# svohr/mixemt

Measured on AMD Instinct MI355X. Metric: read x hap cells/sec through the EM iteration (EM iters/sec reported beside it as em_iters_per_s), 1000000 reads x 5408 haps in total, whole job, higher is better.
Workload: dtype f64

## Files before the change

include/mixemt_hip.h:

```cpp
#ifndef MIXEMT_HIP_H
#define MIXEMT_HIP_H

#include <stddef.h>
#include <stdint.h>

#ifdef __cplusplus
extern "C" {
#endif

#define MXM_VERSION 603

typedef struct mxm_em_state {
    int32_t done;
    int32_t iters;
    double  l1;
    uint32_t ticket;
    uint32_t error;
} mxm_em_state;

int         mxm_version(void);
const char *mxm_last_error(void);
int         mxm_preload(void);

int         mxm_linear_supported(int32_t H);

int         mxm_restart_tile(int32_t H);

size_t      mxm_workspace_bytes(int64_t R, int32_t H, int32_t B);

int mxm_build_em_matrix(const uint8_t *E, int64_t lde,
                        const double *lhit, const double *lmiss,
                        const int64_t *row_ptr, const uint16_t *site,
                        const uint8_t *obs,
                        int64_t R, int32_t H, int32_t S,
                        double *M, int64_t ldm, void *stream);

int mxm_expand_tables(const uint8_t *maj, const int32_t *mk_ptr, const uint16_t *mk_hap, const uint8_t *mk_base,
                      const uint8_t *map256, int32_t S, int32_t H, int64_t lde, uint8_t *out, void *stream);

int mxm_build_em_matrix_lut(const uint8_t *Ecode, int64_t lde, const double *lhit, const double *lmiss,
                            const uint8_t *obsmap, const int64_t *row_ptr, const uint16_t *site,
                            const uint8_t *obs, const int64_t *order, int64_t R, int32_t H, int32_t S,
                            double *M, int64_t ldm, void *stream);

int mxm_build_em_matrix_lut_rows(const uint8_t *Ecode, int64_t lde, const double *lhit, const double *lmiss,
                                 const uint8_t *obsmap, const int64_t *row_ptr, const uint16_t *site,
                                 const uint8_t *obs, const int64_t *rows, int64_t n_rows, int32_t H, int32_t S,
                                 double *M_out, int64_t ldm, void *stream);

int mxm_build_em_matrix_sparse(const uint8_t *maj, const double *lhit, const double *lmiss,
                               const int32_t *mk_ptr, const uint16_t *mk_hap, const uint8_t *mk_base,
                               const int64_t *row_ptr, const uint16_t *site, const uint8_t *obs,
                               const int64_t *order, int64_t R, int32_t H, int32_t S,
                               double *M, int64_t ldm, int64_t *fallback, int64_t *n_fallback, void *stream);

size_t mxm_record_bytes(int64_t R, int32_t H);
int mxm_build_em_records(const uint8_t *maj, const double *lhit, const double *lmiss,
                         const int32_t *mk_ptr, const uint16_t *mk_hap, const uint8_t *mk_base,
                         const int64_t *row_ptr, const uint16_t *site, const uint8_t *obs,
                         const int64_t *order, int64_t R, int32_t H, int32_t S, double *M, int64_t ldm,
                         uint8_t *rec, size_t rec_bytes, int64_t *rec_off, int32_t *ndist, double *rowmax,
                         int64_t *stats, int64_t *fallback, int64_t *n_fallback, void *stream);

int mxm_linearize(const double *M, int64_t ldm, int64_t R, int32_t H,
                  double *P, int64_t ldp, double *rowmax, void *stream);

int mxm_em_iter(const double *M, int64_t ldm, const double *P, int64_t ldp,
                const double *w, const double *props, const double *ln_props,
                int64_t R, int32_t H, int32_t B,
                const mxm_em_state *state, double *colsum,
                void *ws, size_t ws_bytes, void *stream);

int mxm_m_finalize(const double *colsum, double *ln_cur, double *ln_new,
                   double *props_cur, int32_t H, int32_t B, double tol,
                   int32_t max_iter, mxm_em_state *state, void *stream);

int mxm_linearize_f32(const double *M, int64_t ldm, int64_t R, int32_t H,
                      float *P, int64_t ldp, double *rowmax, void *stream);
int mxm_em_iter_f32(const float *P, int64_t ldp, const double *w, const double *props,
                    int64_t R, int32_t H, int32_t B, const mxm_em_state *state,
                    double *colsum, void *ws, size_t ws_bytes, void *stream);
int mxm_em_loop_f32(const float *P, int64_t ldp, const double *w, int64_t R, int32_t H,
                    int32_t B, double *props_cur, double *ln_cur, double *ln_new,
                    double *colsum, mxm_em_state *state, double tol, int32_t max_iter,
                    int32_t check_every, void *ws, size_t ws_bytes, void *stream,
                    mxm_em_state *state_host);

typedef struct mxm_coded {
    const uint8_t *rec;
    const int64_t *rec_off;
    const int32_t *ndist;
    int64_t        R;
    const double  *P_rest;
    int64_t        ldp_rest;
    const double  *w_rest;
    int64_t        R_rest;
    const int64_t *wide_rows;
    int64_t        n_wide;
    const uint8_t *qrec;
    const int64_t *qoff;
    const int32_t *nquad;
    const int64_t *quad_rows;
    int64_t        n_quad_rows;
    const int64_t *byte_rows;
    int64_t        n_byte_rows;
} mxm_coded;
size_t mxm_coded_bytes(int64_t R, int32_t H);
size_t mxm_quad_bytes(int64_t R, int32_t H);
size_t mxm_quad_lists_scratch_bytes(int64_t R);
int mxm_quad_lists(const int32_t *ndist, const int32_t *nquad, int64_t R, int64_t *quad_rows, int64_t *byte_rows,
                   int64_t *counts, void *scratch, size_t scratch_bytes, void *stream);
int mxm_build_quads(const mxm_coded *c, int32_t H, uint8_t *qrec, size_t qrec_bytes, int64_t *qoff, int32_t *nquad,
                    uint64_t *stats, void *stream);
int mxm_encode_rows(const double *M, int64_t ldm, int64_t R, int32_t H, uint8_t *rec, size_t rec_bytes,
                    int64_t *rec_off, int32_t *ndist, double *rowmax, int64_t *stats, void *stream);
int mxm_decode_rows(const mxm_coded *c, int32_t H, double *P, int64_t ldp, void *stream);
int mxm_scatter_records(const int64_t *rows, int64_t n, const int64_t *sub_off, const int32_t *sub_nd, const double *sub_rm,
                        int64_t base, int64_t *rec_off, int32_t *ndist, double *rowmax, void *stream);
int mxm_row_argmax_votes_coded(const mxm_coded *c, int32_t H, int32_t n_runs, const double *ln_props,
                               const double *props, const double *rowmax, const double *M_rest, int64_t ldm_rest,
                               const int64_t *rest_rows, int64_t n_rest, const double *w, int32_t *best,
                               double *votes, void *ws, size_t ws_bytes, void *stream);
int mxm_em_step_coded(const mxm_coded *c, int32_t H, const double *ln_props, const double *props,
                      const double *rowmax, const double *M_rest, int64_t ldm_rest, const int64_t *rest_rows,
                      int64_t n_rest, double *out, int64_t ldo, int32_t mode, void *stream);
int mxm_gather_columns_coded(const mxm_coded *c, int32_t H, const int32_t *cols, int32_t nC,
                             const double *M_rest, int64_t ldm_rest, const int64_t *rest_rows, int64_t n_rest,
                             double *out, int64_t ldo, void *stream);
int mxm_em_iter_coded(const mxm_coded *c, const double *w, const double *props, int32_t H, int32_t B,
                      mxm_em_state *state , double *colsum, void *ws,
                      size_t ws_bytes, void *stream);
int64_t mxm_quad_loop_min_rows(int32_t B );
int mxm_restart_tile_coded(const mxm_coded *c, int32_t H);
int mxm_em_loop_coded(const mxm_coded *c, const double *w, int32_t H, int32_t B,
                      double *props_cur, double *ln_cur, double *ln_new, double *colsum,
                      mxm_em_state *state, double tol, int32_t max_iter, int32_t check_every,
                      void *ws, size_t ws_bytes, void *stream, mxm_em_state *state_host);

typedef struct mxm_sample_tile {
    int32_t sample;
    int32_t count;
    int64_t first;
} mxm_sample_tile;
int64_t mxm_samples_plan(const int64_t *row0_host, int32_t S, mxm_sample_tile *tiles_host, int64_t cap, int32_t *tile0_host);
size_t  mxm_samples_workspace_bytes(int64_t n_tiles, int32_t S, int32_t H);
int mxm_em_iter_samples(const mxm_coded *c, const int64_t *row0_host, int32_t S, const double *w, const double *props,
                        int32_t H, mxm_em_state *state, double *colsum, void *ws, size_t ws_bytes, void *stream);
int mxm_em_loop_samples(const mxm_coded *c, const int64_t *row0_host, int32_t S, const double *w, int32_t H,
                        double *props_cur, double *ln_cur, double *ln_new, double *colsum, mxm_em_state *state, double tol,
                        int32_t max_iter, int32_t check_every, void *ws, size_t ws_bytes, void *stream,
                        mxm_em_state *state_host);


int mxm_em_loop(const double *M, int64_t ldm, const double *P, int64_t ldp,
                const double *w, int64_t R, int32_t H, int32_t B,
                double *props_cur, double *ln_cur, double *ln_new, double *colsum,
                mxm_em_state *state, double tol, int32_t max_iter,
                int32_t check_every, void *ws, size_t ws_bytes, void *stream,
                mxm_em_state *state_host);

int mxm_em_step(const double *M, int64_t ldm, const double *w,
                const double *ln_props, int64_t R, int32_t H,
                double *out, int64_t ldo, int32_t mode, double *colsum,
                void *ws, size_t ws_bytes, void *stream);

int mxm_log_normalize(const double *colsum, int32_t H, double *ln_new,
                      void *stream);

int mxm_l1_exp_diff(const double *a, const double *b, int32_t H,
                    double *l1_out, void *stream);

int mxm_add_scalar(double *x, int64_t ld, int64_t R, int32_t H, double delta,
                   void *stream);

int mxm_row_argmax_votes(const double *X, int64_t ldx, const double *w,
                         int64_t R, int32_t H, int32_t *best, double *votes,
                         void *ws, size_t ws_bytes, void *stream);

int mxm_first_seen(const int32_t *best, int64_t R, int32_t H, int64_t *first, void *stream);

int mxm_assign_reads(const double *X, int64_t ldx, const double *log_props,
                     const int32_t *cols, int32_t nC, int64_t R, int32_t H,
                     double log_min_fold, int32_t *assigned, void *stream);

int mxm_gather_columns(const double *M, int64_t ldm, int64_t R, int32_t H,
                       const int32_t *cols, int32_t nC, double *out, int64_t ldo,
                       void *stream);

int mxm_fold_logaddexp(double *acc, int64_t lda, const double *const *in_host,
                       const int64_t *ld_in_host, int32_t n_in, int64_t R, int32_t H,
                       double delta, void *stream);

int64_t mxm_encode_signatures(const char *text, const int64_t *off, int64_t R,
                              const int32_t *site_of_pos, int64_t ref_len, int64_t *row_ptr,
                              uint16_t *site, uint8_t *obs, int64_t cap);

typedef struct mxm_aln_columns {
    int64_t         n_aln, n_frag;
    const int64_t  *ref_start;
    const int32_t  *mapq;
    const int64_t  *frag;
    const int64_t  *cig_ptr;
    const uint32_t *cigar;
    const int64_t  *seq_ptr;
    const uint8_t  *seq;
    const uint8_t  *qual;
    const uint8_t  *has_qual;
} mxm_aln_columns;
typedef struct mxm_aln_sizes {
    int64_t n_rows, nnz, n_grouped, n_dropped, text_bytes, n_frag_seen, frag_nnz;
} mxm_aln_sizes;
typedef struct mxm_aln_enc mxm_aln_enc;
int  mxm_aln_encode(const mxm_aln_columns *cols, const int32_t *site_of_pos, int64_t ref_len, const int64_t *site_pos,
                    int32_t n_sites, int32_t min_mq, int32_t min_bq, int32_t n_threads, mxm_aln_enc **out);
int  mxm_aln_sizes_of(const mxm_aln_enc *enc, mxm_aln_sizes *sizes);
int  mxm_aln_fetch(const mxm_aln_enc *enc, int64_t *row_ptr, uint16_t *site, uint8_t *obs, int64_t *weights,
                   int64_t *group_ptr, int64_t *group_frag, int64_t *dropped, char *text, int64_t *text_off);
int  mxm_aln_fetch_fragments(const mxm_aln_enc *enc, int64_t *frag_id, int64_t *frag_ptr, uint16_t *site, uint8_t *obs);
void mxm_aln_free(mxm_aln_enc *enc);

typedef struct mxm_bam_sizes {
    int64_t n_aln, n_frag, n_cigar, n_bases, names_bytes, n_ref, n_records_total, n_skipped_unplaced;
} mxm_bam_sizes;
typedef struct mxm_bam mxm_bam;
int  mxm_bam_read(const char *path, int32_t n_threads, mxm_bam **out);
int  mxm_bam_sizes_of(const mxm_bam *bam, mxm_bam_sizes *sizes);
int  mxm_bam_columns(const mxm_bam *bam, mxm_aln_columns *cols);
int  mxm_bam_fetch_names(const mxm_bam *bam, char *names, int64_t *name_off, int32_t *ref_id, uint16_t *flag);
void mxm_bam_free(mxm_bam *bam);

int  mxm_observe_bases(const mxm_aln_columns *cols, const uint8_t *is_reverse, int32_t min_mq, int32_t min_bq, int64_t L,
                       uint32_t *counts, void *stream);

int  mxm_observe_bases_labelled(const mxm_aln_columns *cols, const uint8_t *is_reverse, const int32_t *label,
                                int32_t n_labels, int32_t min_mq, int32_t min_bq, int64_t L, uint32_t *counts,
                                void *stream);

int  mxm_consensus(const uint32_t *counts, int32_t n_labels, int64_t L, int64_t ref_len, int64_t min_cov, int32_t strict,
                   uint8_t *cons, uint8_t *tied, uint32_t *n_tied, void *stream);

int  mxm_new_variants(const uint8_t *cons, int64_t ld, int32_t n_rows, const int32_t *rows, int32_t n_use, int64_t ref_len,
                      uint32_t *newvar, uint32_t *n_new, void *stream);

int  mxm_first_observed(const mxm_aln_columns *cols, const int32_t *label, const int32_t *joined, int32_t n_labels,
                        int32_t min_mq, int32_t min_bq, int64_t ref_len, const uint8_t *tied, uint8_t *cons, void *stream);

int  mxm_extend_assign(const mxm_aln_columns *cols, int32_t *label, int32_t *joined, int32_t unassigned, int32_t n_rows,
                       const int32_t *rows, int32_t n_use, int32_t round, int32_t min_mq, int32_t min_bq,
                       const uint32_t *newvar, int64_t ref_len, int32_t *frag_state, int32_t *moved_owner,
                       uint32_t *n_moved, void *stream);

typedef struct mxm_exchange mxm_exchange;
size_t mxm_exchange_handle_bytes(void);
int  mxm_exchange_create(int32_t world, int32_t rank, int64_t n_doubles, mxm_exchange **out, void *handle_out);
int  mxm_exchange_connect(mxm_exchange *x, const void *handles);
int  mxm_exchange_push(mxm_exchange *x, const double *colsum, int64_t n, void *stream);
int  mxm_exchange_pull(mxm_exchange *x, double *colsum, int64_t n, mxm_em_state *state, int32_t nb, void *stream);
int  mxm_exchange_reduce(mxm_exchange *x, double *colsum, int64_t n, mxm_em_state *state, int32_t nb, void *stream);
int  mxm_exchange_info(const mxm_exchange *x, int32_t *fine_grained, int64_t *bytes);
void mxm_exchange_destroy(mxm_exchange *x);

#ifdef __cplusplus
}
#endif
#include "mixemt_hip_samples_finish.h"
#include "mixemt_hip_var_check.h"
#endif
```

mixemt_amd/_lib.py:

```python

import ctypes
import os

_PKG = os.path.dirname(os.path.abspath(__file__))
LIB_PATH = os.environ.get("MXM_LIB") or os.path.join(_PKG, "lib", "libmixemt_hip.so")

c_i32, c_i64, c_f64 = ctypes.c_int32, ctypes.c_int64, ctypes.c_double
c_ptr, c_size = ctypes.c_void_p, ctypes.c_size_t


class EmState(ctypes.Structure):
    _fields_ = [("done", c_i32), ("iters", c_i32), ("l1", c_f64), ("ticket", ctypes.c_uint32), ("error", ctypes.c_uint32)]


class Coded(ctypes.Structure):
    _fields_ = [("rec", c_ptr), ("rec_off", c_ptr), ("ndist", c_ptr), ("R", c_i64),
                ("P_rest", c_ptr), ("ldp_rest", c_i64), ("w_rest", c_ptr), ("R_rest", c_i64),
                ("wide_rows", c_ptr), ("n_wide", c_i64),
                ("qrec", c_ptr), ("qoff", c_ptr), ("nquad", c_ptr), ("quad_rows", c_ptr), ("n_quad_rows", c_i64),
                ("byte_rows", c_ptr), ("n_byte_rows", c_i64)]


class SampleTile(ctypes.Structure):
    _fields_ = [("sample", c_i32), ("count", c_i32), ("first", c_i64)]


class AlnColumns(ctypes.Structure):
    _fields_ = [("n_aln", c_i64), ("n_frag", c_i64), ("ref_start", c_ptr), ("mapq", c_ptr), ("frag", c_ptr),
                ("cig_ptr", c_ptr), ("cigar", c_ptr), ("seq_ptr", c_ptr), ("seq", c_ptr), ("qual", c_ptr),
                ("has_qual", c_ptr)]


class AlnSizes(ctypes.Structure):
    _fields_ = [("n_rows", c_i64), ("nnz", c_i64), ("n_grouped", c_i64), ("n_dropped", c_i64), ("text_bytes", c_i64),
                ("n_frag_seen", c_i64), ("frag_nnz", c_i64)]


class BamSizes(ctypes.Structure):
    _fields_ = [("n_aln", c_i64), ("n_frag", c_i64), ("n_cigar", c_i64), ("n_bases", c_i64), ("names_bytes", c_i64),
                ("n_ref", c_i64), ("n_records_total", c_i64), ("n_skipped_unplaced", c_i64)]


SIGNATURES = {
    "mxm_version": (ctypes.c_int, []),
    "mxm_last_error": (ctypes.c_char_p, []),
    "mxm_linear_supported": (ctypes.c_int, [c_i32]),
    "mxm_workspace_bytes": (c_size, [c_i64, c_i32, c_i32]),
    "mxm_restart_tile": (ctypes.c_int, [c_i32]),
    "mxm_restart_tile_coded": (ctypes.c_int, [ctypes.POINTER(Coded), c_i32]),
    "mxm_quad_loop_min_rows": (c_i64, [c_i32]),
    "mxm_build_em_matrix": (ctypes.c_int, [c_ptr, c_i64, c_ptr, c_ptr, c_ptr, c_ptr, c_ptr,
                                           c_i64, c_i32, c_i32, c_ptr, c_i64, c_ptr]),
    "mxm_build_em_matrix_lut": (ctypes.c_int, [c_ptr, c_i64, c_ptr, c_ptr, c_ptr, c_ptr, c_ptr, c_ptr, c_ptr,
                                               c_i64, c_i32, c_i32, c_ptr, c_i64, c_ptr]),
    "mxm_build_em_matrix_sparse": (ctypes.c_int, [c_ptr, c_ptr, c_ptr, c_ptr, c_ptr, c_ptr, c_ptr, c_ptr, c_ptr, c_ptr,
                                                  c_i64, c_i32, c_i32, c_ptr, c_i64, c_ptr, c_ptr, c_ptr]),
    "mxm_build_em_matrix_lut_rows": (ctypes.c_int, [c_ptr, c_i64, c_ptr, c_ptr, c_ptr, c_ptr, c_ptr, c_ptr, c_ptr,
                                                    c_i64, c_i32, c_i32, c_ptr, c_i64, c_ptr]),
    "mxm_scatter_records": (ctypes.c_int, [c_ptr, c_i64, c_ptr, c_ptr, c_ptr, c_i64, c_ptr, c_ptr, c_ptr, c_ptr]),
    "mxm_preload": (ctypes.c_int, []),
    "mxm_record_bytes": (c_size, [c_i64, c_i32]),
    "mxm_build_em_records": (ctypes.c_int, [c_ptr, c_ptr, c_ptr, c_ptr, c_ptr, c_ptr, c_ptr, c_ptr, c_ptr, c_ptr,
                                            c_i64, c_i32, c_i32, c_ptr, c_i64, c_ptr, c_size, c_ptr, c_ptr, c_ptr,
                                            c_ptr, c_ptr, c_ptr, c_ptr]),
    "mxm_linearize": (ctypes.c_int, [c_ptr, c_i64, c_i64, c_i32, c_ptr, c_i64, c_ptr, c_ptr]),
    "mxm_em_iter": (ctypes.c_int, [c_ptr, c_i64, c_ptr, c_i64, c_ptr, c_ptr, c_ptr, c_i64, c_i32, c_i32,
                                   c_ptr, c_ptr, c_ptr, c_size, c_ptr]),
    "mxm_m_finalize": (ctypes.c_int, [c_ptr, c_ptr, c_ptr, c_ptr, c_i32, c_i32, c_f64, c_i32, c_ptr,
                                      c_ptr]),
    "mxm_em_loop": (ctypes.c_int, [c_ptr, c_i64, c_ptr, c_i64, c_ptr, c_i64, c_i32, c_i32,
                                   c_ptr, c_ptr, c_ptr, c_ptr, c_ptr, c_f64, c_i32, c_i32, c_ptr, c_size,
                                   c_ptr, ctypes.POINTER(EmState)]),
    "mxm_linearize_f32": (ctypes.c_int, [c_ptr, c_i64, c_i64, c_i32, c_ptr, c_i64, c_ptr, c_ptr]),
    "mxm_em_iter_f32": (ctypes.c_int, [c_ptr, c_i64, c_ptr, c_ptr, c_i64, c_i32, c_i32, c_ptr, c_ptr, c_ptr,
                                       c_size, c_ptr]),
    "mxm_em_loop_f32": (ctypes.c_int, [c_ptr, c_i64, c_ptr, c_i64, c_i32, c_i32, c_ptr, c_ptr, c_ptr, c_ptr,
                                       c_ptr, c_f64, c_i32, c_i32, c_ptr, c_size, c_ptr,
                                       ctypes.POINTER(EmState)]),
    "mxm_coded_bytes": (c_size, [c_i64, c_i32]),
    "mxm_exchange_handle_bytes": (c_size, []),
    "mxm_exchange_create": (ctypes.c_int, [c_i32, c_i32, c_i64, ctypes.POINTER(c_ptr), c_ptr]),
    "mxm_exchange_connect": (ctypes.c_int, [c_ptr, c_ptr]),
    "mxm_exchange_push": (ctypes.c_int, [c_ptr, c_ptr, c_i64, c_ptr]),
    "mxm_exchange_pull": (ctypes.c_int, [c_ptr, c_ptr, c_i64, c_ptr, c_i32, c_ptr]),
    "mxm_exchange_reduce": (ctypes.c_int, [c_ptr, c_ptr, c_i64, c_ptr, c_i32, c_ptr]),
    "mxm_exchange_info": (ctypes.c_int, [c_ptr, ctypes.POINTER(c_i32), ctypes.POINTER(c_i64)]),
    "mxm_exchange_destroy": (None, [c_ptr]),
    "mxm_expand_tables": (ctypes.c_int, [c_ptr, c_ptr, c_ptr, c_ptr, c_ptr, c_i32, c_i32, c_i64, c_ptr, c_ptr]),
    "mxm_quad_bytes": (c_size, [c_i64, c_i32]),
    "mxm_quad_lists_scratch_bytes": (c_size, [c_i64]),
    "mxm_quad_lists": (ctypes.c_int, [c_ptr, c_ptr, c_i64, c_ptr, c_ptr, c_ptr, c_ptr, c_size, c_ptr]),
    "mxm_build_quads": (ctypes.c_int, [ctypes.POINTER(Coded), c_i32, c_ptr, c_size, c_ptr, c_ptr, c_ptr, c_ptr]),
    "mxm_encode_rows": (ctypes.c_int, [c_ptr, c_i64, c_i64, c_i32, c_ptr, c_size, c_ptr, c_ptr, c_ptr, c_ptr, c_ptr]),
    "mxm_decode_rows": (ctypes.c_int, [ctypes.POINTER(Coded), c_i32, c_ptr, c_i64, c_ptr]),
    "mxm_row_argmax_votes_coded": (ctypes.c_int, [ctypes.POINTER(Coded), c_i32, c_i32, c_ptr, c_ptr, c_ptr, c_ptr, c_i64,
                                                  c_ptr, c_i64, c_ptr, c_ptr, c_ptr, c_ptr, c_size, c_ptr]),
    "mxm_em_step_coded": (ctypes.c_int, [ctypes.POINTER(Coded), c_i32, c_ptr, c_ptr, c_ptr, c_ptr, c_i64, c_ptr, c_i64,
                                         c_ptr, c_i64, c_i32, c_ptr]),
    "mxm_gather_columns_coded": (ctypes.c_int, [ctypes.POINTER(Coded), c_i32, c_ptr, c_i32, c_ptr, c_i64, c_ptr, c_i64,
                                                c_ptr, c_i64, c_ptr]),
    "mxm_em_iter_coded": (ctypes.c_int, [ctypes.POINTER(Coded), c_ptr, c_ptr, c_i32, c_i32, c_ptr, c_ptr, c_ptr,
                                         c_size, c_ptr]),
    "mxm_em_loop_coded": (ctypes.c_int, [ctypes.POINTER(Coded), c_ptr, c_i32, c_i32, c_ptr, c_ptr, c_ptr, c_ptr,
                                         c_ptr, c_f64, c_i32, c_i32, c_ptr, c_size, c_ptr,
                                         ctypes.POINTER(EmState)]),
    "mxm_samples_tile_rows": (ctypes.c_int, []),
    "mxm_samples_plan": (c_i64, [c_ptr, c_i32, c_ptr, c_i64, c_ptr]),
    "mxm_samples_workspace_bytes": (c_size, [c_i64, c_i32, c_i32]),
    "mxm_em_iter_samples": (ctypes.c_int, [ctypes.POINTER(Coded), c_ptr, c_i32, c_ptr, c_ptr, c_i32, c_ptr, c_ptr, c_ptr,
                                           c_size, c_ptr]),
    "mxm_em_loop_samples": (ctypes.c_int, [ctypes.POINTER(Coded), c_ptr, c_i32, c_ptr, c_i32, c_ptr, c_ptr, c_ptr, c_ptr,
                                           c_ptr, c_f64, c_i32, c_i32, c_ptr, c_size, c_ptr, ctypes.POINTER(EmState)]),
    "mxm_em_step": (ctypes.c_int, [c_ptr, c_i64, c_ptr, c_ptr, c_i64, c_i32, c_ptr, c_i64, c_i32,
                                   c_ptr, c_ptr, c_size, c_ptr]),
    "mxm_log_normalize": (ctypes.c_int, [c_ptr, c_i32, c_ptr, c_ptr]),
    "mxm_l1_exp_diff": (ctypes.c_int, [c_ptr, c_ptr, c_i32, c_ptr, c_ptr]),
    "mxm_add_scalar": (ctypes.c_int, [c_ptr, c_i64, c_i64, c_i32, c_f64, c_ptr]),
    "mxm_assign_reads": (ctypes.c_int, [c_ptr, c_i64, c_ptr, c_ptr, c_i32, c_i64, c_i32, c_f64, c_ptr, c_ptr]),
    "mxm_diag_stream_read": (ctypes.c_int, [c_ptr, c_size, c_i32, c_i32, c_ptr, c_ptr]),
    "mxm_diag_stream_coded": (ctypes.c_int, [ctypes.POINTER(Coded), c_i32, c_i32, c_ptr, c_ptr]),
    "mxm_diag_stream_quads": (ctypes.c_int, [ctypes.POINTER(Coded), c_i32, c_i32, c_ptr, c_ptr]),
    "mxm_diag_fused_force_abort": (ctypes.c_int, [c_i32]),
    "mxm_set_fused_coded_grid": (ctypes.c_int, [c_i32]),
    "mxm_set_quad_left_grid": (ctypes.c_int, [c_i32]),
    "mxm_set_coded_batch_tile": (ctypes.c_int, [c_i32]),
    "mxm_set_sparse_long_rows": (ctypes.c_int, [c_i32]),
    "mxm_set_quad_encoder": (ctypes.c_int, [c_i32]),
    "mxm_set_sparse_long_entries": (ctypes.c_int, [c_i32]),
    "mxm_diag_fused_stamps": (ctypes.c_int, [c_ptr, ctypes.POINTER(ctypes.c_ulonglong)]),
    "mxm_set_timing_events": (ctypes.c_int, [c_ptr, c_ptr]),
    "mxm_set_batch_tile": (ctypes.c_int, [c_i32]),
    "mxm_encode_signatures": (ctypes.c_int64, [ctypes.c_char_p, c_ptr, c_i64, c_ptr, c_i64, c_ptr, c_ptr, c_ptr,
                                               c_i64]),
    "mxm_aln_encode": (ctypes.c_int, [ctypes.POINTER(AlnColumns), c_ptr, c_i64, c_ptr, c_i32, c_i32, c_i32, c_i32,
                                      ctypes.POINTER(c_ptr)]),
    "mxm_aln_sizes_of": (ctypes.c_int, [c_ptr, ctypes.POINTER(AlnSizes)]),
    "mxm_aln_fetch": (ctypes.c_int, [c_ptr, c_ptr, c_ptr, c_ptr, c_ptr, c_ptr, c_ptr, c_ptr, c_ptr, c_ptr]),
    "mxm_aln_fetch_fragments": (ctypes.c_int, [c_ptr, c_ptr, c_ptr, c_ptr, c_ptr]),
    "mxm_aln_free": (None, [c_ptr]),
    "mxm_bam_read": (ctypes.c_int, [ctypes.c_char_p, c_i32, ctypes.POINTER(c_ptr)]),
    "mxm_bam_sizes_of": (ctypes.c_int, [c_ptr, ctypes.POINTER(BamSizes)]),
    "mxm_bam_columns": (ctypes.c_int, [c_ptr, ctypes.POINTER(AlnColumns)]),
    "mxm_bam_fetch_names": (ctypes.c_int, [c_ptr, c_ptr, c_ptr, c_ptr, c_ptr]),
    "mxm_bam_free": (None, [c_ptr]),
    "mxm_observe_bases": (ctypes.c_int, [ctypes.POINTER(AlnColumns), c_ptr, c_i32, c_i32, c_i64, c_ptr, c_ptr]),
    "mxm_observe_bases_labelled": (ctypes.c_int, [ctypes.POINTER(AlnColumns), c_ptr, c_ptr, c_i32, c_i32, c_i32, c_i64,
                                                  c_ptr, c_ptr]),
    "mxm_consensus": (ctypes.c_int, [c_ptr, c_i32, c_i64, c_i64, c_i64, c_i32, c_ptr, c_ptr, c_ptr, c_ptr]),
    "mxm_new_variants": (ctypes.c_int, [c_ptr, c_i64, c_i32, ctypes.POINTER(c_i32), c_i32, c_i64, c_ptr, c_ptr, c_ptr]),
    "mxm_first_observed": (ctypes.c_int, [ctypes.POINTER(AlnColumns), c_ptr, c_ptr, c_i32, c_i32, c_i32, c_i64, c_ptr,
                                          c_ptr, c_ptr]),
    "mxm_extend_assign": (ctypes.c_int, [ctypes.POINTER(AlnColumns), c_ptr, c_ptr, c_i32, c_i32, ctypes.POINTER(c_i32),
                                         c_i32, c_i32, c_i32, c_i32, c_ptr, c_i64, c_ptr, c_ptr, c_ptr, c_ptr]),
    "mxm_set_compact_restarts": (ctypes.c_int, [c_i32]),
    "mxm_set_loop_graph": (ctypes.c_int, [c_i32]),
    "mxm_set_loop_fused": (ctypes.c_int, [c_i32, c_i32]),
    "mxm_set_progress_callback": (ctypes.c_int, [c_ptr, c_ptr, c_i32]),
    "mxm_set_min_rows_per_wg": (ctypes.c_int, [c_i32]),
    "mxm_reset_tuning": (ctypes.c_int, []),
    "mxm_describe_stream_kernel": (ctypes.c_int, [c_i32, c_i32, ctypes.c_char_p, c_size]),
    "mxm_set_sparse_max_distinct": (ctypes.c_int, [c_i32]),
    "mxm_row_argmax_votes": (ctypes.c_int, [c_ptr, c_i64, c_ptr, c_i64, c_i32, c_ptr, c_ptr,
                                            c_ptr, c_size, c_ptr]),
    "mxm_first_seen": (ctypes.c_int, [c_ptr, c_i64, c_i32, c_ptr, c_ptr]),
    "mxm_gather_columns": (ctypes.c_int, [c_ptr, c_i64, c_i64, c_i32, c_ptr, c_i32, c_ptr, c_i64, c_ptr]),
    "mxm_fold_logaddexp": (ctypes.c_int, [c_ptr, c_i64, ctypes.POINTER(c_ptr), ctypes.POINTER(c_i64), c_i32,
                                          c_i64, c_i32, c_f64, c_ptr]),
}

FINISH_SIGNATURES = {
    "mxm_samples_finish_workspace_bytes": (c_size, [c_i64, c_i32, c_i32]),
    "mxm_votes_samples": (ctypes.c_int, [ctypes.POINTER(Coded), c_ptr, c_i32, c_i32, c_ptr, c_ptr, c_ptr, c_ptr, c_ptr, c_ptr,
                                         c_ptr, c_ptr, c_ptr, c_ptr, c_ptr, c_size, c_ptr]),
    "mxm_gather_columns_samples": (ctypes.c_int, [ctypes.POINTER(Coded), c_ptr, c_i32, c_i32, c_ptr, c_ptr, c_i32, c_ptr,
                                                  c_ptr, c_size, c_ptr]),
    "mxm_em_loop_samples_narrow": (ctypes.c_int, [ctypes.POINTER(Coded), c_ptr, c_i32, c_i32, c_ptr, c_i32, c_ptr, c_ptr,
                                                  c_ptr, c_ptr, c_ptr, c_ptr, c_f64, c_i32, c_i32, c_ptr, c_ptr, c_size,
                                                  c_ptr, ctypes.POINTER(EmState)]),
    "mxm_assign_reads_samples": (ctypes.c_int, [ctypes.POINTER(Coded), c_ptr, c_i32, c_i32, c_ptr, c_i32, c_ptr, c_ptr,
                                                c_ptr, c_ptr, c_ptr, c_ptr, c_f64, c_ptr, c_ptr, c_ptr, c_size, c_ptr]),
}

VARCHECK_SIGNATURES = {
    "mxm_check_variants_samples": (ctypes.c_int, [c_ptr, c_i32, c_i64, c_ptr, c_ptr, c_i32, c_ptr, c_ptr, c_i32, c_i64, c_ptr,
                                                  c_ptr, c_i32, c_f64, c_f64, c_f64, c_i32, c_i32, c_ptr, c_ptr, c_ptr, c_ptr]),
}

ABI_VERSION = 603

PROGRESS_FN = ctypes.CFUNCTYPE(None, ctypes.POINTER(EmState), c_i32, c_ptr)

_lib = None


class MixemtHipError(RuntimeError):
    pass


def load():
    global _lib
    if _lib is not None:
        return _lib
    if not os.path.exists(LIB_PATH):
        raise MixemtHipError(
            "libmixemt_hip.so is not built (%s); run `python -m mixemt_amd.build` -- "
            "there is no CPU fallback for the EM hot path" % LIB_PATH)
    from . import _dev
    lib = ctypes.CDLL(LIB_PATH)
    try:
        lib.mxm_version.restype = ctypes.c_int
        lib.mxm_version.argtypes = []
        have = lib.mxm_version()
    except AttributeError:
        have = None
    if have != ABI_VERSION:
        raise MixemtHipError("%s reports ABI version %s, this binding was written for %d: rebuild with "
                             "`python -m mixemt_amd.build --force`" % (LIB_PATH, have, ABI_VERSION))
    for name, (restype, argtypes) in (list(SIGNATURES.items()) + list(FINISH_SIGNATURES.items())
                                      + list(VARCHECK_SIGNATURES.items())):
        try:
            fn = getattr(lib, name)
        except AttributeError:
            raise MixemtHipError("%s has ABI version %d but lacks %s: rebuild with "
                                 "`python -m mixemt_amd.build --force`" % (LIB_PATH, have, name))
        fn.restype = restype
        fn.argtypes = argtypes
    _lib = lib
    try:
        if _dev.torch is not None and _dev.torch.cuda.is_available():
            lib.mxm_preload()
    except Exception:
        pass
    return lib


def check(rc, what):
    if rc != 0:
        msg = load().mxm_last_error().decode("utf-8", "replace")
        raise ValueError("%s failed (%d): %s" % (what, rc, msg))
```

mixemt_amd/build.py:

```python

import hashlib
import os
import shutil
import subprocess
import sys

_PKG = os.path.dirname(os.path.abspath(__file__))
_ROOT = os.path.dirname(_PKG)
SRC = os.path.join(_PKG, "csrc", "mixemt_hip.hip")
HDRS = [os.path.join(_ROOT, "include", name) for name in ("mixemt_hip.h", "mixemt_hip_tuning.h", "mixemt_hip_samples_finish.h",
                                                           "mixemt_hip_var_check.h")]
LIB_DIR = os.path.join(_PKG, "lib")
LIB = os.path.join(LIB_DIR, "libmixemt_hip.so")
ARCH = "gfx950"


def _hipcc():
    for cand in (os.environ.get("HIPCC"), shutil.which("hipcc"), "/opt/rocm/bin/hipcc"):
        if cand and os.path.exists(cand):
            return cand
    raise RuntimeError("hipcc not found (set HIPCC or add /opt/rocm/bin to PATH)")


def _sources():
    csrc = os.path.dirname(SRC)
    return sorted(os.path.join(csrc, f) for f in os.listdir(csrc) if f.endswith((".hip", ".hpp"))) + HDRS


def _digest(flags):
    h = hashlib.sha256()
    for path in _sources():
        with open(path, "rb") as fin:
            h.update(fin.read())
    h.update(" ".join(flags).encode())
    return h.hexdigest()


def build(force=False, defines=(), verbose=False, out=None):
    global LIB
    if out is not None:
        LIB = os.path.abspath(out)
    flags = ["--offload-arch=%s" % ARCH, "-O3", "-std=c++17", "-shared", "-fPIC", "-Werror=format",
             "-I" + os.path.join(_ROOT, "include"), "-I" + os.path.dirname(SRC)]
    flags += ["-D%s" % d for d in defines]
    stamp = LIB + ".stamp"
    want = _digest(flags)
    if not force and os.path.exists(LIB) and os.path.exists(stamp):
        with open(stamp) as fin:
            if fin.read().strip() == want:
                return LIB
    os.makedirs(os.path.dirname(LIB), exist_ok=True)
    cmd = [_hipcc()] + flags + [SRC, "-o", LIB, "-lz"]
    if verbose:
        sys.stderr.write(" ".join(cmd) + "\n")
    proc = subprocess.run(cmd, stdout=subprocess.PIPE, stderr=subprocess.STDOUT, text=True)
    if proc.returncode != 0:
        raise RuntimeError("hipcc failed:\n" + proc.stdout)
    with open(stamp, "w") as fout:
        fout.write(want + "\n")
    return LIB


if __name__ == "__main__":
    defs = []
    argv = sys.argv[1:]
    i = 0
    while i < len(argv):
        if argv[i] == "-D":
            defs.append(argv[i + 1])
            i += 2
        elif argv[i].startswith("-D"):
            defs.append(argv[i][2:])
            i += 1
        else:
            i += 1
    out_path = argv[argv.index("--out") + 1] if "--out" in argv else None
    print(build(force="--force" in argv, defines=defs, verbose=True, out=out_path))
```

mixemt_amd/csrc/mixemt_hip.hip:

```cpp
#include <hip/hip_runtime.h>
#include <stdint.h>
#include <stdio.h>
#include <stdlib.h>
#include <string.h>
#include <math.h>
#include <algorithm>
#include <atomic>
#include <mutex>
#include <type_traits>
#include <utility>
#include <vector>

#include "mixemt_hip.h"
#include "mixemt_hip_tuning.h"

#include "common.hpp"
#include "aln_encode.hpp"
#include "bam_reader.hpp"
#include "coded_kernels.hpp"
#include "quad_kernels.hpp"
#include "quad_batched_kernels.hpp"
#include "build_kernels.hpp"
#include "build_lut_kernels.hpp"
#include "build_sparse_kernels.hpp"
#include "em_kernels.hpp"
#include "estep_kernels.hpp"
#include "aux_kernels.hpp"
#include "records_kernels.hpp"
#include "fused_kernels.hpp"
#include "fused_cols_kernels.hpp"
#include "fused_coded_kernels.hpp"
#include "fused_narrow_kernels.hpp"
#include "samples_kernels.hpp"
#include "samples_finish_kernels.hpp"
#include "exchange.hpp"
#include "aln_walk.hpp"
#include "observe_kernels.hpp"
#include "var_check_kernels.hpp"
#include "assemble_kernels.hpp"


struct mxm_em_state;
typedef void (*mxm_progress_fn)(const mxm_em_state *state_host, int32_t B, void *user);
struct mxm_tuning {
    int sparse_maxd = -1;
    int min_rows_per_wg = 8;
    int compact_restarts = 2;
    int max_bt = 4;
    int loop_graph = -1;
    int loop_fused = -1;
    int fused_chunk = 0;
    int fused_cols = 1;
    int fused_coded_wg = 0;
    int quad_left_wg = 0;
    int sparse_long_entries = 5120;
    int quad_encoder = 1;
    int sparse_long = 1;
    int coded_bt = 3;
    int fused_force_abort = 0;
    double fused_cells = 1.0e8;
    hipEvent_t ev_start = nullptr, ev_stop = nullptr;
    mxm_progress_fn progress = nullptr;
    void *progress_user = nullptr;
    int progress_every = 10;
};
static std::mutex g_tune_mu;
static mxm_tuning g_tune;
static thread_local mxm_tuning T;
#define MXM_ENTER() do { std::lock_guard<std::mutex> lk_(g_tune_mu); T = g_tune; } while (0)
template <typename F>
static int tune_set(F f) {
    std::lock_guard<std::mutex> lk(g_tune_mu);
    f(g_tune);
    return 0;
}
extern "C" int mxm_reset_tuning(void) {
    return tune_set([](mxm_tuning &t) { t = mxm_tuning(); });
}

static inline int clamp_grid(int64_t want, int cap) {
    if (want < 1) want = 1;
    return (int)(want < cap ? want : cap);
}

static inline int64_t part_ld(int H) { return ((int64_t)H + 1) & ~(int64_t)1; }

static hipError_t raise_dynamic_lds(const void *kernel, size_t bytes, const char *name) {
    const hipError_t e = hipFuncSetAttribute(kernel, hipFuncAttributeMaxDynamicSharedMemorySize, (int)bytes);
    if (e != hipSuccess)
        snprintf(g_err, sizeof(g_err), "%s: cannot opt into %zu bytes of dynamic LDS: %s", name, bytes,
                 hipGetErrorString(e));
    return e;
}
static int dynamic_lds_ok(const void *kernel, size_t bytes, const char *name, const char *who = nullptr, int H = 0,
                          const char *too_wide = nullptr) {
    if (too_wide != nullptr && bytes > 150 * 1024) return fail(-1, "%s: H=%d %s", who, H, too_wide);
    if (bytes > 60 * 1024 && raise_dynamic_lds(kernel, bytes, name) != hipSuccess) return -2;
    return 0;
}

#define RC_TRY(expr)                                                                         \
    do {                                                                                     \
        const int rc_ = (expr);                                                              \
        if (rc_ != 0) return rc_;                                                            \
    } while (0)

template <int MAX, typename F>
static bool dispatch_width(int n, F &&f) {
    if constexpr (MAX < 1) {
        return false;
    } else {
        if (n != MAX) return dispatch_width<MAX - 1>(n, f);
        f(std::integral_constant<int, MAX>{});
        return true;
    }
}

extern "C" int mxm_version(void) { return MXM_VERSION; }
extern "C" const char *mxm_last_error(void) { return g_err; }

extern "C" int mxm_linear_supported(int32_t H) {
    return (H >= MXM_LINEAR_MIN_H && H <= 8192) ? 1 : 0;
}

static size_t fused_sync_bytes() { return (sizeof(fused_sync) + 255) & ~(size_t)255; }
static size_t fused_snapshot_bytes(int H, int B) {
    return ((size_t)3 * B * H * sizeof(double) + (size_t)B * sizeof(mxm_em_state) + 255) & ~(size_t)255;
}
static size_t fused_rows_bytes(int H, int nwg) { return (size_t)(nwg + 2) * part_ld(H) * sizeof(double); }
static size_t fused_cols_bytes(int64_t R, int nwg) {
    const size_t ldz = (size_t)((R + 1) & ~(int64_t)1);
    return ((size_t)(nwg + 1) * ldz + 2 * (size_t)nwg) * sizeof(double);
}

extern "C" size_t mxm_workspace_bytes(int64_t R, int32_t H, int32_t B) {
    const size_t tiles = (size_t)MXM_MAX_WG * MXM_MAX_BT * (size_t)part_ld(H) * sizeof(double);
    size_t fused = fused_rows_bytes(H, MXM_MAX_WG);
    if (R > 0 && R <= (int64_t)FCOLS_MAX_RPT * FCOLS_THREADS) fused = std::max(fused, fused_cols_bytes(R, MXM_MAX_WG));
    fused += fused_sync_bytes() + fused_snapshot_bytes(H, B > 0 ? B : 1) + 512;
    return std::max(tiles, fused);
}

extern "C" int64_t mxm_encode_signatures(const char *text, const int64_t *off, int64_t R,
                                         const int32_t *site_of_pos, int64_t ref_len, int64_t *row_ptr,
                                         uint16_t *site, uint8_t *obs, int64_t cap) {
    int64_t n = 0;
    row_ptr[0] = 0;
    for (int64_t r = 0; r < R; ++r) {
        const char *p = text + off[r];
        const char *end = text + off[r + 1] - 1;
        if (p >= end) return -(r + 1);
        while (p < end) {
            int64_t pos = 0;
            int digits = 0;
            while (p < end && *p >= '0' && *p <= '9' && digits < 10) {
                pos = pos * 10 + (*p - '0');
                ++p;
                ++digits;
            }
            if (digits == 0 || digits >= 10 || p >= end || *p != ':') return -(r + 1);
            ++p;
            const char *b = p;
            while (p < end && *p != ',') {
                if (*p == ':') return -(r + 1);
                ++p;
            }
            if (pos >= ref_len || site_of_pos[pos] < 0 || n >= cap) return -(r + 1);
            site[n] = (uint16_t)site_of_pos[pos];
            obs[n] = (p - b == 1) ? (uint8_t)*b : (uint8_t)0;
            ++n;
            if (p < end) {
                ++p;
                if (p >= end) return -(r + 1);
            }
        }
        row_ptr[r + 1] = n;
    }
    return n;
}

extern "C" int mxm_build_em_matrix(const uint8_t *E, int64_t lde, const double *lhit,
                                   const double *lmiss, const int64_t *row_ptr, const uint16_t *site,
                                   const uint8_t *obs, int64_t R, int32_t H, int32_t S, double *M,
                                   int64_t ldm, void *stream) {
    if (R < 0 || H <= 0 || S <= 0) return fail(-1, "mxm_build_em_matrix: bad shape R=%lld H=%d", (long long)R, H);
    if (lde < (((int64_t)H + 7) & ~(int64_t)7) || (lde & 7) != 0 || (reinterpret_cast<uintptr_t>(E) & 7) != 0)
        return fail(-1, "mxm_build_em_matrix: E must be 8-byte aligned with lde a multiple of 8 and >= H rounded up to 8 (lde=%lld)", (long long)lde);
    if (ldm < H) return fail(-1, "mxm_build_em_matrix: ldm < H");
    if (S > 65536) return fail(-1, "mxm_build_em_matrix: more than 65536 variant sites");
    if (R == 0) return 0;
    const int grid = clamp_grid(R, num_cu() * 8);
    const int vec_ok = ((ldm & 1) == 0) && ((reinterpret_cast<uintptr_t>(M) & 15) == 0);
    hipLaunchKernelGGL(build_em_matrix_kernel, dim3(grid), dim3(BUILD_THREADS), 0, (hipStream_t)stream, E,
                       lde, lhit, lmiss, row_ptr, site, obs, R, (int)H, M, ldm, vec_ok);
    HIP_TRY(hipGetLastError());
    return 0;
}

static int build_lut_impl(const char *who, const uint8_t *Ecode, int64_t lde, const double *lhit,
                          const double *lmiss, const uint8_t *obsmap, const int64_t *row_ptr, const uint16_t *site,
                          const uint8_t *obs, const int64_t *order, int64_t R, int32_t H, int32_t S, double *M, int64_t ldm,
                          int compact, hipStream_t s) {
    if (H > 8192) return fail(-1, "%s: more than 8192 haplogroups (H=%d)%s", who, H, compact ? "" : ": use mxm_build_em_matrix");
    if (lde < (((int64_t)H + 7) & ~(int64_t)7) || (lde & 7) != 0 || (reinterpret_cast<uintptr_t>(Ecode) & 7) != 0)
        return fail(-1, "%s: Ecode must be 8-byte aligned with lde a multiple of 8 and >= H rounded up to 8 (lde=%lld)", who, (long long)lde);
    if (ldm < H) return fail(-1, "%s: ldm < H", who);
    if (S > 65536 || (int64_t)S * lde >= ((int64_t)1 << 31))
        return fail(-1, "%s: table of %d x %lld bytes exceeds one buffer descriptor", who, S, (long long)lde);
    if (R == 0) return 0;
    const int grid = clamp_grid(R, num_cu() * 8);
    const int nt = (H + LUT_THREADS * LUT_CPL - 1) / (LUT_THREADS * LUT_CPL);
    const int vec_ok = ((ldm & 1) == 0) && ((reinterpret_cast<uintptr_t>(M) & 15) == 0);
    const bool ok = dispatch_width<8>(nt, [&](auto n) {
        constexpr int NT = decltype(n)::value;
        hipLaunchKernelGGL((build_lut_kernel<NT, LUT_CPL>), dim3(grid), dim3(LUT_THREADS), 0, s, Ecode, lde, (int64_t)S * lde, lhit,
                           lmiss, obsmap, row_ptr, site, obs, order, R, (int)H, M, ldm, vec_ok, compact);
    });
    if (!ok) return fail(-1, "%s: H=%d outside the kernel's range", who, H);
    HIP_TRY(hipGetLastError());
    return 0;
}

extern "C" int mxm_build_em_matrix_lut(const uint8_t *Ecode, int64_t lde, const double *lhit, const double *lmiss,
                                       const uint8_t *obsmap, const int64_t *row_ptr, const uint16_t *site,
                                       const uint8_t *obs, const int64_t *order, int64_t R, int32_t H, int32_t S,
                                       double *M, int64_t ldm, void *stream) {
    if (R < 0 || H <= 0 || S <= 0) return fail(-1, "mxm_build_em_matrix_lut: bad shape R=%lld H=%d", (long long)R, H);
    return build_lut_impl("mxm_build_em_matrix_lut", Ecode, lde, lhit, lmiss, obsmap, row_ptr, site, obs,
                          order, R, H, S, M, ldm, 0, (hipStream_t)stream);
}

extern "C" int mxm_build_em_matrix_lut_rows(const uint8_t *Ecode, int64_t lde, const double *lhit, const double *lmiss,
                                            const uint8_t *obsmap, const int64_t *row_ptr, const uint16_t *site,
                                            const uint8_t *obs, const int64_t *rows, int64_t n_rows, int32_t H, int32_t S,
                                            double *M_out, int64_t ldm, void *stream) {
    if (n_rows < 0 || H <= 0 || S <= 0 || rows == nullptr) return fail(-1, "mxm_build_em_matrix_lut_rows: bad arguments");
    return build_lut_impl("mxm_build_em_matrix_lut_rows", Ecode, lde, lhit, lmiss, obsmap, row_ptr, site, obs, rows, n_rows, H, S,
                          M_out, ldm, 1, (hipStream_t)stream);
}

__global__ __launch_bounds__(256) void scatter_records_kernel(const int64_t *__restrict__ rows, int64_t n, const int64_t *__restrict__ sub_off,
                                                             const int32_t *__restrict__ sub_nd, const double *__restrict__ sub_rm,
                                                             int64_t base, int64_t *__restrict__ rec_off, int32_t *__restrict__ ndist,
                                                             double *__restrict__ rowmax) {
    const int64_t i = (int64_t)blockIdx.x * 256 + threadIdx.x;
    if (i >= n || sub_nd[i] <= 0) return;
    const int64_t r = rows[i];
    rec_off[r] = sub_off[i] + base;
    ndist[r] = sub_nd[i];
    rowmax[r] = sub_rm[i];
}
extern "C" int mxm_scatter_records(const int64_t *rows, int64_t n, const int64_t *sub_off, const int32_t *sub_nd, const double *sub_rm,
                                   int64_t base, int64_t *rec_off, int32_t *ndist, double *rowmax, void *stream) {
    if (n < 0 || (n > 0 && (rows == nullptr || sub_off == nullptr || sub_nd == nullptr || sub_rm == nullptr || rec_off == nullptr ||
                            ndist == nullptr || rowmax == nullptr)))
        return fail(-1, "mxm_scatter_records: bad arguments");
    if (n == 0) return 0;
    hipLaunchKernelGGL(scatter_records_kernel, dim3((unsigned)((n + 255) / 256)), dim3(256), 0, (hipStream_t)stream, rows, n, sub_off,
                       sub_nd, sub_rm, base, rec_off, ndist, rowmax);
    HIP_TRY(hipGetLastError());
    return 0;
}

__global__ void preload_kernel() {}
extern "C" int mxm_preload(void) {
    hipLaunchKernelGGL(preload_kernel, dim3(1), dim3(64), 0, (hipStream_t)nullptr);
    HIP_TRY(hipGetLastError());
    HIP_TRY(hipDeviceSynchronize());
    return 0;
}

extern "C" int mxm_set_sparse_max_distinct(int32_t n) {
    return tune_set([n](mxm_tuning &t) { t.sparse_maxd = n < 0 ? -1 : n; });
}

static inline int coded_ld(int H) { return (H + 7) & ~7; }

static int build_sparse_impl(const char *who, const uint8_t *maj, const double *lhit, const double *lmiss,
                             const int32_t *mk_ptr, const uint16_t *mk_hap, const uint8_t *mk_base,
                             const int64_t *row_ptr, const uint16_t *site, const uint8_t *obs, const int64_t *order,
                             int64_t R, int32_t H, int32_t S, double *M, int64_t ldm, const spb_records *out,
                             int64_t *fallback, int64_t *n_fallback, hipStream_t s) {
    if (R < 0 || H <= 0 || S <= 0) return fail(-1, "%s: bad shape R=%lld H=%d", who, (long long)R, H);
    if (H > 8192) return fail(-1, "%s: more than 8192 haplogroups (H=%d): use mxm_build_em_matrix", who, H);
    if (M != nullptr && ldm < H) return fail(-1, "%s: ldm < H", who);
    if (maj == nullptr || mk_ptr == nullptr || fallback == nullptr || n_fallback == nullptr)
        return fail(-1, "%s: marker tables and the fallback list are required", who);
    HIP_TRY(hipMemsetAsync(n_fallback, 0, sizeof(int64_t), s));
    if (out != nullptr) HIP_TRY(hipMemsetAsync(out->stats, 0, 2 * sizeof(int64_t), s));
    if (R == 0) return 0;
    const int hpad = (H + 1) & ~1;
    const int nch = (hpad / 2 + SPB_THREADS - 1) / SPB_THREADS;
    const int vec_ok = (M != nullptr) && ((ldm & 1) == 0) && ((reinterpret_cast<uintptr_t>(M) & 15) == 0);
#ifndef SPB_PASSES
#define SPB_PASSES 3
#endif
    const int passes = SPB_PASSES;
    const int maxd = (T.sparse_maxd < 0 || T.sparse_maxd > SPB_MAXD) ? SPB_MAXD : T.sparse_maxd;
    const int maxd_long = (T.sparse_maxd < 0 || T.sparse_maxd > SPB_MAXD_LONG) ? SPB_MAXD_LONG : T.sparse_maxd;
    const int kpp = (nch + passes - 1) / passes;
    const size_t lds = (size_t)kpp * 2 * SPB_THREADS * 8 + SPB_SLOTS * 8 + 6 * 1024;
    int per_cu = (int)((160 * 1024) / lds);
    if (per_cu > 8) per_cu = 8;
    if (per_cu < 1) per_cu = 1;
    const int grid = clamp_grid(R, num_cu() * per_cu * 2);
    const int long_too = T.sparse_long;
    const int grid_long = clamp_grid((R + SPB_LONG_CHUNK - 1) / SPB_LONG_CHUNK, num_cu() * 4 * 2);
    spb_records none = {};
    const spb_records rec = out != nullptr ? *out : none;
    auto launch = [&](auto kernel, int nwg, int max_distinct, int long_rows_too, int long_entries) {
        hipLaunchKernelGGL(kernel, dim3(nwg), dim3(SPB_THREADS), 0, s, maj, lhit, lmiss, mk_ptr, mk_hap, mk_base, row_ptr, site, obs,
                           order, R, (int)H, M, ldm, vec_ok, fallback, reinterpret_cast<unsigned long long *>(n_fallback), max_distinct,
                           rec, long_rows_too, long_entries);
    };
    constexpr int P = SPB_PASSES < 4 ? SPB_PASSES : 4;
    bool one_pass_too_wide = false;
    const bool ok = dispatch_width<16>(nch, [&](auto n) {
        constexpr int N = decltype(n)::value;
        if constexpr (P == 1 && N > 7) one_pass_too_wide = true;
        else if (out != nullptr) launch(build_sparse_kernel<N, P, true, 1>, grid, maxd, long_too, 0);
        else launch(build_sparse_kernel<N, P, false, 1>, grid, maxd, long_too, 0);
    });
    if (one_pass_too_wide) return fail(-1, "%s: one pass covers H <= 3584", who);
    if (!ok) return fail(-1, "%s: H=%d outside the kernel's range", who, H);
    HIP_TRY(hipGetLastError());
    if (long_too != 0) {
#ifndef SPB_LONG_KPP
#define SPB_LONG_KPP 2
#endif
        (void)dispatch_width<16>(nch, [&](auto n) {
            constexpr int N = decltype(n)::value, PL = (N + SPB_LONG_KPP - 1) / SPB_LONG_KPP;
            if (out != nullptr) launch(build_sparse_kernel<N, PL, true, 2>, grid_long, maxd_long, 0, T.sparse_long_entries);
            else launch(build_sparse_kernel<N, PL, false, 2>, grid_long, maxd_long, 0, T.sparse_long_entries);
        });
    }
    HIP_TRY(hipGetLastError());
    return 0;
}

extern "C" int mxm_build_em_matrix_sparse(const uint8_t *maj, const double *lhit, const double *lmiss,
                                          const int32_t *mk_ptr, const uint16_t *mk_hap, const uint8_t *mk_base,
                                          const int64_t *row_ptr, const uint16_t *site, const uint8_t *obs,
                                          const int64_t *order, int64_t R, int32_t H, int32_t S, double *M, int64_t ldm,
                                          int64_t *fallback, int64_t *n_fallback, void *stream) {
    MXM_ENTER();
    if (M == nullptr) return fail(-1, "mxm_build_em_matrix_sparse: M required");
    return build_sparse_impl("mxm_build_em_matrix_sparse", maj, lhit, lmiss, mk_ptr, mk_hap, mk_base, row_ptr, site, obs,
                             order, R, H, S, M, ldm, nullptr, fallback, n_fallback, (hipStream_t)stream);
}

extern "C" size_t mxm_record_bytes(int64_t R, int32_t H) {
    if (R < 0 || H <= 0) return 0;
    return (size_t)(R > 0 ? R : 1) * (2 * (size_t)coded_ld(H) + 16 * ENC_MAX_WIDE);
}

extern "C" int mxm_build_em_records(const uint8_t *maj, const double *lhit, const double *lmiss,
                                    const int32_t *mk_ptr, const uint16_t *mk_hap, const uint8_t *mk_base,
                                    const int64_t *row_ptr, const uint16_t *site, const uint8_t *obs,
                                    const int64_t *order, int64_t R, int32_t H, int32_t S, double *M, int64_t ldm,
                                    uint8_t *rec, size_t rec_bytes, int64_t *rec_off, int32_t *ndist, double *rowmax,
                                    int64_t *stats, int64_t *fallback, int64_t *n_fallback, void *stream) {
    MXM_ENTER();
    if (!mxm_linear_supported(H))
        return fail(-1, "mxm_build_em_records: records need H in [65, 8192] (H=%d)", H);
    if (rec == nullptr || (reinterpret_cast<uintptr_t>(rec) & 15) || rec_bytes < (size_t)coded_ld(H) + 16 * ENC_MAX_CODES ||
        rec_off == nullptr || ndist == nullptr || rowmax == nullptr || stats == nullptr)
        return fail(-1, "mxm_build_em_records: record buffer (16-byte aligned, >= one record) and output arrays required");
    spb_records out;
    out.rec = rec;
    out.rec_cap = (long long)rec_bytes;
    out.rec_off = rec_off;
    out.ndist = ndist;
    out.rowmax = rowmax;
    out.stats = reinterpret_cast<unsigned long long *>(stats);
    out.ldc = coded_ld(H);
    return build_sparse_impl("mxm_build_em_records", maj, lhit, lmiss, mk_ptr, mk_hap, mk_base, row_ptr, site, obs, order,
                             R, H, S, M, ldm, &out, fallback, n_fallback, (hipStream_t)stream);
}

template <typename ST>
static int linearize_wide(const double *M, int64_t ldm, int64_t R, int H, ST *P, int64_t ldp, double *rowmax,
                          hipStream_t s) {
    const int nch = (H / 2 + 255) / 256;
    int cap = num_cu() * 2 < MXM_MAX_WG ? num_cu() * 2 : MXM_MAX_WG;
    const int nwg = clamp_grid((R + 1) / 2, cap);
    const bool ok = dispatch_width<16>(nch, [&](auto n) {
        hipLaunchKernelGGL((linearize_wide_kernel<decltype(n)::value, ST>), dim3(nwg), dim3(256), 0, s, M, ldm, R, H, P, ldp, rowmax);
    });
    return ok ? 0 : 1;
}

static inline bool wide_rows_ok(const void *M, int64_t ldm, int H) {
    return ((H & 1) == 0) && ((ldm & 1) == 0) && ((reinterpret_cast<uintptr_t>(M) & 15) == 0) && H >= 64 && H <= 8192;
}

extern "C" int mxm_linearize(const double *M, int64_t ldm, int64_t R, int32_t H, double *P, int64_t ldp,
                             double *rowmax, void *stream) {
    if (R < 0 || H <= 0) return fail(-1, "mxm_linearize: bad shape");
    if (ldm < H || ldp < H || (ldp & 1)) return fail(-1, "mxm_linearize: ldp must be even and >= H (ldp=%lld)", (long long)ldp);
    if (R == 0) return 0;
    if (wide_rows_ok(M, ldm, H) && (reinterpret_cast<uintptr_t>(P) & 15) == 0 &&
        linearize_wide<double>(M, ldm, R, (int)H, P, ldp, rowmax, (hipStream_t)stream) == 0) {
        HIP_TRY(hipGetLastError());
        return 0;
    }
    const int grid = clamp_grid(R, num_cu() * 8);
    hipLaunchKernelGGL(linearize_kernel, dim3(grid), dim3(ROW_THREADS), 0, (hipStream_t)stream, M, ldm, R,
                       (int)H, P, ldp, rowmax);
    HIP_TRY(hipGetLastError());
    return 0;
}

extern "C" int mxm_set_timing_events(void *ev_start, void *ev_stop) {
    return tune_set([=](mxm_tuning &t) { t.ev_start = (hipEvent_t)ev_start; t.ev_stop = (hipEvent_t)ev_stop; });
}

extern "C" int mxm_set_min_rows_per_wg(int32_t n) {
    if (n < 1) return fail(-1, "mxm_set_min_rows_per_wg: n < 1");
    return tune_set([n](mxm_tuning &t) { t.min_rows_per_wg = n; });
}

extern "C" int mxm_set_compact_restarts(int32_t mode) {
    return tune_set([mode](mxm_tuning &t) { t.compact_restarts = mode < 0 ? 0 : (mode > 2 ? 2 : mode); });
}

extern "C" int mxm_set_batch_tile(int32_t bt) {
    if (bt < 1 || bt > 4) return fail(-1, "mxm_set_batch_tile: tile must be 1..4");
    return tune_set([bt](mxm_tuning &t) { t.max_bt = bt; });
}

extern "C" int mxm_set_fused_coded_grid(int32_t nwg) {
    return tune_set([nwg](mxm_tuning &t) { t.fused_coded_wg = nwg > 0 ? nwg : 0; });
}

extern "C" int mxm_set_sparse_long_rows(int32_t on) {
    return tune_set([on](mxm_tuning &t) { t.sparse_long = on ? 1 : 0; });
}
extern "C" int mxm_set_sparse_long_entries(int32_t n) {
    return tune_set([n](mxm_tuning &t) { t.sparse_long_entries = n > 0 ? n : 0; });
}
extern "C" int mxm_set_coded_batch_tile(int32_t bt) {
    if (bt != 1 && bt != 3) return fail(-1, "mxm_set_coded_batch_tile: 1 or 3, got %d", bt);
    return tune_set([bt](mxm_tuning &t) { t.coded_bt = bt; });
}
extern "C" int mxm_set_quad_encoder(int32_t kind) {
    if (kind != 0 && kind != 1) return fail(-1, "mxm_set_quad_encoder: 0 or 1, got %d", kind);
    return tune_set([kind](mxm_tuning &t) { t.quad_encoder = kind; });
}
extern "C" int mxm_set_quad_left_grid(int32_t nwg) {
    return tune_set([nwg](mxm_tuning &t) { t.quad_left_wg = nwg > 0 ? nwg : 0; });
}

extern "C" int mxm_diag_fused_force_abort(int32_t on) {
    return tune_set([on](mxm_tuning &t) { t.fused_force_abort = on ? 1 : 0; });
}

#ifndef MXM_V1_THREADS
#define MXM_V1_THREADS 256
#endif
#ifndef MXM_V1_NBUF
#define MXM_V1_NBUF 2
#endif
#ifndef MXM_V1_WG_PER_CU
#define MXM_V1_WG_PER_CU 2
#endif
#ifndef MXM_V2_THREADS
#define MXM_V2_THREADS 512
#endif
#ifndef MXM_V2_NBUF
#define MXM_V2_NBUF 2
#endif
#ifndef MXM_V3_THREADS
#define MXM_V3_THREADS 512
#endif
#ifndef MXM_V3_NBUF
#define MXM_V3_NBUF 2
#endif
#ifndef MXM_V4_THREADS
#define MXM_V4_THREADS 512
#endif
#ifndef MXM_V4_NBUF
#define MXM_V4_NBUF 2
#endif
#ifndef MXM_V2_PREG
#define MXM_V2_PREG 1
#endif
#ifndef MXM_V3_PREG
#define MXM_V3_PREG 2
#endif
#ifndef MXM_V4_PREG
#define MXM_V4_PREG 2
#endif
#ifndef MXM_V1B_THREADS
#define MXM_V1B_THREADS 512
#endif
#ifndef MXM_V1B_NBUF
#define MXM_V1B_NBUF 3
#endif
#define MXM_MAX_COL2 4096
#define MXM_LDS_BUDGET (156 * 1024)

static inline int variant_threads(int nb) {
    return nb == 1 ? MXM_V1_THREADS : (nb == 2 ? MXM_V2_THREADS : (nb == 3 ? MXM_V3_THREADS : MXM_V4_THREADS));
}
static inline int variant_preg(int nb) {
    return nb == 1 ? 1 : (nb == 2 ? MXM_V2_PREG : (nb == 3 ? MXM_V3_PREG : MXM_V4_PREG));
}

static size_t batch_lds_bytes(int H, int nb) {
    const int threads = variant_threads(nb);
    const int nch = ((H + 1) / 2 + threads - 1) / threads;
    return (size_t)(nb - variant_preg(nb)) * nch * threads * 16;
}

static bool batch_fits(int H, int nb) {
    if (nb <= 1) return true;
    static const int max_nch[MXM_MAX_BT + 1] = {0, 16, 8, 7, 6};
    const int threads = variant_threads(nb);
    const int nch = ((H + 1) / 2 + threads - 1) / threads;
    return nch <= max_nch[nb] && batch_lds_bytes(H, nb) <= MXM_LDS_BUDGET;
}

template <int THREADS, int NCH, int BT, int NBUF, int PREG>
static int launch_wide(const double *P, int64_t ldp, const double *w, const double *props, int64_t R,
                       int H, int grid, double *partial, int64_t ldpart,
                       const mxm_em_state *state, mxm_slots slots, hipStream_t stream) {
    if constexpr (NCH * THREADS > MXM_MAX_COL2) {
        return fail(-1, "mxm_em_iter: H=%d outside the linear kernel's range", H);
    } else {
        const size_t lds = (size_t)(BT - PREG) * NCH * THREADS * sizeof(d2);
        RC_TRY(dynamic_lds_ok(reinterpret_cast<const void *>(&em_iter_wide_kernel<THREADS, NCH, BT, NBUF, PREG>), lds, "em_iter_wide_kernel"));
        hipLaunchKernelGGL((em_iter_wide_kernel<THREADS, NCH, BT, NBUF, PREG>), dim3(grid), dim3(THREADS), lds,
                           stream, P, ldp, w, props, R, H, partial, ldpart, state, slots);
        return 0;
    }
}

template <int THREADS, int BT, int NBUF, int PREG>
static int dispatch_wide(int nch, const double *P, int64_t ldp, const double *w, const double *props,
                         int64_t R, int H, int grid, double *partial,
                         int64_t ldpart, const mxm_em_state *state, mxm_slots slots, hipStream_t stream) {
    int rc = 0;
    const bool ok = dispatch_width<16>(nch, [&](auto n) {
        rc = launch_wide<THREADS, decltype(n)::value, BT, NBUF, PREG>(P, ldp, w, props, R, H, grid, partial, ldpart, state, slots, stream);
    });
    return ok ? rc : fail(-1, "mxm_em_iter: H=%d outside the linear kernel's range", H);
}

static inline mxm_slots slots_from(int first) {
    mxm_slots sl;
    for (int i = 0; i < MXM_MAX_BT; ++i) sl.s[i] = first + i;
    return sl;
}

static int stream_linear_tile(const double *P, int64_t ldp, const double *w, const double *props, int64_t R,
                              int H, int nb, mxm_slots &slots, const mxm_em_state *state,
                              double *partial, hipStream_t stream, bool timed, int *nwg_out, int max_wg = MXM_MAX_WG,
                              int v1_shape = -1) {
    const int64_t ldpart = part_ld(H);
    const int ncol2 = (H + 1) / 2;
    if (v1_shape < 0) v1_shape = 1;
    const bool alt = (nb == 1) && (v1_shape == 1);
    const int threads = alt ? MXM_V1B_THREADS : variant_threads(nb);
    const int wg_per_cu = alt ? 1 : ((nb == 1) ? MXM_V1_WG_PER_CU : 1);
    const int nch = (ncol2 + threads - 1) / threads;
    int cap = num_cu() * wg_per_cu;
    if (cap > max_wg) cap = max_wg;
    const int nwg = clamp_grid((R + T.min_rows_per_wg - 1) / T.min_rows_per_wg, cap);
    for (int i = nb; i < MXM_MAX_BT; ++i) slots.s[i] = slots.s[0];
    if (timed && T.ev_start != nullptr) HIP_TRY(hipEventRecord(T.ev_start, stream));
    int rc;
    if (alt)
        rc = dispatch_wide<MXM_V1B_THREADS, 1, MXM_V1B_NBUF, 1>(nch, P, ldp, w, props, R, H, nwg, partial, ldpart, state, slots, stream);
    else if (nb == 1)
        rc = dispatch_wide<MXM_V1_THREADS, 1, MXM_V1_NBUF, 1>(nch, P, ldp, w, props, R, H, nwg, partial, ldpart, state, slots, stream);
    else if (nb == 2)
        rc = dispatch_wide<MXM_V2_THREADS, 2, MXM_V2_NBUF, MXM_V2_PREG>(nch, P, ldp, w, props, R, H, nwg, partial, ldpart, state, slots, stream);
    else if (nb == 3)
        rc = dispatch_wide<MXM_V3_THREADS, 3, MXM_V3_NBUF, MXM_V3_PREG>(nch, P, ldp, w, props, R, H, nwg, partial, ldpart, state, slots, stream);
    else
        rc = dispatch_wide<MXM_V4_THREADS, 4, MXM_V4_NBUF, MXM_V4_PREG>(nch, P, ldp, w, props, R, H, nwg, partial, ldpart, state, slots, stream);
    if (rc != 0) return rc;
    HIP_TRY(hipGetLastError());
    if (timed && T.ev_stop != nullptr) HIP_TRY(hipEventRecord(T.ev_stop, stream));
    *nwg_out = nwg;
    return 0;
}

extern "C" int mxm_describe_stream_kernel(int32_t H, int32_t nb, char *buf, size_t len) {
    if (buf == nullptr || len == 0 || H <= 0 || nb < 1 || nb > MXM_MAX_BT) return fail(-1, "mxm_describe_stream_kernel: bad arguments");
    const int ncol2 = (H + 1) / 2;
    const bool alt = nb == 1;
    const int threads = alt ? MXM_V1B_THREADS : variant_threads(nb);
    const int nbuf = alt ? MXM_V1B_NBUF : (nb == 2 ? MXM_V2_NBUF : (nb == 3 ? MXM_V3_NBUF : MXM_V4_NBUF));
    snprintf(buf, len, "em_iter_wide_kernel<%d, %d, %d, %d, %d>", threads, (ncol2 + threads - 1) / threads, nb, nbuf,
             variant_preg(nb));
    return 0;
}

struct fin_args {
    double *ln_cur, *ln_new, *props_cur;
    mxm_em_state *state;
    double tol;
    int max_iter;
};

static int reduce_tile(const double *partial, int nwg, int nb, int H, double *colsum, const mxm_em_state *state,
                       const mxm_slots &slots, const fin_args *fin, hipStream_t stream,
                       wide_check wc = wide_check{nullptr, 0, 0}) {
    if (fin != nullptr && H <= 64 * FIN_MAX_BLOCKS)
        hipLaunchKernelGGL(colreduce_finalize_kernel, dim3((H + 63) / 64, nb), dim3(COLRED_THREADS), 0, stream, partial,
                           part_ld(H), nwg, nb, H, colsum, fin->ln_cur, fin->ln_new, fin->props_cur, fin->tol, fin->max_iter,
                           fin->state, slots, wc);
    else
        hipLaunchKernelGGL(colreduce_kernel, dim3((H + 63) / 64, nb), dim3(COLRED_THREADS), 0, stream, partial, part_ld(H), nwg,
                           nb, H, (const double *)nullptr, colsum, const_cast<mxm_em_state *>(state), slots, wc);
    HIP_TRY(hipGetLastError());
    return 0;
}

static int reduce_one(const double *partial, int nwg, int H, double *colsum, const mxm_em_state *state, hipStream_t stream) {
    hipLaunchKernelGGL(colreduce_kernel, dim3((H + 63) / 64, 1), dim3(COLRED_THREADS), 0, stream, partial, part_ld(H), nwg, 1, H,
                       (const double *)nullptr, colsum, const_cast<mxm_em_state *>(state), slots_from(0), wide_check{nullptr, 0, 0});
    HIP_TRY(hipGetLastError());
    return 0;
}

static int em_iter_linear_tile(const double *P, int64_t ldp, const double *w, const double *props, int64_t R,
                               int H, int nb, mxm_slots slots, const mxm_em_state *state, double *colsum,
                               double *partial, hipStream_t stream, bool timed, const fin_args *fin = nullptr) {
    int nwg = 0;
    RC_TRY(stream_linear_tile(P, ldp, w, props, R, H, nb, slots, state, partial, stream, timed, &nwg));
    return reduce_tile(partial, nwg, nb, H, colsum, state, slots, fin, stream);
}

#ifndef MXM_F32_THREADS
#define MXM_F32_THREADS 256
#endif
#ifndef MXM_F32_NBUF
#define MXM_F32_NBUF 2
#endif
#ifndef MXM_F32_WG_PER_CU
#define MXM_F32_WG_PER_CU 2
#endif

template <int NCH>
static int launch_wide_f32(const float *P, int64_t ldp, const double *w, const double *props, int64_t R, int H,
                           int grid, double *partial, int64_t ldpart,
                           const mxm_em_state *state, hipStream_t stream) {
    if constexpr (NCH * MXM_F32_THREADS > 2048) {
        return fail(-1, "mxm_em_iter_f32: H=%d outside the kernel's range", H);
    } else {
        hipLaunchKernelGGL((em_iter_wide_f32_kernel<MXM_F32_THREADS, NCH, MXM_F32_NBUF>), dim3(grid),
                           dim3(MXM_F32_THREADS), 0, stream, P, ldp, w, props, R, H, partial, ldpart,
                           state);
        return 0;
    }
}

static int em_iter_f32_one(const float *P, int64_t ldp, const double *w, const double *props, int64_t R, int H,
                           const mxm_em_state *state, double *colsum, double *partial, hipStream_t stream,
                           bool timed) {
    const int64_t ldpart = part_ld(H);
    const int nch = ((H + 3) / 4 + MXM_F32_THREADS - 1) / MXM_F32_THREADS;
    const int nbuf = MXM_F32_NBUF;
    int cap = num_cu() * MXM_F32_WG_PER_CU;
    if (cap > MXM_MAX_WG) cap = MXM_MAX_WG;
    const int nwg = clamp_grid((R + nbuf - 1) / nbuf, cap);
    if (timed && T.ev_start != nullptr) HIP_TRY(hipEventRecord(T.ev_start, stream));
    int lrc = 0;
    const bool ok = dispatch_width<8>(nch, [&](auto n) {
        lrc = launch_wide_f32<decltype(n)::value>(P, ldp, w, props, R, H, nwg, partial, ldpart, state, stream);
    });
    if (!ok) return fail(-1, "mxm_em_iter_f32: H=%d outside the kernel's range", H);
    if (lrc != 0) return lrc;
    HIP_TRY(hipGetLastError());
    if (timed && T.ev_stop != nullptr) HIP_TRY(hipEventRecord(T.ev_stop, stream));
    return reduce_one(partial, nwg, H, colsum, state, stream);
}

#define MXM_NARROW_MAX_H 64
template <bool ITER>
static int launch_narrow(const double *M, int64_t ldm, const double *w, const double *ln_props, int64_t R, int H,
                         double *out, int64_t ldo, int mode, double *partial, int64_t ldpart,
                         const mxm_em_state *state, hipStream_t stream, int *nwg_out) {
    const int cap = num_cu() * 4 < MXM_MAX_WG ? num_cu() * 4 : MXM_MAX_WG;
    const int rows_per_wg = (H <= 32) ? 256 : 128;
    const int nwg = clamp_grid((R + rows_per_wg - 1) / rows_per_wg, cap);
    *nwg_out = nwg;
#define NARROW_LAUNCH(hmax, lpr)                                                                             \
    hipLaunchKernelGGL((estep_narrow_kernel<hmax, ITER, lpr>), dim3(nwg), dim3(256), 0, stream, M, ldm, w, ln_props, R, H, \
                       out, ldo, mode, partial, ldpart, state)
    if (H <= 4) NARROW_LAUNCH(4, 1);
    else if (H <= 8) NARROW_LAUNCH(8, 1);
    else if (H <= 16) NARROW_LAUNCH(16, 1);
    else if (H <= 32) NARROW_LAUNCH(32, 1);
    else NARROW_LAUNCH(32, 2);
#undef NARROW_LAUNCH
    HIP_TRY(hipGetLastError());
    return 0;
}

static int em_iter_log_one(const double *M, int64_t ldm, const double *w, const double *ln_props, int64_t R, int H,
                           const mxm_em_state *state, double *colsum, double *partial, hipStream_t stream) {
    if (M == nullptr) return fail(-1, "mxm_em_iter: M is NULL and the linear path does not apply");
    if (ln_props == nullptr) return fail(-1, "mxm_em_iter: ln_props is NULL and the log-space path needs it");
    const size_t lds = 2 * (size_t)H * sizeof(double);
    const int64_t ldpart = part_ld(H);
    int nwg;
    if (lds > 150 * 1024) {
        nwg = clamp_grid(R, num_cu() * 2 < MXM_MAX_WG ? num_cu() * 2 : MXM_MAX_WG);
        hipLaunchKernelGGL((estep_global_kernel<true>), dim3(nwg), dim3(ROW_THREADS), 0, stream, M, ldm, w, ln_props, R, H,
                           (double *)nullptr, (int64_t)0, 0, partial, ldpart, state, (const int64_t *)nullptr);
        HIP_TRY(hipGetLastError());
    } else if (H <= MXM_NARROW_MAX_H) {
        const int rc = launch_narrow<true>(M, ldm, w, ln_props, R, H, (double *)nullptr, (int64_t)0, 0, partial, ldpart,
                                           state, stream, &nwg);
        if (rc != 0) return rc;
    } else {
        nwg = clamp_grid(R, num_cu() * 2 < MXM_MAX_WG ? num_cu() * 2 : MXM_MAX_WG);
        RC_TRY(dynamic_lds_ok(reinterpret_cast<const void *>(&estep_log_kernel<true>), lds, "estep_log_kernel"));
        hipLaunchKernelGGL((estep_log_kernel<true>), dim3(nwg), dim3(ROW_THREADS), lds, stream, M, ldm, w, ln_props,
                           R, H, (double *)nullptr, (int64_t)0, 0, partial, ldpart, state);
        HIP_TRY(hipGetLastError());
    }
    return reduce_one(partial, nwg, H, colsum, state, stream);
}

extern "C" int mxm_em_iter(const double *M, int64_t ldm, const double *P, int64_t ldp, const double *w,
                           const double *props, const double *ln_props, int64_t R, int32_t H, int32_t B,
                           const mxm_em_state *state, double *colsum, void *ws, size_t ws_bytes, void *stream) {
    MXM_ENTER();
    if (R <= 0 || H <= 0 || B <= 0) return fail(-1, "mxm_em_iter: bad shape R=%lld H=%d", (long long)R, H);
    if (ws == nullptr || ws_bytes < mxm_workspace_bytes(R, H, B)) return fail(-1, "mxm_em_iter: workspace too small");
    if (P != nullptr && ((ldp & 1) || ldp < H)) return fail(-1, "mxm_em_iter: ldp must be even and >= H");
    if (M != nullptr && ldm < H) return fail(-1, "mxm_em_iter: ldm < H");
    const bool linear = (P != nullptr) && mxm_linear_supported(H);
    int max_bt = linear ? T.max_bt : 1;
    while (max_bt > 1 && !batch_fits((int)H, max_bt)) --max_bt;
    for (int b = 0; b < B;) {
        const int left = B - b;
        const int passes = (left + max_bt - 1) / max_bt;
        const int nb = (left + passes - 1) / passes;
        const mxm_em_state *st = state ? state + b : nullptr;
        int rc;
        if (linear)
            rc = em_iter_linear_tile(P, ldp, w, props, R, (int)H, nb, slots_from(b), state, colsum, (double *)ws,
                                     (hipStream_t)stream, b == 0);
        else
            rc = em_iter_log_one(M, ldm, w, ln_props ? ln_props + (int64_t)b * H : nullptr, R, (int)H, st,
                                 colsum + (int64_t)b * H, (double *)ws, (hipStream_t)stream);
        if (rc != 0) return rc;
        b += nb;
    }
    return 0;
}

extern "C" int mxm_linearize_f32(const double *M, int64_t ldm, int64_t R, int32_t H, float *P, int64_t ldp,
                                 double *rowmax, void *stream) {
    if (R < 0 || H <= 0) return fail(-1, "mxm_linearize_f32: bad shape");
    if (ldm < H || ldp < H || (ldp & 3)) return fail(-1, "mxm_linearize_f32: ldp must be a multiple of 4 and >= H (ldp=%lld)", (long long)ldp);
    if (R == 0) return 0;
    if (wide_rows_ok(M, ldm, H) && (reinterpret_cast<uintptr_t>(P) & 7) == 0 && (ldp & 1) == 0 &&
        linearize_wide<float>(M, ldm, R, (int)H, P, ldp, rowmax, (hipStream_t)stream) == 0) {
        HIP_TRY(hipGetLastError());
        return 0;
    }
    const int grid = clamp_grid(R, num_cu() * 8);
    hipLaunchKernelGGL(linearize_f32_kernel, dim3(grid), dim3(ROW_THREADS), 0, (hipStream_t)stream, M, ldm, R, (int)H,
                       P, ldp, rowmax);
    HIP_TRY(hipGetLastError());
    return 0;
}

extern "C" int mxm_em_iter_f32(const float *P, int64_t ldp, const double *w, const double *props, int64_t R,
                               int32_t H, int32_t B, const mxm_em_state *state, double *colsum, void *ws,
                               size_t ws_bytes, void *stream) {
    MXM_ENTER();
    if (R <= 0 || H <= 0 || B <= 0) return fail(-1, "mxm_em_iter_f32: bad shape R=%lld H=%d", (long long)R, H);
    if (!mxm_linear_supported(H)) return fail(-1, "mxm_em_iter_f32: H=%d outside the linear kernel's range", H);
    if (P == nullptr || (ldp & 3) || ldp < H) return fail(-1, "mxm_em_iter_f32: ldp must be a multiple of 4 and >= H");
    if (ws == nullptr || ws_bytes < mxm_workspace_bytes(R, H, B)) return fail(-1, "mxm_em_iter_f32: workspace too small");
    for (int b = 0; b < B; ++b) {
        const int rc = em_iter_f32_one(P, ldp, w, props + (int64_t)b * H, R, (int)H, state ? state + b : nullptr,
                                       colsum + (int64_t)b * H, (double *)ws, (hipStream_t)stream, b == 0);
        if (rc != 0) return rc;
    }
    return 0;
}

extern "C" size_t mxm_coded_bytes(int64_t R, int32_t H) { return mxm_record_bytes(R, H); }

extern "C" int mxm_encode_rows(const double *M, int64_t ldm, int64_t R, int32_t H, uint8_t *rec, size_t rec_bytes,
                               int64_t *rec_off, int32_t *ndist, double *rowmax, int64_t *stats, void *stream) {
    if (R <= 0 || H <= 0 || ldm < H) return fail(-1, "mxm_encode_rows: bad shape R=%lld H=%d", (long long)R, H);
    if (!mxm_linear_supported(H) || (reinterpret_cast<uintptr_t>(M) & 7) != 0)
        return fail(-1, "mxm_encode_rows: needs H in [65, 8192] (H=%d ldm=%lld)", H, (long long)ldm);
    if (rec == nullptr || (reinterpret_cast<uintptr_t>(rec) & 15) || rec_bytes < (size_t)coded_ld(H) + 16 * ENC_MAX_CODES)
        return fail(-1, "mxm_encode_rows: record buffer missing, unaligned or smaller than one record");
    if (rec_off == nullptr || ndist == nullptr || rowmax == nullptr || stats == nullptr)
        return fail(-1, "mxm_encode_rows: output arrays required");
    hipStream_t s = (hipStream_t)stream;
    HIP_TRY(hipMemsetAsync(stats, 0, 2 * sizeof(int64_t), s));
    const int ldc = coded_ld(H);
    const int nch = (ldc / 4 + ENC_THREADS - 1) / ENC_THREADS;
    const int grid = clamp_grid(R, num_cu() * 4);
    const int grid_w = clamp_grid((R + 31) / 32, num_cu() * 3);
    const bool ok = dispatch_width<8>(nch, [&](auto n) {
        constexpr int NCH = decltype(n)::value;
        unsigned long long *st = reinterpret_cast<unsigned long long *>(stats);
        hipLaunchKernelGGL((encode_rows_kernel<NCH>), dim3(grid), dim3(ENC_THREADS), 0, s, M, ldm, R, (int)H, ldc, rec,
                           (int64_t)rec_bytes, rec_off, ndist, rowmax, st);
        hipLaunchKernelGGL((encode_wide_rows_kernel<NCH>), dim3(grid_w), dim3(ENC_THREADS), 0, s, M, ldm, R, (int)H, ldc, rec,
                           (int64_t)rec_bytes, rec_off, ndist, rowmax, st);
    });
    if (!ok) return fail(-1, "mxm_encode_rows: H=%d outside the kernel's range", H);
    HIP_TRY(hipGetLastError());
    return 0;
}

static int coded_check(const mxm_coded *c, int32_t H, const char *who) {
    if (c == nullptr || c->R <= 0 || H <= 0 || !mxm_linear_supported(H))
        return fail(-1, "%s: bad coded matrix (rows %lld, H %d)", who, (long long)(c ? c->R : 0), H);
    if (c->rec == nullptr || c->rec_off == nullptr || c->ndist == nullptr) return fail(-1, "%s: coded matrix arrays missing", who);
    if (c->R_rest < 0 || (c->R_rest > 0 && (c->P_rest == nullptr || c->ldp_rest < H || (c->ldp_rest & 1) ||
                                            (reinterpret_cast<uintptr_t>(c->P_rest) & 15))))
        return fail(-1, "%s: the dense rest needs 16-byte aligned rows with an even ld >= H", who);
    if (c->n_wide < 0 || (c->n_wide > 0 && c->wide_rows == nullptr)) return fail(-1, "%s: n_wide > 0 needs wide_rows", who);
    if (c->qrec != nullptr) {
        if (c->qoff == nullptr || c->nquad == nullptr || c->n_quad_rows < 0 || c->n_byte_rows < 0 ||
            (c->n_quad_rows > 0 && c->quad_rows == nullptr) || (c->n_byte_rows > 0 && c->byte_rows == nullptr) ||
            (reinterpret_cast<uintptr_t>(c->qrec) & 31))
            return fail(-1, "%s: quad dictionary arrays missing (or qrec not 32-byte aligned)", who);
        if (c->n_quad_rows + c->n_byte_rows + c->n_wide + c->R_rest != c->R)
            return fail(-1, "%s: quad_rows + byte_rows + wide_rows + the dense rest must be all %lld rows", who, (long long)c->R);
    }
    return 0;
}

static int rest_check(const char *who, int32_t H, const double *M_rest, int64_t ldm_rest, const int64_t *rest_rows, int64_t n_rest) {
    if (n_rest < 0 || (n_rest > 0 && (M_rest == nullptr || rest_rows == nullptr || ldm_rest < H)))
        return fail(-1, "%s: the rows without a record need M_rest, rest_rows and ldm_rest >= H", who);
    return 0;
}

extern "C" size_t mxm_quad_bytes(int64_t R, int32_t H) {
    (void)H;
    constexpr size_t largest = QUAD_CODE_BYTES + QUAD_MAX * 32, per_piece = (size_t)QUAD_CHUNK / largest;
    return R > 0 ? (((size_t)R + per_piece - 1) / per_piece + 5120) * (size_t)QUAD_CHUNK : 0;
}

extern "C" int mxm_expand_tables(const uint8_t *maj, const int32_t *mk_ptr, const uint16_t *mk_hap, const uint8_t *mk_base,
                                 const uint8_t *map256, int32_t S, int32_t H, int64_t lde, uint8_t *out, void *stream) {
    if (maj == nullptr || mk_ptr == nullptr || mk_hap == nullptr || mk_base == nullptr || out == nullptr || S <= 0 || H <= 0 || lde < H)
        return fail(-1, "mxm_expand_tables: bad arguments");
    hipLaunchKernelGGL(expand_tables_kernel, dim3(clamp_grid(S, num_cu() * 8)), dim3(256), 0, (hipStream_t)stream, maj, mk_ptr, mk_hap,
                       mk_base, map256, (int)S, (int)H, lde, out);
    HIP_TRY(hipGetLastError());
    return 0;
}

extern "C" size_t mxm_quad_lists_scratch_bytes(int64_t R) {
    return R > 0 ? (size_t)((R + QLIST_CHUNK - 1) / QLIST_CHUNK) * 2 * sizeof(long long) : 0;
}

extern "C" int mxm_quad_lists(const int32_t *ndist, const int32_t *nquad, int64_t R, int64_t *quad_rows, int64_t *byte_rows,
                              int64_t *counts, void *scratch, size_t scratch_bytes, void *stream) {
    MXM_ENTER();
    if (ndist == nullptr || nquad == nullptr || R <= 0 || quad_rows == nullptr || byte_rows == nullptr || counts == nullptr)
        return fail(-1, "mxm_quad_lists: bad arguments");
    if (scratch == nullptr || scratch_bytes < mxm_quad_lists_scratch_bytes(R)) return fail(-1, "mxm_quad_lists: scratch too small");
    const int64_t nchunk = (R + QLIST_CHUNK - 1) / QLIST_CHUNK;
    if (nchunk > 0x7fffffff) return fail(-1, "mxm_quad_lists: too many rows");
    hipStream_t s = (hipStream_t)stream;
    long long *cc = static_cast<long long *>(scratch);
    hipLaunchKernelGGL(quad_list_count_kernel, dim3((unsigned)nchunk), dim3(QLIST_THREADS), 0, s, ndist, nquad, R, cc);
    hipLaunchKernelGGL(quad_list_scan_kernel, dim3(1), dim3(QLIST_THREADS), 0, s, cc, nchunk, reinterpret_cast<long long *>(counts));
    hipLaunchKernelGGL(quad_list_fill_kernel, dim3((unsigned)nchunk), dim3(QLIST_THREADS), 0, s, ndist, nquad, R, cc, quad_rows, byte_rows);
    HIP_TRY(hipGetLastError());
    return 0;
}

extern "C" int mxm_build_quads(const mxm_coded *c, int32_t H, uint8_t *qrec, size_t qrec_bytes, int64_t *qoff, int32_t *nquad,
                               uint64_t *stats, void *stream) {
    MXM_ENTER();
    if (c == nullptr || c->R <= 0 || c->rec == nullptr || c->rec_off == nullptr || c->ndist == nullptr || !mxm_linear_supported(H))
        return fail(-1, "mxm_build_quads: bad coded matrix (rows %lld, H %d)", (long long)(c ? c->R : 0), H);
    if (qoff == nullptr || nquad == nullptr || stats == nullptr || (qrec == nullptr && qrec_bytes > 0) ||
        (reinterpret_cast<uintptr_t>(qrec) & 31))
        return fail(-1, "mxm_build_quads: qoff, nquad, stats and a 32-byte aligned qrec required");
    const int ldc = coded_ld(H);
    if (ldc / 4 > 8 * QUAD_THREADS) return fail(-1, "mxm_build_quads: H=%d beyond eight quads per thread", H);
    HIP_TRY(hipMemsetAsync(stats, 0, 2 * sizeof(uint64_t), (hipStream_t)stream));
    if (T.quad_encoder == 1 && ldc / 4 <= 64 * QW_K)
        hipLaunchKernelGGL(quad_encode_wave_kernel, dim3(clamp_grid((c->R + QW_WAVES - 1) / QW_WAVES, std::min(num_cu() * QW_MIN_WAVES, 5120 / QW_WAVES))), dim3(QUAD_THREADS),
                           0, (hipStream_t)stream, c->rec, c->rec_off, c->ndist, ldc, (int)H, c->R, qrec,
                           (unsigned long long)qrec_bytes, qoff, nquad, reinterpret_cast<unsigned long long *>(stats));
    else
        hipLaunchKernelGGL(quad_encode_kernel, dim3(clamp_grid(c->R, num_cu() * 8)), dim3(QUAD_THREADS), 0, (hipStream_t)stream,
                           c->rec, c->rec_off, c->ndist, ldc, (int)H, c->R, qrec, (unsigned long long)qrec_bytes, qoff, nquad,
                           reinterpret_cast<unsigned long long *>(stats));
    HIP_TRY(hipGetLastError());
    return 0;
}

extern "C" int mxm_decode_rows(const mxm_coded *c, int32_t H, double *P, int64_t ldp, void *stream) {
    RC_TRY(coded_check(c, H, "mxm_decode_rows"));
    if (P == nullptr || ldp < H) return fail(-1, "mxm_decode_rows: ldp < H");
    hipLaunchKernelGGL(decode_rows_kernel, dim3(clamp_grid(c->R, num_cu() * 8)), dim3(256), 0, (hipStream_t)stream, c->rec,
                       c->rec_off, c->ndist, coded_ld(H), c->R, (int)H, P, ldp);
    HIP_TRY(hipGetLastError());
    return 0;
}

extern "C" int mxm_row_argmax_votes_coded(const mxm_coded *c, int32_t H, int32_t n_runs, const double *ln_props,
                                          const double *props, const double *rowmax, const double *M_rest, int64_t ldm_rest,
                                          const int64_t *rest_rows, int64_t n_rest, const double *w, int32_t *best,
                                          double *votes, void *ws, size_t ws_bytes, void *stream) {
    RC_TRY(coded_check(c, H, "mxm_row_argmax_votes_coded"));
    if (ln_props == nullptr || best == nullptr || n_runs < 1 || n_runs > RECK_MAX_RUNS)
        return fail(-1, "mxm_row_argmax_votes_coded: ln_props, best and 1..%d runs required", RECK_MAX_RUNS);
    if (n_runs > 1 && (props == nullptr || rowmax == nullptr))
        return fail(-1, "mxm_row_argmax_votes_coded: several runs need props and rowmax (each run's row normaliser)");
    RC_TRY(rest_check("mxm_row_argmax_votes_coded", H, M_rest, ldm_rest, rest_rows, n_rest));
    if (votes != nullptr && (ws == nullptr || ws_bytes < mxm_workspace_bytes(c->R, H, 1)))
        return fail(-1, "mxm_row_argmax_votes_coded: workspace too small");
    hipStream_t s = (hipStream_t)stream;
    const size_t lse_lds = (size_t)n_runs * sizeof(double);
    const int ldc_a = coded_ld(H);
    const int nch_a = (ldc_a / 4 + 255) / 256;
    const bool fast = n_runs == 1 && dispatch_width<8>(nch_a, [&](auto n) {
        constexpr int NCH = decltype(n)::value;
        int per_cu = 2;
        if (hipOccupancyMaxActiveBlocksPerMultiprocessor(&per_cu, records_argmax_narrow_kernel<NCH>, 256, 0) != hipSuccess || per_cu < 1) {
            (void)hipGetLastError();
            per_cu = 2;
        }
        hipLaunchKernelGGL((records_argmax_narrow_kernel<NCH>), dim3(clamp_grid(c->R, num_cu() * per_cu)), dim3(256), 0, s, c->rec,
                           c->rec_off, c->ndist, ldc_a, c->R, (int)H, ln_props, best);
        hipLaunchKernelGGL((records_argmax_kernel<NCH, true>), dim3(clamp_grid((c->R + 255) / 256, num_cu() * 2)), dim3(256), 0, s,
                           c->rec, c->rec_off, c->ndist, ldc_a, c->R, (int)H, ln_props, best, (const int64_t *)nullptr);
    });
    if (!fast)
        hipLaunchKernelGGL(posterior_argmax_kernel<true>, dim3(clamp_grid(c->R, num_cu() * 8)), dim3(256), lse_lds, s, c->rec, c->rec_off,
                           c->ndist, coded_ld(H), (const double *)nullptr, (int64_t)0, (const int64_t *)nullptr, c->R, (int)H,
                           (int)n_runs, ln_props, props, rowmax, best);
    HIP_TRY(hipGetLastError());
    if (n_rest > 0) {
        hipLaunchKernelGGL(posterior_argmax_kernel<false>, dim3(clamp_grid(n_rest, num_cu() * 8)), dim3(256), lse_lds, s,
                           (const uint8_t *)nullptr, (const int64_t *)nullptr, (const int32_t *)nullptr, 0, M_rest, ldm_rest,
                           rest_rows, n_rest, (int)H, (int)n_runs, ln_props, props, rowmax, best);
        HIP_TRY(hipGetLastError());
    }
    if (votes != nullptr) {
        const int64_t ldpart = part_ld(H);
        const int nwg = clamp_grid((c->R + 255) / 256, num_cu() * 2 < MXM_MAX_WG ? num_cu() * 2 : MXM_MAX_WG);
        const size_t vlds = (size_t)H * sizeof(double);
        RC_TRY(dynamic_lds_ok(reinterpret_cast<const void *>(&votes_from_best_kernel), vlds, "votes_from_best_kernel",
                              "mxm_row_argmax_votes_coded", H, "too wide for the vote kernel"));
        hipLaunchKernelGGL(votes_from_best_kernel, dim3(nwg), dim3(256), vlds, s, best, w, c->R, (int)H, (double *)ws, ldpart);
        HIP_TRY(hipGetLastError());
        return reduce_one((const double *)ws, nwg, (int)H, votes, nullptr, s);
    }
    return 0;
}

extern "C" int mxm_em_step_coded(const mxm_coded *c, int32_t H, const double *ln_props, const double *props,
                                 const double *rowmax, const double *M_rest, int64_t ldm_rest, const int64_t *rest_rows,
                                 int64_t n_rest, double *out, int64_t ldo, int32_t mode, void *stream) {
    RC_TRY(coded_check(c, H, "mxm_em_step_coded"));
    if (ln_props == nullptr || props == nullptr || rowmax == nullptr || out == nullptr || ldo < H)
        return fail(-1, "mxm_em_step_coded: bad arguments");
    RC_TRY(rest_check("mxm_em_step_coded", H, M_rest, ldm_rest, rest_rows, n_rest));
    hipLaunchKernelGGL(coded_posterior_kernel, dim3(clamp_grid(c->R, num_cu() * 8)), dim3(256), 0, (hipStream_t)stream, c->rec,
                       c->rec_off, c->ndist, coded_ld(H), c->R, (int)H, ln_props, props, rowmax, out, ldo, (int)mode);
    HIP_TRY(hipGetLastError());
    if (n_rest > 0) {
        const size_t lds = 2 * (size_t)H * sizeof(double);
        RC_TRY(dynamic_lds_ok(reinterpret_cast<const void *>(&estep_log_kernel<false>), lds, "estep_log_kernel", "mxm_em_step_coded", H,
                              "too large"));
        hipLaunchKernelGGL((estep_log_kernel<false>), dim3(clamp_grid(n_rest, num_cu() * 2)), dim3(ROW_THREADS), lds,
                           (hipStream_t)stream, M_rest, ldm_rest, (const double *)nullptr, ln_props, n_rest, (int)H, out, ldo,
                           (int)mode, (double *)nullptr, (int64_t)0, (const mxm_em_state *)nullptr, rest_rows);
        HIP_TRY(hipGetLastError());
    }
    return 0;
}

extern "C" int mxm_gather_columns_coded(const mxm_coded *c, int32_t H, const int32_t *cols, int32_t nC, const double *M_rest,
                                        int64_t ldm_rest, const int64_t *rest_rows, int64_t n_rest, double *out,
                                        int64_t ldo, void *stream) {
    RC_TRY(coded_check(c, H, "mxm_gather_columns_coded"));
    if (cols == nullptr || out == nullptr || nC <= 0 || ldo < nC) return fail(-1, "mxm_gather_columns_coded: bad arguments");
    RC_TRY(rest_check("mxm_gather_columns_coded", H, M_rest, ldm_rest, rest_rows, n_rest));
    const int64_t blocks = (c->R * nC + 255) / 256;
    hipLaunchKernelGGL(coded_gather_columns_kernel, dim3(clamp_grid(blocks, num_cu() * 16)), dim3(256), 0, (hipStream_t)stream,
                       c->rec, c->rec_off, c->ndist, coded_ld(H), c->R, cols, (int)nC, out, ldo);
    HIP_TRY(hipGetLastError());
    if (n_rest > 0) {
        hipLaunchKernelGGL(gather_columns_kernel, dim3(clamp_grid((n_rest * nC + 255) / 256, num_cu() * 16)), dim3(256), 0,
                           (hipStream_t)stream, M_rest, ldm_rest, n_rest, cols, (int)nC, out, ldo, rest_rows);
        HIP_TRY(hipGetLastError());
    }
    return 0;
}

struct coded_shape { int threads, nbuf, wg_per_cu; };
static const coded_shape g_coded_shapes[] = {{256, 4, 2}};
static const int g_coded_shape = 0;
template <int THREADS, int NBUF, int MINWG>
static int launch_coded(int nch, int nwg, hipStream_t stream, const mxm_coded *c, int ldc, const double *w, const double *props,
                        int H, double *partial, int64_t ldpart, const mxm_em_state *state, int run,
                        const int64_t *row_list = nullptr, int64_t n_list = 0, int part_row0 = 0) {
    bool launched = false;
    (void)dispatch_width<8>(nch, [&](auto n) {
        constexpr int NCH = decltype(n)::value;
        if constexpr (NCH * THREADS <= 2048) {
            hipLaunchKernelGGL((em_iter_coded_kernel<THREADS, NCH, NBUF, MINWG>), dim3(nwg), dim3(THREADS), 0, stream, c->rec, c->rec_off,
                               c->ndist, ldc, w, c->wide_rows, c->n_wide, props, c->R, H, partial, ldpart, state, run, row_list, n_list,
                               c->nquad, part_row0);
            launched = true;
        }
    });
    return launched ? 0 : fail(-1, "mxm_em_iter_coded: H=%d outside the kernel's range", H);
}
#define QUAD_MAX_NCH 6
static int quad_left_share(const mxm_coded *c, int slots) {
    if (c->n_byte_rows <= 0 && c->n_wide <= 0) return 0;
    const double left_cost = 1.0 * (double)c->n_byte_rows + 1.5 * (double)c->n_wide;
    const double quad_cost = 0.67 * (double)c->n_quad_rows;
    int n = (int)((double)slots * left_cost / (left_cost + quad_cost) + 0.5);
    if (T.quad_left_wg > 0) n = T.quad_left_wg;
    if (n < 4) n = 4;
    if (n > slots / 2) n = slots / 2;
    const int64_t left = c->n_byte_rows > c->n_wide ? c->n_byte_rows : c->n_wide;
    n = clamp_grid(left, n);
    return n < 1 ? 1 : n;
}
static int launch_quad(int nch, int nwg, hipStream_t stream, const mxm_coded *c, const double *w, const double *props, int H,
                       double *partial, int64_t ldpart, const mxm_em_state *state, int run) {
    const bool ok = dispatch_width<QUAD_MAX_NCH>(nch, [&](auto n) {
        hipLaunchKernelGGL((em_iter_quad_kernel<decltype(n)::value, 4>), dim3(nwg), dim3(QUAD_THREADS), 0, stream, c->qrec, c->qoff,
                           c->nquad, c->quad_rows, c->n_quad_rows, c->R, w, props, H, partial, ldpart, 0, state, run);
    });
    return ok ? 0 : fail(-1, "mxm_em_iter_coded: H=%d outside the quad kernel's range", H);
}
static int launch_quad_coded(int nch, int nwg, int nwg_left, hipStream_t stream, const mxm_coded *c, int ldc, const double *w,
                             const double *props, int H, double *partial, int64_t ldpart, const mxm_em_state *state, int run) {
    const int64_t *byte_rows = c->byte_rows != nullptr ? c->byte_rows : c->quad_rows;
    const bool ok = dispatch_width<QUAD_MAX_NCH>(nch, [&](auto n) {
        hipLaunchKernelGGL((em_iter_quad_coded_kernel<decltype(n)::value, 4>), dim3(nwg), dim3(QUAD_THREADS), 0, stream, c->rec,
                           c->rec_off, c->ndist, ldc, c->wide_rows, c->n_wide, byte_rows, c->n_byte_rows, c->qrec, c->qoff, c->nquad,
                           c->quad_rows, c->n_quad_rows, c->R, w, props, H, partial, ldpart, nwg_left, state, run);
    });
    return ok ? 0 : fail(-1, "mxm_em_iter_coded: H=%d outside the quad kernel's range", H);
}

static int em_iter_coded_one(const mxm_coded *c, const double *w, const double *props, int H, int run,
                             const mxm_em_state *state, double *colsum, double *partial, hipStream_t stream, bool timed,
                             const fin_args *fin = nullptr) {
    const int64_t ldpart = part_ld(H);
    const int ldc = coded_ld(H);
    const coded_shape sh = g_coded_shapes[g_coded_shape];
    const int nch = (ldc / 4 + sh.threads - 1) / sh.threads;
    int cap = num_cu() * sh.wg_per_cu;
    if (cap > MXM_MAX_WG - num_cu()) cap = MXM_MAX_WG - num_cu();
    if (cap < 1) cap = 1;
    const bool quads = c->qrec != nullptr && c->n_quad_rows > 0 && nch <= QUAD_MAX_NCH;
    int nwg_q = 0, nwg = 0;
    if (quads) {
        const int slots = cap < 2 * num_cu() ? cap : 2 * num_cu();
        const int nwg_b = quad_left_share(c, slots);
        nwg_q = clamp_grid((c->n_quad_rows + sh.nbuf - 1) / sh.nbuf, slots - nwg_b < 1 ? 1 : slots - nwg_b);
        nwg = nwg_q + nwg_b;
    } else {
        nwg = clamp_grid((c->R + sh.nbuf - 1) / sh.nbuf, cap);
    }
    if (timed && T.ev_start != nullptr) HIP_TRY(hipEventRecord(T.ev_start, stream));
    int *chk = reinterpret_cast<int *>(partial + (int64_t)MXM_MAX_WG * ldpart);
    int lrc;
    if (quads) {
        if (nwg > nwg_q) lrc = launch_quad_coded(nch, nwg, nwg - nwg_q, stream, c, ldc, w, props, H, partial, ldpart, state, run);
        else lrc = launch_quad(nch, nwg_q, stream, c, w, props, H, partial, ldpart, state, run);
        if (lrc != 0) return lrc;
    } else {
        lrc = launch_coded<256, 4, 2>(nch, nwg, stream, c, ldc, w, props, H, partial, ldpart, state, run);
        if (lrc != 0) return lrc;
    }
    HIP_TRY(hipGetLastError());
    if (timed && T.ev_stop != nullptr) HIP_TRY(hipEventRecord(T.ev_stop, stream));
    int nwg_rest = 0;
    mxm_slots sl;
    for (int i = 0; i < MXM_MAX_BT; ++i) sl.s[i] = run;
    if (c->R_rest > 0) {
        const int rc = stream_linear_tile(c->P_rest, c->ldp_rest, c->w_rest, props, c->R_rest, H, 1, sl, state,
                                          partial + (int64_t)nwg * ldpart, stream, false, &nwg_rest, MXM_MAX_WG - nwg,
                                          0 );
        if (rc != 0) return rc;
    }
    return reduce_tile(partial, nwg + nwg_rest, 1, H, colsum, state, sl, fin, stream, wide_check{chk, nwg, quads ? 0ll : (long long)c->n_wide});
}

#define QB_BT 3
static bool coded_batch_ok(const mxm_coded *c, int H) {
    if (T.coded_bt < QB_BT || c == nullptr || c->qrec == nullptr || c->n_quad_rows <= 0) return false;
    if (c->R_rest > 0 && !batch_fits(H, QB_BT)) return false;
    const int nch256 = (coded_ld(H) / 4 + QUAD_THREADS - 1) / QUAD_THREADS;
    return nch256 <= QUAD_MAX_NCH && mxm_linear_supported(H);
}
static int em_iter_coded_batched(const mxm_coded *c, const double *w, const double *props, int H, const mxm_slots &tile,
                                 const mxm_em_state *state, double *colsum, double *partial, hipStream_t stream, bool timed,
                                 const fin_args *fin = nullptr) {
    const int64_t ldpart = part_ld(H);
    const int ldc = coded_ld(H);
    const int nch = ((ldc / 4 + QUAD_THREADS - 1) / QUAD_THREADS + 1) / 2;
    int cap = num_cu();
    if (cap > MXM_MAX_WG / QB_BT - num_cu() / QB_BT) cap = MXM_MAX_WG / QB_BT - num_cu() / QB_BT;
    if (cap < 1) cap = 1;
    const int nwg = clamp_grid((c->n_quad_rows + 2) / 3, cap);
    mxm_slots sl = tile;
    for (int i = QB_BT; i < MXM_MAX_BT; ++i) sl.s[i] = sl.s[0];
    if (timed && T.ev_start != nullptr) HIP_TRY(hipEventRecord(T.ev_start, stream));
    const int64_t *byte_rows = c->byte_rows != nullptr ? c->byte_rows : c->quad_rows;
    const int64_t *wide_rows = c->wide_rows != nullptr ? c->wide_rows : c->quad_rows;
    const bool left = c->n_byte_rows > 0 || c->n_wide > 0;
    const bool ok = dispatch_width<3>(nch, [&](auto n) {
        constexpr int NCH = decltype(n)::value;
        auto pass = [&](auto kernel) {
            hipLaunchKernelGGL(kernel, dim3(nwg), dim3(QB_THREADS), 0, stream, c->rec, c->rec_off, c->ndist, ldc, wide_rows, c->n_wide,
                               byte_rows, c->n_byte_rows, c->qrec, c->qoff, c->nquad, c->quad_rows, c->n_quad_rows, c->R, w, props, H,
                               partial, ldpart, state, sl);
        };
        pass(em_iter_quad_batched_kernel<QB_BT, NCH, 1>);
        if (left) pass(em_iter_quad_batched_kernel<QB_BT, NCH, 6>);
    });
    if (!ok) return fail(-1, "mxm_em_iter_coded: H=%d outside the batched quad kernel's range", H);
    HIP_TRY(hipGetLastError());
    if (timed && T.ev_stop != nullptr) HIP_TRY(hipEventRecord(T.ev_stop, stream));
    int nwg_rest = 0;
    if (c->R_rest > 0) {
        const int rc = stream_linear_tile(c->P_rest, c->ldp_rest, c->w_rest, props, c->R_rest, H, QB_BT, sl, state,
                                          partial + (int64_t)nwg * QB_BT * ldpart, stream, false, &nwg_rest,
                                          (MXM_MAX_WG - nwg * QB_BT) / QB_BT);
        if (rc != 0) return rc;
    }
    int *chk = reinterpret_cast<int *>(partial + (int64_t)MXM_MAX_WG * ldpart);
    return reduce_tile(partial, nwg + nwg_rest, QB_BT, H, colsum, state, sl, fin, stream, wide_check{chk, nwg, 0ll});
}

extern "C" int mxm_em_iter_coded(const mxm_coded *c, const double *w, const double *props, int32_t H, int32_t B,
                                 mxm_em_state *state, double *colsum, void *ws, size_t ws_bytes, void *stream) {
    MXM_ENTER();
    RC_TRY(coded_check(c, H, "mxm_em_iter_coded"));
    if (B <= 0 || props == nullptr || colsum == nullptr) return fail(-1, "mxm_em_iter_coded: bad arguments");
    if (ws == nullptr || ws_bytes < mxm_workspace_bytes(c->R, H, B)) return fail(-1, "mxm_em_iter_coded: workspace too small");
    int b = 0;
    if (coded_batch_ok(c, (int)H)) {
        for (; b + QB_BT <= B; b += QB_BT) {
            RC_TRY(em_iter_coded_batched(c, w, props, (int)H, slots_from(b), state, colsum, (double *)ws, (hipStream_t)stream, b == 0));
        }
    }
    for (; b < B; ++b) {
        RC_TRY(em_iter_coded_one(c, w, props, (int)H, b, state, colsum, (double *)ws, (hipStream_t)stream, b == 0));
    }
    return 0;
}

extern "C" int mxm_restart_tile_coded(const mxm_coded *c, int32_t H) {
    MXM_ENTER();
    return coded_batch_ok(c, (int)H) ? QB_BT : 1;
}

extern "C" int mxm_restart_tile(int32_t H) {
    MXM_ENTER();
    if (!mxm_linear_supported(H)) return 1;
    int bt = T.max_bt;
    while (bt > 1 && !batch_fits((int)H, bt)) --bt;
    return bt;
}

extern "C" int mxm_m_finalize(const double *colsum, double *ln_cur, double *ln_new, double *props_cur, int32_t H,
                              int32_t B, double tol, int32_t max_iter, mxm_em_state *state, void *stream) {
    if (H <= 0 || B <= 0 || state == nullptr) return fail(-1, "mxm_m_finalize: bad arguments");
    if (H > 64 * FIN_MAX_BLOCKS) {
        hipLaunchKernelGGL(finalize_any_kernel, dim3(1, B), dim3(FIN_THREADS), 0, (hipStream_t)stream, colsum, ln_cur, ln_new,
                           props_cur, (int)H, tol, (int)max_iter, state, 0, 0, slots_from(0));
        HIP_TRY(hipGetLastError());
        return 0;
    }
    hipLaunchKernelGGL(finalize_kernel, dim3((H + FIN_THREADS - 1) / FIN_THREADS, B), dim3(FIN_THREADS), 0, (hipStream_t)stream,
                       colsum, ln_cur, ln_new, props_cur, (int)H, tol, (int)max_iter, state, 0, 0, slots_from(0));
    HIP_TRY(hipGetLastError());
    return 0;
}

extern "C" int mxm_set_loop_graph(int32_t mode) {
    return tune_set([mode](mxm_tuning &t) { t.loop_graph = mode < 0 ? -1 : (mode > 0 ? 1 : 0); });
}

extern "C" int mxm_set_progress_callback(mxm_progress_fn fn, void *user, int32_t every) {
    return tune_set([=](mxm_tuning &t) { t.progress = fn; t.progress_user = user; t.progress_every = every > 0 ? every : 10; });
}

extern "C" int mxm_set_loop_fused(int32_t mode, int32_t chunk) {
    return tune_set([=](mxm_tuning &t) {
        t.loop_fused = mode < 0 ? -1 : (mode > 0 ? 1 : 0);
        t.fused_cols = (mode == 2) ? 0 : 1;
        t.fused_chunk = chunk > 0 ? chunk : 0;
    });
}

static bool fused_cols_eligible(int64_t R, int H, int nwg) {
    if (!T.fused_cols || nwg != 256) return false;
    if (R > (int64_t)FCOLS_MAX_RPT * FCOLS_THREADS || (R + nwg - 1) / nwg > 2 * FCOLS_NQ) return false;
    const int cp = (H + nwg - 1) / nwg;
    if (cp > FCOLS_MAX_CP) return false;
    return cp <= 22 || R <= 2 * (int64_t)FCOLS_THREADS;
}
static bool fused_cols_fits(int64_t R, int H, int B, int nwg, size_t ws_bytes) {
    return ws_bytes >= fused_sync_bytes() + fused_cols_bytes(R, nwg) + fused_snapshot_bytes(H, B) + 256;
}

static bool fused_eligible(const double *P, int64_t ldp, int64_t R, int H, int B, size_t ws_bytes, bool p_is_f32, int running) {
    if (T.loop_fused == 0 || p_is_f32 || P == nullptr || !mxm_linear_supported(H)) return false;
    if ((ldp & 1) || (reinterpret_cast<uintptr_t>(P) & 15)) return false;
    int nwg = num_cu() < MXM_MAX_WG ? num_cu() : MXM_MAX_WG;
    const int ncol2 = (H + 1) / 2;
    if ((ncol2 + nwg - 1) / nwg > 16 * FUSED_MAX_M) return false;
    if ((ncol2 + FUSED_THREADS - 1) / FUSED_THREADS > FUSED_MAX_NCH) return false;
    if ((int64_t)nwg * part_ld(H) * 8 >= ((int64_t)1 << 31)) return false;
    if (ws_bytes < fused_sync_bytes() + fused_rows_bytes(H, nwg) + fused_snapshot_bytes(H, B) + 256) return false;
    if (T.loop_fused == 1) return true;
    if (running <= 3 && fused_cols_eligible(R, H, nwg) && fused_cols_fits(R, H, B, nwg, ws_bytes)) return true;
    return running <= 1 && (double)R * (double)H <= T.fused_cells;
}

static int fused_coded_grid(int64_t R) {
    int nwg = num_cu() * 2 < MXM_MAX_WG ? num_cu() * 2 : MXM_MAX_WG;
    if (T.fused_coded_wg > 0) {
        if (T.fused_coded_wg < nwg) nwg = T.fused_coded_wg;
    } else {
        const int best = ((int)(5.2 * sqrt((double)R)) + 7) & ~7;
        if (best < nwg) nwg = best;
    }
    if ((int64_t)nwg > R) nwg = (int)R;
    return nwg < 1 ? 1 : nwg;
}
#define QUAD_PER_ITER_MIN_ROWS 300000
#define QUAD_BATCH_MIN_ROWS 15000
extern "C" int64_t mxm_quad_loop_min_rows(int32_t B) { return B >= 3 ? QUAD_BATCH_MIN_ROWS : QUAD_PER_ITER_MIN_ROWS; }
static bool fused_coded_eligible(const mxm_coded *c, int H, int B, size_t ws_bytes, int running = 1) {
    if (T.loop_fused == 0 || c == nullptr || c->R_rest > 0 || !mxm_linear_supported(H) || (H & 1)) return false;
    if (c->qrec != nullptr && c->n_quad_rows >= QUAD_PER_ITER_MIN_ROWS && T.loop_fused != 1 &&
        (coded_ld(H) / 4 + QUAD_THREADS - 1) / QUAD_THREADS <= QUAD_MAX_NCH)
        return false;
    if (running >= 3 && T.loop_fused != 1 && c->n_quad_rows >= QUAD_BATCH_MIN_ROWS && coded_batch_ok(c, H)) return false;
    const int nwg = fused_coded_grid(c->R);
    const int ncol2 = H / 2;
    if ((ncol2 + nwg - 1) / nwg > 16 * FCODED_MAX_M) return false;
    if ((coded_ld(H) / 4 + FCODED_THREADS - 1) / FCODED_THREADS > 8) return false;
    if ((int64_t)nwg * part_ld(H) * 8 >= ((int64_t)1 << 31)) return false;
    return ws_bytes >= fused_sync_bytes() + fused_rows_bytes(H, nwg) + fused_snapshot_bytes(H, B) + 256;
}

extern "C" int mxm_diag_fused_stamps(const void *ws, unsigned long long *out_host) {
    if (ws == nullptr || out_host == nullptr) return fail(-1, "mxm_diag_fused_stamps: bad arguments");
    const fused_sync *sync = reinterpret_cast<const fused_sync *>(ws);
    HIP_TRY(hipMemcpy(out_host, sync->stamps, sizeof(sync->stamps), hipMemcpyDeviceToHost));
    return 0;
}

template <typename K>
static bool grid_fits(K kernel, int threads, int nwg) {
    int per_cu = 0;
    if (hipOccupancyMaxActiveBlocksPerMultiprocessor(&per_cu, kernel, threads, 0) != hipSuccess) {
        (void)hipGetLastError();
        return false;
    }
    return (long long)per_cu * num_cu() >= nwg;
}

template <int CP, int RPT>
static bool launch_fused_cols(int nwg, hipStream_t s, const double *P, int64_t ldp, const double *w, int64_t R, int H,
                              int B, double *ln_cur, double *ln_new, double *props_cur, mxm_em_state *state, double tol,
                              int max_iter, int chunk, double *zpart, int64_t ldz, double *cbuf, double *l1part,
                              fused_sync *sync) {
    if (!grid_fits(em_fused_cols_kernel<CP, RPT>, FCOLS_THREADS, nwg)) return false;
    hipLaunchKernelGGL((em_fused_cols_kernel<CP, RPT>), dim3(nwg), dim3(FCOLS_THREADS), 0, s, P, ldp, w, R, H, B, ln_cur,
                       ln_new, props_cur, state, tol, max_iter, chunk, zpart, ldz, cbuf, l1part, sync);
    return true;
}

template <int NCH>
static bool launch_fused(int nwg, hipStream_t s, const double *P, int64_t ldp, const double *w, int64_t R, int H, int B,
                         double *ln_cur, double *ln_new, double *props_cur, mxm_em_state *state, double tol,
                         int max_iter, int chunk, double *partial, int64_t ldpart, double *tbuf, fused_sync *sync) {
    if (!grid_fits(em_fused_loop_kernel<NCH, FUSED_NBUF>, FUSED_THREADS, nwg)) return false;
    hipLaunchKernelGGL((em_fused_loop_kernel<NCH, FUSED_NBUF>), dim3(nwg), dim3(FUSED_THREADS), 0, s, P, ldp, w, R, H, B, ln_cur,
                       ln_new, props_cur, state, tol, max_iter, chunk, partial, ldpart, tbuf, sync);
    return true;
}

template <int NCH>
static bool launch_fused_coded(int nwg, bool resident, hipStream_t s, const mxm_coded *c, int ldc, const double *w, int H, int B,
                               double *ln_cur, double *ln_new, double *props_cur, mxm_em_state *state, double tol,
                               int max_iter, int chunk, double *partial, int64_t ldpart, double *tbuf, fused_sync *sync) {
    if constexpr (NCH * FCODED_THREADS > 2048) {
        return false;
    } else {
        fcoded_args a;
        a.partial = partial; a.tbuf = tbuf; a.ln_cur = ln_cur; a.ln_new = ln_new; a.props_cur = props_cur;
        a.state = state; a.sync = sync; a.ldpart = ldpart; a.tol = tol; a.max_iter = max_iter; a.H = H;
        if (resident) {
            if (!grid_fits(em_fused_coded_kernel<NCH, 4, true>, FCODED_THREADS, nwg)) return false;
            hipLaunchKernelGGL((em_fused_coded_kernel<NCH, 4, true>), dim3(nwg), dim3(FCODED_THREADS), 0, s, c->rec, c->rec_off,
                               c->ndist, ldc, w, c->wide_rows, c->n_wide, c->R, B, chunk, a);
        } else {
            if (!grid_fits(em_fused_coded_kernel<NCH, 4, false>, FCODED_THREADS, nwg)) return false;
            hipLaunchKernelGGL((em_fused_coded_kernel<NCH, 4, false>), dim3(nwg), dim3(FCODED_THREADS), 0, s, c->rec, c->rec_off,
                               c->ndist, ldc, w, c->wide_rows, c->n_wide, c->R, B, chunk, a);
        }
        return true;
    }
}

static int fused_narrow_grid(int64_t R, int H, int *rpt_out) {
    if (H < 1 || H > 16 || R < 1) return 0;
    const int hmax = H <= 4 ? 4 : (H <= 8 ? 8 : 16);
    int cap = num_cu() < FNARROW_MAX_WG ? num_cu() : FNARROW_MAX_WG;
    const int nwg = clamp_grid((R + FNARROW_THREADS - 1) / FNARROW_THREADS, cap);
    const int64_t per = (R + (int64_t)nwg * FNARROW_THREADS - 1) / ((int64_t)nwg * FNARROW_THREADS);
    int rpt = 1;
    while (rpt < per) rpt *= 2;
    if (rpt * hmax > FNARROW_MAX_CELLS || (hmax == 16 && rpt > 1)) return 0;
    *rpt_out = rpt;
    return nwg;
}
static size_t fused_narrow_bytes(int H, int nwg) { return (size_t)2 * H * ((nwg + 7) & ~7) * sizeof(double); }

template <int HMAX, int RPT>
static bool launch_fused_narrow_one(int nwg, hipStream_t s, const double *M, int64_t ldm, const double *w, int64_t R, int H, int B,
                                    double *ln_cur, double *ln_new, double *props_cur, mxm_em_state *state, double tol,
                                    int max_iter, int chunk, double *partial, fused_sync *sync) {
    if constexpr (HMAX * RPT > FNARROW_MAX_CELLS || (HMAX == 16 && RPT > 1)) {
        return false;
    } else {
        if (!grid_fits(em_fused_narrow_kernel<HMAX, RPT>, FNARROW_THREADS, nwg)) return false;
        hipLaunchKernelGGL((em_fused_narrow_kernel<HMAX, RPT>), dim3(nwg), dim3(FNARROW_THREADS), 0, s, M, ldm, w, R, H, B, ln_cur,
                           ln_new, props_cur, state, tol, max_iter, chunk, partial, (nwg + 7) & ~7, sync);
        return true;
    }
}
static bool launch_fused_narrow(int nwg, int rpt, hipStream_t s, const double *M, int64_t ldm, const double *w, int64_t R, int H,
                                int B, double *ln_cur, double *ln_new, double *props_cur, mxm_em_state *state, double tol,
                                int max_iter, int chunk, double *partial, fused_sync *sync) {
    bool fits = false;
    auto columns = [&](auto hmax) {
        (void)dispatch_width<8>(rpt, [&](auto k) {
            constexpr int HMAX = decltype(hmax)::value, RPT = decltype(k)::value;
            if constexpr ((RPT & (RPT - 1)) == 0)
                fits = launch_fused_narrow_one<HMAX, RPT>(nwg, s, M, ldm, w, R, H, B, ln_cur, ln_new, props_cur, state, tol, max_iter,
                                                          chunk, partial, sync);
        });
    };
    if (H <= 4) columns(std::integral_constant<int, 4>{});
    else if (H <= 8) columns(std::integral_constant<int, 8>{});
    else columns(std::integral_constant<int, 16>{});
    return fits;
}

enum class fused_route { none, records, narrow, dense };
struct fused_matrix {
    fused_route route;
    const mxm_coded *coded;
    const double *M;
    int64_t ldm;
    const double *P;
    int64_t ldp;
};

static int read_state(mxm_em_state *state_host, const mxm_em_state *state, int n, hipStream_t s) {
    HIP_TRY(hipMemcpyAsync(state_host, state, sizeof(mxm_em_state) * n, hipMemcpyDeviceToHost, s));
    HIP_TRY(hipStreamSynchronize(s));
    return 0;
}

#define MXM_FUSED_GAVE_UP 1
static int em_loop_fused(const fused_matrix &m, const double *w, int64_t R, int32_t H, int32_t B, double *props_cur,
                         double *ln_cur, double *ln_new, mxm_em_state *state, double tol, int32_t max_iter, int32_t chunk,
                         void *ws, size_t ws_bytes, hipStream_t s, mxm_em_state *state_host) {
    const mxm_coded *coded = m.coded;
    const double *P = m.P;
    const int64_t ldp = m.ldp;
    static std::mutex one_loop_at_a_time;
    std::lock_guard<std::mutex> guard(one_loop_at_a_time);
    int narrow_rpt = 1;
    const int nwg = m.route == fused_route::narrow    ? fused_narrow_grid(R, (int)H, &narrow_rpt)
                    : m.route == fused_route::records ? fused_coded_grid(coded->R)
                                                      : (num_cu() < MXM_MAX_WG ? num_cu() : MXM_MAX_WG);
    const int64_t ldpart = part_ld(H);
    char *base = static_cast<char *>(ws);
    fused_sync *sync = reinterpret_cast<fused_sync *>(base);
    double *tbuf = reinterpret_cast<double *>(base + fused_sync_bytes());
    double *partial = tbuf + 2 * ldpart;
    const int nch = ((H + 1) / 2 + FUSED_THREADS - 1) / FUSED_THREADS;
    const size_t vec = (size_t)B * H * sizeof(double);
    char *snap = base + ((ws_bytes - fused_snapshot_bytes(H, B)) & ~(size_t)255);
    auto snapshot = [&](bool save) -> hipError_t {
        double *vecs[3] = {props_cur, ln_cur, ln_new};
        for (int i = 0; i < 3; ++i) {
            const hipError_t e = save ? hipMemcpyAsync(snap + i * vec, vecs[i], vec, hipMemcpyDeviceToDevice, s)
                                      : hipMemcpyAsync(vecs[i], snap + i * vec, vec, hipMemcpyDeviceToDevice, s);
            if (e != hipSuccess) return e;
        }
        return save ? hipMemcpyAsync(snap + 3 * vec, state, sizeof(mxm_em_state) * B, hipMemcpyDeviceToDevice, s)
                    : hipMemcpyAsync(state, snap + 3 * vec, sizeof(mxm_em_state) * B, hipMemcpyDeviceToDevice, s);
    };
    if (chunk < 1) chunk = 1;
    bool launched_once = false;
    for (;;) {
        RC_TRY(read_state(state_host, state, B, s));
        bool all_done = true, gave_up = false;
        for (int b = 0; b < B; ++b) {
            gave_up = gave_up || state_host[b].done < 0;
            all_done = all_done && state_host[b].done != 0;
        }
        if (gave_up) {
            HIP_TRY(snapshot(false));
            RC_TRY(read_state(state_host, state, B, s));
            fail(-3, "mxm_em_loop: the one-launch loop's grid barrier timed out: not all %d workgroups became resident "
                     "(is another process or stream using the GPU?)", nwg);
            return MXM_FUSED_GAVE_UP;
        }
        if (launched_once && T.progress != nullptr) T.progress(state_host, B, T.progress_user);
        if (all_done) return 0;
        HIP_TRY(snapshot(true));
        HIP_TRY(hipMemsetAsync(sync, 0, fused_sync_bytes(), s));
        if (T.fused_force_abort)
            HIP_TRY(hipMemsetAsync(&sync->abort_[0], 1, sizeof(unsigned), s));
        bool fits = true;
        if (m.route == fused_route::narrow) {
            fits = launch_fused_narrow(nwg, narrow_rpt, s, m.M, m.ldm, w, R, (int)H, (int)B, ln_cur, ln_new, props_cur,
                                       state, tol, (int)max_iter, (int)chunk, reinterpret_cast<double *>(base + fused_sync_bytes()), sync);
        } else if (m.route == fused_route::records) {
            const int ldc = coded_ld(H);
            const int cnch = (ldc / 4 + FCODED_THREADS - 1) / FCODED_THREADS;
            const bool resident = (coded->R + nwg - 1) / nwg <= FCODED_THREADS && (coded->n_wide + nwg - 1) / nwg <= FCODED_THREADS;
            const bool ok = dispatch_width<8>(cnch, [&](auto n) {
                fits = launch_fused_coded<decltype(n)::value>(nwg, resident, s, coded, ldc, w, (int)H, (int)B, ln_cur, ln_new, props_cur,
                                                              state, tol, (int)max_iter, (int)chunk, partial, ldpart, tbuf, sync);
            });
            if (!ok) return fail(-1, "mxm_em_loop_coded: H=%d outside the one-launch loop's range", H);
        } else if (fused_cols_eligible(R, (int)H, nwg) && fused_cols_fits(R, (int)H, (int)B, nwg, ws_bytes)) {
            const int64_t ldz = (R + 1) & ~(int64_t)1;
            double *zpart = reinterpret_cast<double *>(base + fused_sync_bytes());
            double *cbuf = zpart + (int64_t)nwg * ldz;
            double *l1part = cbuf + ldz;
            const int cp = ((int)H + nwg - 1) / nwg;
            const int rpt = (int)((R + FCOLS_THREADS - 1) / FCOLS_THREADS);
            auto columns = [&](auto cpmax) {
                constexpr int CP = decltype(cpmax)::value, MAX_RPT = CP == 24 ? 2 : 3;
                (void)dispatch_width<MAX_RPT>(rpt < 1 ? 1 : (rpt > MAX_RPT ? MAX_RPT : rpt), [&](auto k) {
                    fits = launch_fused_cols<CP, decltype(k)::value>(nwg, s, P, ldp, w, R, (int)H, (int)B, ln_cur, ln_new, props_cur, state,
                                                                    tol, (int)max_iter, (int)chunk, zpart, ldz, cbuf, l1part, sync);
                });
            };
            if (cp <= 12) columns(std::integral_constant<int, 12>{});
            else if (cp <= 22) columns(std::integral_constant<int, 22>{});
            else columns(std::integral_constant<int, 24>{});
        } else {
            const bool ok = dispatch_width<FUSED_MAX_NCH>(nch, [&](auto n) {
                fits = launch_fused<decltype(n)::value>(nwg, s, P, ldp, w, R, (int)H, (int)B, ln_cur, ln_new, props_cur, state, tol,
                                                        (int)max_iter, (int)chunk, partial, ldpart, tbuf, sync);
            });
            if (!ok) return fail(-1, "mxm_em_loop: H=%d outside the one-launch loop's range", H);
        }
        if (!fits) {
            fail(-3, "mxm_em_loop: the one-launch loop's %d workgroups cannot be co-resident on this device", nwg);
            return MXM_FUSED_GAVE_UP;
        }
        HIP_TRY(hipGetLastError());
        launched_once = true;
    }
}

static int enqueue_tile_iteration(const double *M, int64_t ldm, const double *P, int64_t ldp, const double *w,
                                  int64_t R, int32_t H, const mxm_slots &tile, int nb, double *props_cur,
                                  double *ln_cur, double *ln_new, double *colsum, mxm_em_state *state, double tol,
                                  int32_t max_iter, void *ws, size_t ws_bytes, hipStream_t s, bool p_is_f32,
                                  bool timed, const mxm_coded *coded) {
    const bool linear = !p_is_f32 && P != nullptr && mxm_linear_supported(H);
    fin_args fin = {ln_cur, ln_new, props_cur, state, tol, (int)max_iter};
    if (coded != nullptr) {
        if (nb == QB_BT && coded_batch_ok(coded, (int)H))
            return em_iter_coded_batched(coded, w, props_cur, (int)H, tile, state, colsum, (double *)ws, s, timed, &fin);
        for (int i = 0; i < nb; ++i) {
            RC_TRY(em_iter_coded_one(coded, w, props_cur, (int)H, tile.s[i], state, colsum, (double *)ws, s, timed && i == 0, &fin));
        }
        return 0;
    } else if (linear) {
        return em_iter_linear_tile(P, ldp, w, props_cur, R, (int)H, nb, tile, state, colsum, (double *)ws, s, timed, &fin);
    } else {
        for (int i = 0; i < nb; ++i) {
            const int64_t off = (int64_t)tile.s[i] * H;
            const int rc = p_is_f32 ? mxm_em_iter_f32(reinterpret_cast<const float *>(P), ldp, w, props_cur + off, R, H, 1,
                                                      state + tile.s[i], colsum + off, ws, ws_bytes, s)
                                    : mxm_em_iter(M, ldm, P, ldp, w, props_cur + off, ln_cur + off, R, H, 1,
                                                  state + tile.s[i], colsum + off, ws, ws_bytes, s);
            if (rc != 0) return rc;
        }
    }
    if (H > 64 * FIN_MAX_BLOCKS)
        hipLaunchKernelGGL(finalize_any_kernel, dim3(1, nb), dim3(FIN_THREADS), 0, s, colsum, ln_cur, ln_new, props_cur, (int)H, tol,
                           (int)max_iter, state, 0, 1, tile);
    else
        hipLaunchKernelGGL(finalize_kernel, dim3((H + FIN_THREADS - 1) / FIN_THREADS, nb), dim3(FIN_THREADS), 0, s, colsum, ln_cur,
                           ln_new, props_cur, (int)H, tol, (int)max_iter, state, 0, 1, tile);
    HIP_TRY(hipGetLastError());
    return 0;
}

static int records_lists_check(const mxm_coded *c, const char *who, void *scratch, hipStream_t s, bool with_quads) {
    unsigned long long *chk = static_cast<unsigned long long *>(scratch), host[2] = {0, 0};
    const dim3 grid(clamp_grid((c->R + 255) / 256, num_cu() * 4));
    auto faults_of = [&](auto launch) -> int {
        HIP_TRY(hipMemsetAsync(chk, 0, sizeof(host), s));
        launch();
        HIP_TRY(hipGetLastError());
        HIP_TRY(hipMemcpyAsync(host, chk, sizeof(host), hipMemcpyDeviceToHost, s));
        HIP_TRY(hipStreamSynchronize(s));
        return 0;
    };
    RC_TRY(faults_of([&] {
        hipLaunchKernelGGL(coded_validate_kernel, grid, dim3(256), 0, s, c->ndist, c->R, c->wide_rows, c->n_wide, chk);
    }));
    if (host[1] != 0 || (long long)host[0] != (long long)c->n_wide)
        return fail(-1, "%s: wide_rows must list exactly the rows with more than 256 values, ascending (%lld such rows, n_wide = %lld)",
                    who, (long long)host[0], (long long)c->n_wide);
    if (!with_quads) return 0;
    RC_TRY(faults_of([&] {
        hipLaunchKernelGGL(quad_validate_kernel, grid, dim3(256), 0, s, c->ndist, c->nquad, c->R, c->quad_rows, c->n_quad_rows,
                           c->byte_rows, c->n_byte_rows, chk);
    }));
    if (host[1] != 0) return fail(-1, "%s: quad_rows / byte_rows must list the rows with / without quads, ascending", who);
    return 0;
}

struct loop_resources {
    hipStream_t s = nullptr;
    hipEvent_t ev = nullptr;
    hipGraph_t graph = nullptr;
    hipGraphExec_t exec = nullptr;
    loop_resources() = default;
    loop_resources(const loop_resources &) = delete;
    loop_resources &operator=(const loop_resources &) = delete;
// ... 1027 lines not shown
```

mixemt_amd/em.py:

```python

import ctypes
import math
import os
import sys
import time

import numpy

from . import _lib
from ._dev import as_device, current_stream, device_empty, ptr, require_gpu, to_host, torch


def init_props(nhaps, alpha=1.0):
    if alpha == float("inf"):
        return numpy.array([1.0 / nhaps] * nhaps)
    return numpy.random.dirichlet([alpha] * nhaps)


def converged(prop, last_prop, tolerance=0.0001):
    lib = _lib.load()
    dev = require_gpu()
    a = as_device(prop, torch.float64, dev)
    b = as_device(last_prop, torch.float64, dev)
    if a.numel() != b.numel():
        raise ValueError("operands could not be broadcast together")
    out = torch.empty(1, dtype=torch.float64, device=dev)
    _lib.check(lib.mxm_l1_exp_diff(a.data_ptr(), b.data_ptr(), a.numel(), out.data_ptr(),
                                   current_stream()), "mxm_l1_exp_diff")
    return bool(out.item() < tolerance)


def _workspace(lib, n_rows, n_haps, n_runs, dev):
    nbytes = lib.mxm_workspace_bytes(n_rows, n_haps, n_runs)
    return torch.empty(nbytes // 8 + 1, dtype=torch.float64, device=dev), nbytes


def em_step(read_hap_mat, weights, ln_props, read_mix_mat):
    lib = _lib.load()
    dev = require_gpu()
    on_host = not isinstance(read_hap_mat, torch.Tensor)
    mat = as_device(read_hap_mat, torch.float64, dev)
    n_rows, n_haps = mat.shape
    wts = as_device(weights, torch.float64, dev)
    lnp = as_device(ln_props, torch.float64, dev)
    if wts.numel() != n_rows or lnp.numel() != n_haps:
        raise ValueError("em_step: weights/ln_props do not match the matrix shape")
    if on_host:
        out = torch.empty_like(mat)
    else:
        out = read_mix_mat
        if out.shape != mat.shape or out.dtype != torch.float64 or out.stride(1) != 1:
            raise ValueError("em_step: read_mix_mat must be a float64 matrix like read_hap_mat")
    colsum = torch.empty(n_haps, dtype=torch.float64, device=dev)
    ln_new = torch.empty(n_haps, dtype=torch.float64, device=dev)
    ws, ws_bytes = _workspace(lib, n_rows, n_haps, 1, dev)
    stream = current_stream()
    _lib.check(lib.mxm_em_step(mat.data_ptr(), mat.stride(0), wts.data_ptr(), lnp.data_ptr(),
                               n_rows, n_haps, out.data_ptr(), out.stride(0), 0,
                               colsum.data_ptr(), ws.data_ptr(), ws_bytes, stream),
               "mxm_em_step")
    _lib.check(lib.mxm_log_normalize(colsum.data_ptr(), n_haps, ln_new.data_ptr(), stream),
               "mxm_log_normalize")
    if on_host:
        read_mix_mat[...] = to_host(out)
        return read_mix_mat, ln_new.cpu().numpy()
    return out, ln_new


AUTO_CODED_MIN_CELLS = 1.5e7
QUADS = {"off": False, "0": False, "on": True, "1": True}.get(os.environ.get("MXM_QUADS", "auto").strip().lower(), "auto")
QUADS_MIN_ROWS = 300000
QUADS_MIN_ROWS_MULTI = 20000
QUADS_MAX_FOOTPRINT = 60e9
AUTO_CODED_MIN_CELLS_MULTI = 5e7
AUTO_CODED_MAX_REST = 0.25


class EmPlan(object):

    def __init__(self, read_hap_mat, weights, n_runs=1, keep_log_matrix=True, storage="f64", records=None):
        if records is not None:
            self._from_records(records, read_hap_mat, weights, n_runs)
            return
        if storage not in ("f64", "f32", "coded", "auto"):
            raise ValueError("storage must be 'f64', 'f32', 'coded' or 'auto'")
        self.storage = storage
        self.lib = _lib.load()
        self.dev = require_gpu()
        self.mat = as_device(read_hap_mat, torch.float64, self.dev)
        if self.mat.dim() != 2:
            raise ValueError("read_hap_mat must be 2-D")
        self.n_rows, self.n_haps = self.mat.shape
        self.wts = as_device(weights, torch.float64, self.dev)
        if self.wts.numel() != self.n_rows:
            raise ValueError("weights do not match the matrix height")
        self.n_runs = n_runs
        self.ws, self.ws_bytes = _workspace(self.lib, self.n_rows, self.n_haps, n_runs, self.dev)
        self.lin = None
        self.rowmax = None
        self.coded = None
        auto = storage == "auto"
        if auto:
            floor = AUTO_CODED_MIN_CELLS if n_runs <= 1 else AUTO_CODED_MIN_CELLS_MULTI
            storage = "coded" if (float(self.n_rows) * self.n_haps > floor) else "f64"
            self.storage = storage
        if storage == "coded":
            if self.n_rows > 0 and self.lib.mxm_linear_supported(self.n_haps) and self.mat.stride(1) == 1:
                self.encode()
                if auto and self.coded_rest > AUTO_CODED_MAX_REST * self.n_rows:
                    self.coded = None
                    self._coded_keep = self.coded_ndist = None
            if self.coded is None:
                self.storage = storage = "f64"
        if self.coded is not None:
            pass
        elif self.lib.mxm_linear_supported(self.n_haps) and self.n_rows > 0:
            self.rowmax = torch.empty(self.n_rows, dtype=torch.float64, device=self.dev)
            if storage == "f32":
                ldp = (self.n_haps + 3) // 4 * 4
                self.lin = device_empty((self.n_rows, ldp), torch.float32, self.dev, "the linearised matrix")
                _lib.check(self.lib.mxm_linearize_f32(self.mat.data_ptr(), self.mat.stride(0),
                                                      self.n_rows, self.n_haps, self.lin.data_ptr(),
                                                      self.lin.stride(0), self.rowmax.data_ptr(),
                                                      current_stream()), "mxm_linearize_f32")
            else:
                ldp = (self.n_haps + 1) // 2 * 2
                self.lin = device_empty((self.n_rows, ldp), torch.float64, self.dev, "the linearised matrix")
                _lib.check(self.lib.mxm_linearize(self.mat.data_ptr(), self.mat.stride(0),
                                                  self.n_rows, self.n_haps, self.lin.data_ptr(),
                                                  self.lin.stride(0), self.rowmax.data_ptr(),
                                                  current_stream()), "mxm_linearize")
        elif storage == "f32":
            self.storage = "f64"
        if not keep_log_matrix and (self.lin is not None or self.coded is not None):
            self.mat = None

    def _from_records(self, cm, read_hap_mat, weights, n_runs):
        self.storage = "coded"
        self.lib = _lib.load()
        self.dev = require_gpu()
        self.n_rows, self.n_haps = cm.n_rows, cm.n_haps
        self.mat = None if read_hap_mat is None else as_device(read_hap_mat, torch.float64, self.dev)
        if self.mat is not None and tuple(self.mat.shape) != (self.n_rows, self.n_haps):
            raise ValueError("read_hap_mat does not match the records")
        self.wts = as_device(weights, torch.float64, self.dev)
        if self.wts.numel() != self.n_rows:
            raise ValueError("weights do not match the matrix height")
        self.n_runs = n_runs
        self.ws, self.ws_bytes = _workspace(self.lib, self.n_rows, self.n_haps, n_runs, self.dev)
        self.lin = None
        self.rowmax = cm.rowmax
        n_rest = int(cm.rest_rows.numel())
        p_rest = w_rest = None
        if n_rest:
            ldp = (self.n_haps + 1) // 2 * 2
            p_rest = torch.empty((n_rest, ldp), dtype=torch.float64, device=self.dev)
            rm = torch.empty(n_rest, dtype=torch.float64, device=self.dev)
            _lib.check(self.lib.mxm_linearize(cm.m_rest.data_ptr(), cm.m_rest.stride(0), n_rest, self.n_haps,
                                              p_rest.data_ptr(), p_rest.stride(0), rm.data_ptr(), current_stream()),
                       "mxm_linearize")
            if self.n_rows < 2 ** 31:
                cols = torch.from_numpy(cm.rest_rows.cpu().numpy().astype(numpy.int32)).to(self.dev)
                w_rest = torch.empty(n_rest, dtype=torch.float64, device=self.dev)
                _lib.check(self.lib.mxm_gather_columns(self.wts.data_ptr(), self.n_rows, 1, self.n_rows, cols.data_ptr(), n_rest,
                                                       w_rest.data_ptr(), n_rest, current_stream()), "mxm_gather_columns")
            else:
                w_rest = self.wts.index_select(0, cm.rest_rows).contiguous()
        self.coded_record_bytes = cm.used - 8 * int(cm.ndist_host().sum(dtype=numpy.int64))
        self.coded_bytes = self.coded_record_bytes + n_rest * self.n_haps * 8
        self.coded_rest = n_rest
        self.coded_ndist = cm.ndist
        wide = cm.wide_rows()
        self.coded_wide = int(wide.numel())
        self._coded_keep = (cm.rec, cm.rec_off, cm.ndist, p_rest, w_rest, cm, wide)
        self.records = cm
        self.coded = _lib.Coded(cm.rec.data_ptr(), cm.rec_off.data_ptr(), cm.ndist.data_ptr(), self.n_rows,
                                p_rest.data_ptr() if n_rest else None, p_rest.stride(0) if n_rest else 0,
                                w_rest.data_ptr() if n_rest else None, n_rest,
                                wide.data_ptr() if self.coded_wide else None, self.coded_wide)
        self._quad_keep = None
        self.attach_quads()

    def attach_quads(self, mode=None, cap=None, min_rows=None):
        mode = QUADS if mode is None else mode
        if self.coded is None or mode is False or self._quad_keep is not None:
            return self._quad_keep is not None
        lib, dev = self.lib, self.dev
        rec, rec_off, ndist = self._coded_keep[:3]
        nd_h = self.records.ndist_host() if getattr(self, "records", None) is not None else ndist.cpu().numpy()
        byte_coded = (nd_h > 0) & (nd_h <= 256)
        n_byte = int(byte_coded.sum())
        ldc = (self.n_haps + 7) // 8 * 8
        if n_byte == 0 or ldc // 4 > 6 * 256:
            return False
        per_row = int(min(256, max(112, 2.3 * float(nd_h[byte_coded].mean()) + 12)))
        guess = n_byte * (2048 + 32 * per_row) + min(self.n_rows, 5120) * 65536 + (1 << 20)
        if mode == "auto":
            floor_ok = n_byte >= (min_rows if min_rows is not None else
                                  (QUADS_MIN_ROWS_MULTI if getattr(self, "n_runs", 1) >= 3 else QUADS_MIN_ROWS))
            if not floor_ok or int(rec.numel()) + guess > QUADS_MAX_FOOTPRINT:
                return False
        n_rows = self.n_rows
        laps = {} if os.environ.get("MXM_PIPELINE_TIMING") else None
        self.quad_laps = laps
        t_lap = [time.perf_counter()]

        def lap(name):
            if laps is not None:
                torch.cuda.synchronize()
                laps[name] = round(laps.get(name, 0.0) + (time.perf_counter() - t_lap[0]) * 1e3, 2)
                t_lap[0] = time.perf_counter()

        qoff = torch.empty(n_rows, dtype=torch.int64, device=dev)
        nquad = torch.empty(n_rows, dtype=torch.int32, device=dev)
        stats = torch.empty(2, dtype=torch.int64, device=dev)
        cap = guess if cap is None else max(32, int(cap) // 32 * 32)
        for attempt in (0, 1):
            try:
                qrec = device_empty((cap,), torch.uint8, dev, "the quad dictionary")
            except ValueError:
                if mode == "auto":
                    return False
                raise
            lap("buffers")
            _lib.check(lib.mxm_build_quads(ctypes.byref(self.coded), self.n_haps, qrec.data_ptr(), qrec.numel(), qoff.data_ptr(),
                                           nquad.data_ptr(), stats.data_ptr(), current_stream()), "mxm_build_quads")
            used, n_left = (int(v) for v in stats.cpu())
            lap("quad_encode_kernel")
            if used <= cap:
                break
            if attempt == 1:
                raise ValueError("mxm_build_quads: buffer of %d bytes overflowed (%d needed)" % (cap, used))
            del qrec
            cap = (used + (256 << 20) + 31) // 32 * 32
        quad_rows_d = torch.empty(n_rows, dtype=torch.int64, device=dev)
        byte_rows_d = torch.empty(n_rows, dtype=torch.int64, device=dev)
        counts = torch.empty(2, dtype=torch.int64, device=dev)
        sbytes = lib.mxm_quad_lists_scratch_bytes(n_rows)
        scratch = torch.empty(max(1, (sbytes + 7) // 8), dtype=torch.int64, device=dev)
        _lib.check(lib.mxm_quad_lists(ndist.data_ptr(), nquad.data_ptr(), n_rows, quad_rows_d.data_ptr(), byte_rows_d.data_ptr(),
                                      counts.data_ptr(), scratch.data_ptr(), scratch.numel() * 8, current_stream()), "mxm_quad_lists")
        n_quad, n_byte_left = (int(v) for v in counts.cpu())
        lap("row lists (device)")
        if n_quad == 0:
            return False
        if mode == "auto" and min_rows is None and n_quad < int(lib.mxm_quad_loop_min_rows(int(getattr(self, "n_runs", 1)))):
            return False
        quad_rows_d, byte_rows_d = quad_rows_d[:n_quad], byte_rows_d[:n_byte_left]
        self._quad_keep = (qrec, qoff, nquad, quad_rows_d, byte_rows_d)
        self.coded.qrec, self.coded.qoff, self.coded.nquad = qrec.data_ptr(), qoff.data_ptr(), nquad.data_ptr()
        self.coded.quad_rows, self.coded.n_quad_rows = quad_rows_d.data_ptr(), n_quad
        self.coded.byte_rows, self.coded.n_byte_rows = (byte_rows_d.data_ptr() if n_byte_left else None), n_byte_left
        if laps is not None:
            laps["quads per row (room for / used, table entries)"] = "%d / %.1f, %.1f" % (
                per_row, (used / max(1, n_quad) - 2048) / 32.0, float(nd_h[byte_coded].mean()))
            sys.stderr.write("[attach_quads] %s\n" % laps)
        self.quad_rows_n = n_quad
        rest_bytes = self.coded_rest * self.n_haps * 8

        def account():
            nq_h = nquad.cpu().numpy()
            left = byte_coded & (nq_h == 0)
            wide_h = nd_h > 256
            rec_left = int((ldc + 8 * nd_h[left].astype(numpy.int64)).sum() + (2 * ldc + 8 * nd_h[wide_h].astype(numpy.int64)).sum())
            quad_exact = int((2048 + 32 * nq_h[nq_h > 0].astype(numpy.int64)).sum())
            return {"quad_bytes": quad_exact, "coded_record_bytes": quad_exact + rec_left,
                    "coded_bytes": quad_exact + rec_left + rest_bytes}

        self._accounting = account
        for name in ("quad_bytes", "coded_record_bytes", "coded_bytes"):
            self.__dict__.pop(name, None)
        return True

    def __getattr__(self, name):
        if name in ("quad_bytes", "coded_record_bytes", "coded_bytes"):
            account = self.__dict__.get("_accounting")
            if account is not None:
                self.__dict__.update(account())
                self.__dict__["_accounting"] = None
                return self.__dict__[name]
        raise AttributeError(name)

    def encode(self):
        lib, dev, n_rows, n_haps = self.lib, self.dev, self.n_rows, self.n_haps
        ldc = (n_haps + 7) // 8 * 8
        one = 2 * ldc + 16 * 1024
        if self.coded is not None:
            rec, rec_off, ndist = self._coded_keep[:3]
            cap = rec.numel()
        else:
            cap = max(one, min(lib.mxm_coded_bytes(n_rows, n_haps), n_rows * (ldc + 16 * 96) + (1 << 20)))
            rec = device_empty((cap,), torch.uint8, dev, "the coded matrix")
            rec_off = torch.empty(n_rows, dtype=torch.int64, device=dev)
            ndist = torch.empty(n_rows, dtype=torch.int32, device=dev)
            self.rowmax = torch.empty(n_rows, dtype=torch.float64, device=dev)
        stats = torch.zeros(2, dtype=torch.int64, device=dev)
        for attempt in (0, 1):
            _lib.check(lib.mxm_encode_rows(self.mat.data_ptr(), self.mat.stride(0), n_rows, n_haps, rec.data_ptr(), cap,
                                           rec_off.data_ptr(), ndist.data_ptr(), self.rowmax.data_ptr(), stats.data_ptr(),
                                           current_stream()), "mxm_encode_rows")
            used, n_rest = (int(v) for v in stats.cpu())
            if used <= cap:
                break
            if attempt == 1:
                raise ValueError("mxm_encode_rows: record buffer of %d bytes overflowed (%d needed)" % (cap, used))
            del rec
            cap = max(one, used)
            rec = device_empty((cap,), torch.uint8, dev, "the coded matrix")
        p_rest = w_rest = None
        if n_rest:
            idx = torch.nonzero(ndist == 0).flatten()
            m_rest = self.mat.index_select(0, idx)
            ldp = (n_haps + 1) // 2 * 2
            p_rest = torch.empty((n_rest, ldp), dtype=torch.float64, device=dev)
            rm = torch.empty(n_rest, dtype=torch.float64, device=dev)
            _lib.check(lib.mxm_linearize(m_rest.data_ptr(), m_rest.stride(0), n_rest, n_haps, p_rest.data_ptr(),
                                         p_rest.stride(0), rm.data_ptr(), current_stream()), "mxm_linearize")
            w_rest = self.wts.index_select(0, idx).contiguous()
        self.coded_record_bytes = used - 8 * int(ndist.sum().item())
        self.coded_bytes = self.coded_record_bytes + (n_rest * n_haps * 8)
        self.coded_rest = n_rest
        wide = torch.nonzero(ndist > 256).flatten()
        self.coded_wide = int(wide.numel())
        self._coded_keep = (rec, rec_off, ndist, p_rest, w_rest, wide)
        self.coded_ndist = ndist
        self.coded = _lib.Coded(rec.data_ptr(), rec_off.data_ptr(), ndist.data_ptr(), n_rows,
                                p_rest.data_ptr() if n_rest else None, p_rest.stride(0) if n_rest else 0,
                                w_rest.data_ptr() if n_rest else None, n_rest,
                                wide.data_ptr() if self.coded_wide else None, self.coded_wide)
        self._quad_keep = None
        self.attach_quads()

    def mat_args(self):
        if self.mat is None:
            return 0, 0
        return self.mat.data_ptr(), self.mat.stride(0)

    def lin_args(self):
        if self.lin is None:
            return 0, 0
        return self.lin.data_ptr(), self.lin.stride(0)

    def release_linear(self):
        lin = self.lin
        if lin is None or lin.dtype != torch.float64 or lin.stride(0) != self.n_haps:
            return None
        self.lin = None
        self.spent = True
        return lin

    def restart_tile(self):
        if self.coded is not None:
            return int(self.lib.mxm_restart_tile_coded(ctypes.byref(self.coded), self.n_haps))
        if self.lin is None or self.storage != "f64":
            return 1
        return int(self.lib.mxm_restart_tile(self.n_haps))

    def alloc_props(self, host):
        return torch.from_numpy(numpy.ascontiguousarray(host, dtype=numpy.float64)).to(self.dev)

    def alloc_state(self, n_runs):
        return new_state(n_runs, self.dev)

    def read_state(self, state):
        return read_state(state)

    def em_iter(self, props, ln_props, state, colsum):
        if getattr(self, "spent", False):
            raise ValueError("this plan's linearised matrix has been released (release_linear)")
        m_ptr, ldm = self.mat_args()
        p_ptr, ldp = self.lin_args()
        if self.coded is not None:
            _lib.check(self.lib.mxm_em_iter_coded(ctypes.byref(self.coded), self.wts.data_ptr(), props.data_ptr(),
                                                  self.n_haps, props.shape[0], ptr(state), colsum.data_ptr(),
                                                  self.ws.data_ptr(), self.ws_bytes, current_stream()),
                       "mxm_em_iter_coded")
            return
        if self.storage == "f32":
            _lib.check(self.lib.mxm_em_iter_f32(p_ptr, ldp, self.wts.data_ptr(), props.data_ptr(),
                                                self.n_rows, self.n_haps, props.shape[0], ptr(state),
                                                colsum.data_ptr(), self.ws.data_ptr(), self.ws_bytes,
                                                current_stream()), "mxm_em_iter_f32")
            return
        _lib.check(self.lib.mxm_em_iter(m_ptr, ldm, p_ptr, ldp, self.wts.data_ptr(),
                                        props.data_ptr(), ln_props.data_ptr(), self.n_rows,
                                        self.n_haps, props.shape[0], ptr(state), colsum.data_ptr(),
                                        self.ws.data_ptr(), self.ws_bytes, current_stream()),
                   "mxm_em_iter")

    def finalize(self, colsum, ln_cur, ln_new, props_cur, state, tol, max_iter):
        _lib.check(self.lib.mxm_m_finalize(colsum.data_ptr(), ln_cur.data_ptr(), ln_new.data_ptr(),
                                           props_cur.data_ptr(), self.n_haps, props_cur.shape[0],
                                           float(tol), int(max_iter), state.data_ptr(),
                                           current_stream()), "mxm_m_finalize")


def new_state(n_runs, dev):
    return torch.zeros(n_runs * (ctypes.sizeof(_lib.EmState) // 8), dtype=torch.int64, device=dev)


def read_state(state):
    raw = state.cpu().numpy().tobytes()
    n = len(raw) // ctypes.sizeof(_lib.EmState)
    arr = (_lib.EmState * n).from_buffer_copy(raw)
    if any(s.error == 2 for s in arr):
        raise ValueError("EM loop state: the one-shot exchange timed out waiting for a rank (mxm_exchange_pull poisoned the sums)")
    if any(s.error for s in arr):
        raise ValueError("EM loop state: the records' wide_rows list does not match the rows with more than 256 values "
                         "(mxm_em_iter_coded poisoned the sums)")
    return [(s.done, s.iters, s.l1) for s in arr]


def log_inits(inits):
    with numpy.errstate(divide="ignore"):
        ln0 = numpy.log(numpy.ascontiguousarray(inits, dtype=numpy.float64))
    return ln0, numpy.exp(ln0)


def em_loop(plan, inits, tolerance, max_iter, check_every=16):
    lib, dev = plan.lib, plan.dev
    if getattr(plan, "spent", False):
        raise ValueError("this plan's linearised matrix has been released (release_linear)")
    ln0, p0 = log_inits(inits)
    n_runs, n_haps = ln0.shape
    props_cur = torch.from_numpy(p0).to(dev)
    ln_cur = torch.from_numpy(ln0).to(dev)
    ln_new = ln_cur.clone()
    colsum = torch.zeros_like(props_cur)
    state = new_state(n_runs, dev)
    host_state = (_lib.EmState * n_runs)()
    if max_iter > 0 and plan.coded is not None:
        _lib.check(lib.mxm_em_loop_coded(ctypes.byref(plan.coded), plan.wts.data_ptr(), n_haps, n_runs,
                                         props_cur.data_ptr(), ln_cur.data_ptr(), ln_new.data_ptr(),
                                         colsum.data_ptr(), state.data_ptr(), float(tolerance),
                                         int(max_iter), int(check_every), plan.ws.data_ptr(),
                                         plan.ws_bytes, current_stream(), host_state), "mxm_em_loop_coded")
    elif max_iter > 0 and plan.storage == "f32":
        p_ptr, ldp = plan.lin_args()
        _lib.check(lib.mxm_em_loop_f32(p_ptr, ldp, plan.wts.data_ptr(), plan.n_rows, n_haps, n_runs,
                                       props_cur.data_ptr(), ln_cur.data_ptr(), ln_new.data_ptr(),
                                       colsum.data_ptr(), state.data_ptr(), float(tolerance),
                                       int(max_iter), int(check_every), plan.ws.data_ptr(),
                                       plan.ws_bytes, current_stream(), host_state), "mxm_em_loop_f32")
    elif max_iter > 0:
        m_ptr, ldm = plan.mat_args()
        p_ptr, ldp = plan.lin_args()
        _lib.check(lib.mxm_em_loop(m_ptr, ldm, p_ptr, ldp, plan.wts.data_ptr(), plan.n_rows,
                                   n_haps, n_runs, props_cur.data_ptr(), ln_cur.data_ptr(),
                                   ln_new.data_ptr(), colsum.data_ptr(), state.data_ptr(),
                                   float(tolerance), int(max_iter), int(check_every),
                                   plan.ws.data_ptr(), plan.ws_bytes, current_stream(), host_state),
                   "mxm_em_loop")
    states = [(s.done, s.iters, s.l1) for s in host_state]
    return ln_cur, ln_new, states


def posterior(plan, ln_theta, out=None, fold=False):
    lnp = as_device(ln_theta, torch.float64, plan.dev)
    if out is None:
        out = device_empty((plan.n_rows, plan.n_haps), torch.float64, plan.dev, "the posterior matrix")
    if plan.mat is None and getattr(plan, "records", None) is not None:
        cm = plan.records
        lnp = lnp.reshape(-1).contiguous()
        coded = cm.struct()
        props_d = torch.exp(lnp)
        n_rest = int(cm.rest_rows.numel())
        _lib.check(plan.lib.mxm_em_step_coded(ctypes.byref(coded), plan.n_haps, lnp.data_ptr(), props_d.data_ptr(),
                                              cm.rowmax.data_ptr(), cm.m_rest.data_ptr() if n_rest else 0,
                                              cm.m_rest.stride(0) if n_rest else 0,
                                              cm.rest_rows.data_ptr() if n_rest else 0, n_rest,
                                              out.data_ptr(), out.stride(0), 1 if fold else 0,
                                              current_stream()), "mxm_em_step_coded")
        return out
    if plan.mat is None:
        raise ValueError("posterior pass needs the log matrix (keep_log_matrix=True)")
    _lib.check(plan.lib.mxm_em_step(plan.mat.data_ptr(), plan.mat.stride(0), 0, lnp.data_ptr(),
                                    plan.n_rows, plan.n_haps, out.data_ptr(), out.stride(0),
                                    1 if fold else 0, 0, 0, 0, current_stream()),
               "mxm_em_step")
    return out


class RecordsPosterior(object):

    def __init__(self, cm, ln_theta_k):
        self.cm, self.rec = cm, cm.rec
        self.ln_theta_k = numpy.atleast_2d(numpy.asarray(ln_theta_k, dtype=numpy.float64))
        self.shape = (cm.n_rows, cm.n_haps)

    def dense(self, lo=0, hi=None):
        import types
        part = self.cm.rows(lo, self.cm.n_rows if hi is None else hi)
        lib = _lib.load()
        shim = types.SimpleNamespace(dev=self.rec.device, n_rows=part.n_rows, n_haps=self.cm.n_haps, mat=None,
                                     records=part, lib=lib)
        out = device_empty((part.n_rows, self.cm.n_haps), torch.float64, self.rec.device, "rows of the posterior matrix")
        if part.n_rows == 0:
            return out
        n_multi = self.ln_theta_k.shape[0]
        for run in range(n_multi):
            posterior(shim, self.ln_theta_k[run], out=out, fold=(run > 0))
        if n_multi > 1:
            _lib.check(lib.mxm_add_scalar(out.data_ptr(), out.stride(0), part.n_rows, self.cm.n_haps,
                                          -math.log(n_multi), current_stream()), "mxm_add_scalar")
        return out


def collect_result(plan, inits, ln_cur, ln_new, states, want_read_mix=True, verbose=False,
                   reuse_linear=False):
    n_multi, n_haps = inits.shape
    ln_k = ln_cur.cpu().numpy()
    ln_next = ln_new.cpu().numpy()
    if verbose:
        for run, (done, iters, _) in enumerate(states):
            sys.stderr.write("Starting EM run %d...\n" % (run + 1))
            sys.stderr.write("." * (iters // 10))
            if done == 1:
                sys.stderr.write("\nConverged! (%d)\n" % iters)
    read_mix = None
    if want_read_mix:
        if reuse_linear and plan.mat is not None:
            read_mix = plan.release_linear()
        for run in range(n_multi):
            read_mix = posterior(plan, ln_k[run], out=read_mix, fold=(run > 0))
        if n_multi > 1:
            _lib.check(plan.lib.mxm_add_scalar(read_mix.data_ptr(), read_mix.stride(0),
                                               plan.n_rows, n_haps, -math.log(n_multi),
                                               current_stream()), "mxm_add_scalar")
    res = ln_next[0].copy()
    if n_multi > 1:
        for run in range(1, n_multi):
            res += ln_next[run]
        res /= n_multi
    props = numpy.exp(res)
    return {"props": props, "read_mix": read_mix, "iters": [s[1] for s in states],
            "done": [s[0] for s in states], "run_props": numpy.exp(ln_next), "inits": inits,
            "l1": [s[2] for s in states], "ln_theta_k": ln_k}


def run_em_ex(read_hap_mat, weights, args, inits=None, want_read_mix=True, storage=None, records=None):
    n_multi = int(args.n_multi)
    storage = storage or getattr(args, "storage", "auto")
    t_plan = time.perf_counter()
    plan = EmPlan(read_hap_mat, weights, n_runs=n_multi, storage=storage, records=records)
    torch.cuda.synchronize()
    t_plan = time.perf_counter() - t_plan
    if inits is None:
        inits = numpy.stack([init_props(plan.n_haps, alpha=args.init_alpha)
                             for _ in range(n_multi)])
    inits = numpy.ascontiguousarray(inits, dtype=numpy.float64)
    verbose = getattr(args, "verbose", False)
    t_loop = time.perf_counter()
    if verbose:
        report = {"run": 0, "dots": 0, "open": False}

        def tell(iters_done, n_runs):
            while report["run"] < n_runs:
                run = report["run"]
                iters, done = iters_done[run]
                if not report["open"]:
                    sys.stderr.write("Starting EM run %d...\n" % (run + 1))
                    report["open"], report["dots"] = True, 0
                dots = iters // 10 - report["dots"]
                if dots > 0:
                    sys.stderr.write("." * dots)
                    report["dots"] += dots
                if done == 0:
                    break
                if done == 1:
                    sys.stderr.write("\nConverged! (%d)\n" % iters)
                report["run"], report["open"] = run + 1, False
            sys.stderr.flush()

        def on_state(state_host, n_runs, _user):
            tell([(state_host[i].iters, state_host[i].done) for i in range(n_runs)], n_runs)
        hook = _lib.PROGRESS_FN(on_state)
        try:
            plan.lib.mxm_set_progress_callback(ctypes.cast(hook, ctypes.c_void_p), None, 10)
            ln_cur, ln_new, states = em_loop(plan, inits, args.tolerance, args.max_iter)
        finally:
            plan.lib.mxm_set_progress_callback(None, None, 10)
        tell([(st[1], st[0]) for st in states], n_multi)
    else:
        ln_cur, ln_new, states = em_loop(plan, inits, args.tolerance, args.max_iter)
    t_loop = time.perf_counter() - t_loop
    res = collect_result(plan, inits, ln_cur, ln_new, states, want_read_mix, False, reuse_linear=True)
    res["plan_s"], res["loop_s"], res["storage"] = t_plan, t_loop, plan.storage
    return res


class SampleBatch(object):

    def __init__(self, rec, rec_off, ndist, wts, row0, n_haps):
        self.lib = _lib.load()
        self.dev = rec.device
        self.rec, self.rec_off, self.ndist, self.wts = rec, rec_off.contiguous(), ndist.contiguous(), wts.contiguous()
        self.row0 = numpy.ascontiguousarray(row0, dtype=numpy.int64)
        self.n_entries, self.n_rows, self.n_haps = len(self.row0) - 1, int(self.row0[-1]), int(n_haps)
        if self.rec_off.numel() != self.n_rows or self.ndist.numel() != self.n_rows or self.wts.numel() != self.n_rows:
            raise ValueError("rec_off / ndist / weights do not match row0")
        nd_h = self.ndist.cpu().numpy()
        self.wide = torch.from_numpy(numpy.flatnonzero(nd_h > 256)).to(self.dev)
        n_wide = int(self.wide.numel())
        self.coded = _lib.Coded(self.rec.data_ptr(), self.rec_off.data_ptr(), self.ndist.data_ptr(), self.n_rows,
                                None, 0, None, 0, self.wide.data_ptr() if n_wide else None, n_wide)
        self.row0_ptr = self.row0.ctypes.data_as(ctypes.c_void_p)
        self.n_tiles = int(self.lib.mxm_samples_plan(self.row0_ptr, self.n_entries, None, 0, None))
        if self.n_tiles < 0:
            raise ValueError("mxm_samples_plan failed: %s" % self.lib.mxm_last_error().decode("utf-8", "replace"))
        self.ws_bytes = int(self.lib.mxm_samples_workspace_bytes(self.n_tiles, self.n_entries, self.n_haps))
        self.ws = device_empty((self.ws_bytes // 8 + 1,), torch.float64, self.dev, "the batched loop's workspace")

    def em_iter(self, props, state, colsum):
        _lib.check(self.lib.mxm_em_iter_samples(ctypes.byref(self.coded), self.row0_ptr, self.n_entries, self.wts.data_ptr(),
                                                props.data_ptr(), self.n_haps, ptr(state), colsum.data_ptr(),
                                                self.ws.data_ptr(), self.ws_bytes, current_stream()), "mxm_em_iter_samples")

    def em_loop(self, inits, tolerance, max_iter, check_every=16):
        ln0, p0 = log_inits(inits)
        if ln0.shape != (self.n_entries, self.n_haps):
            raise ValueError("inits must be [%d][%d]" % (self.n_entries, self.n_haps))
        props_cur = torch.from_numpy(p0).to(self.dev)
        ln_cur = torch.from_numpy(ln0).to(self.dev)
        ln_new = ln_cur.clone()
        colsum = torch.zeros_like(props_cur)
        state = new_state(self.n_entries, self.dev)
        host_state = (_lib.EmState * self.n_entries)()
        _lib.check(self.lib.mxm_em_loop_samples(ctypes.byref(self.coded), self.row0_ptr, self.n_entries, self.wts.data_ptr(),
                                                self.n_haps, props_cur.data_ptr(), ln_cur.data_ptr(), ln_new.data_ptr(),
                                                colsum.data_ptr(), state.data_ptr(), float(tolerance), int(max_iter),
                                                int(check_every), self.ws.data_ptr(), self.ws_bytes, current_stream(),
                                                host_state), "mxm_em_loop_samples")
        return ln_cur, ln_new, [(s.done, s.iters, s.l1) for s in host_state]
# ... 194 lines not shown
```

Before: 865.6 billion.

## Group rows with shared column-equivalence classes into precomputed class tables for EM

Adds a class-based encoding. Rows whose non-majority column sets hash to the same key are sorted into runs and chunked. Within each chunk, columns with identical code patterns across all rows are merged into equivalence classes, and per-chunk class tables are built so the EM step can work over classes instead of every haplotype column. Remaining rows go through the existing quad and byte paths. This adds build-time hashing and sorting, more device memory for directories and tables, a per-slot loop instead of batched iterations when classes are in use, and possible hash-collision risk in the class assignment.

```diff
diff --git a/include/mixemt_hip.h b/include/mixemt_hip.h
--- a/include/mixemt_hip.h
+++ b/include/mixemt_hip.h
@@ -104,6 +104,7 @@
     int64_t        n_quad_rows;
     const int64_t *byte_rows;
     int64_t        n_byte_rows;
+    const struct mxm_classes *classes;
 } mxm_coded;
 size_t mxm_coded_bytes(int64_t R, int32_t H);
 size_t mxm_quad_bytes(int64_t R, int32_t H);
diff --git a/include/mixemt_hip_classes.h b/include/mixemt_hip_classes.h
--- /dev/null
+++ b/include/mixemt_hip_classes.h
@@ -0,0 +1,39 @@
+#ifndef MIXEMT_HIP_CLASSES_H
+#define MIXEMT_HIP_CLASSES_H
+
+#include "mixemt_hip.h"
+
+#ifdef __cplusplus
+extern "C" {
+#endif
+
+typedef struct mxm_classes {
+    int64_t        n_chunks;
+    const int64_t *chunk_ptr;
+    const int64_t *rows;
+    int64_t        n_member;
+    const uint8_t *cdir;
+    const int32_t *ncls;
+    const int64_t *tab_off;
+    const double  *tab;
+    int64_t        tab_len;
+    const int64_t *left_quad_rows;
+    int64_t        n_left_quad;
+    const int64_t *left_byte_rows;
+    int64_t        n_left_byte;
+} mxm_classes;
+int mxm_class_keys(const mxm_coded *c, int32_t H, int64_t *keys, void *stream);
+size_t mxm_class_bytes(int64_t n_chunks, int32_t H);
+int mxm_build_classes(const mxm_coded *c, int32_t H, const int64_t *rows, const int64_t *chunk_ptr, int64_t n_chunks,
+                      uint8_t *cdir, size_t cdir_bytes, int32_t *ncls, void *stream);
+int mxm_build_class_tables(const mxm_coded *c, int32_t H, const int64_t *rows, const int64_t *chunk_ptr, int64_t n_chunks,
+                           const uint8_t *cdir, const int32_t *ncls, const int64_t *tab_off, double *tab, int64_t tab_len,
+                           int64_t *rows_out, uint8_t *in_class, void *stream);
+
+int mxm_set_class_form(int32_t mode, int32_t hash_rows);
+
+#ifdef __cplusplus
+}
+#endif
+
+#endif
diff --git a/mixemt_amd/_lib.py b/mixemt_amd/_lib.py
--- a/mixemt_amd/_lib.py
+++ b/mixemt_amd/_lib.py
@@ -18,7 +18,14 @@
                 ("P_rest", c_ptr), ("ldp_rest", c_i64), ("w_rest", c_ptr), ("R_rest", c_i64),
                 ("wide_rows", c_ptr), ("n_wide", c_i64),
                 ("qrec", c_ptr), ("qoff", c_ptr), ("nquad", c_ptr), ("quad_rows", c_ptr), ("n_quad_rows", c_i64),
-                ("byte_rows", c_ptr), ("n_byte_rows", c_i64)]
+                ("byte_rows", c_ptr), ("n_byte_rows", c_i64),
+                ("classes", c_ptr)]
+
+
+class Classes(ctypes.Structure):
+    _fields_ = [("n_chunks", c_i64), ("chunk_ptr", c_ptr), ("rows", c_ptr), ("n_member", c_i64), ("cdir", c_ptr), ("ncls", c_ptr),
+                ("tab_off", c_ptr), ("tab", c_ptr), ("tab_len", c_i64), ("left_quad_rows", c_ptr), ("n_left_quad", c_i64),
+                ("left_byte_rows", c_ptr), ("n_left_byte", c_i64)]
 
 
 class SampleTile(ctypes.Structure):
@@ -186,6 +193,15 @@
                                                   c_ptr, c_i32, c_f64, c_f64, c_f64, c_i32, c_i32, c_ptr, c_ptr, c_ptr, c_ptr]),
 }
 
+CLASS_SIGNATURES = {
+    "mxm_class_keys": (ctypes.c_int, [ctypes.POINTER(Coded), c_i32, c_ptr, c_ptr]),
+    "mxm_class_bytes": (c_size, [c_i64, c_i32]),
+    "mxm_build_classes": (ctypes.c_int, [ctypes.POINTER(Coded), c_i32, c_ptr, c_ptr, c_i64, c_ptr, c_size, c_ptr, c_ptr]),
+    "mxm_build_class_tables": (ctypes.c_int, [ctypes.POINTER(Coded), c_i32, c_ptr, c_ptr, c_i64, c_ptr, c_ptr, c_ptr, c_ptr, c_i64,
+                                              c_ptr, c_ptr, c_ptr]),
+    "mxm_set_class_form": (ctypes.c_int, [c_i32, c_i32]),
+}
+
 ABI_VERSION = 603
 
 PROGRESS_FN = ctypes.CFUNCTYPE(None, ctypes.POINTER(EmState), c_i32, c_ptr)
@@ -217,7 +233,7 @@
         raise MixemtHipError("%s reports ABI version %s, this binding was written for %d: rebuild with "
                              "`python -m mixemt_amd.build --force`" % (LIB_PATH, have, ABI_VERSION))
     for name, (restype, argtypes) in (list(SIGNATURES.items()) + list(FINISH_SIGNATURES.items())
-                                      + list(VARCHECK_SIGNATURES.items())):
+                                      + list(VARCHECK_SIGNATURES.items()) + list(CLASS_SIGNATURES.items())):
         try:
             fn = getattr(lib, name)
         except AttributeError:
diff --git a/mixemt_amd/build.py b/mixemt_amd/build.py
--- a/mixemt_amd/build.py
+++ b/mixemt_amd/build.py
@@ -9,7 +9,7 @@
 _ROOT = os.path.dirname(_PKG)
 SRC = os.path.join(_PKG, "csrc", "mixemt_hip.hip")
 HDRS = [os.path.join(_ROOT, "include", name) for name in ("mixemt_hip.h", "mixemt_hip_tuning.h", "mixemt_hip_samples_finish.h",
-                                                           "mixemt_hip_var_check.h")]
+                                                           "mixemt_hip_var_check.h", "mixemt_hip_classes.h")]
 LIB_DIR = os.path.join(_PKG, "lib")
 LIB = os.path.join(LIB_DIR, "libmixemt_hip.so")
 ARCH = "gfx950"
diff --git a/mixemt_amd/csrc/class_kernels.hpp b/mixemt_amd/csrc/class_kernels.hpp
--- /dev/null
+++ b/mixemt_amd/csrc/class_kernels.hpp
@@ -0,0 +1,528 @@
+#ifndef MIXEMT_CLASS_KERNELS_HPP
+#define MIXEMT_CLASS_KERNELS_HPP
+
+#define CLS_THREADS 256
+#define CLS_MAX 1024
+#define CLS_MAX_ROWS 256
+#define CLS_HASH 2048
+#define CLS_CPTR 1032
+#define CLS_MAX_LDC 6144
+#define CLS_BIG 64
+
+__host__ __device__ __forceinline__ size_t cls_stride(int ldc) { return ((size_t)4 * ldc + 2 * CLS_CPTR + 63) & ~(size_t)63; }
+
+__device__ __forceinline__ unsigned long long cls_mix(unsigned long long x) {
+    x += 0x9e3779b97f4a7c15ull;
+    x = (x ^ (x >> 30)) * 0xbf58476d1ce4e5b9ull;
+    x = (x ^ (x >> 27)) * 0x94d049bb133111ebull;
+    return x ^ (x >> 31);
+}
+__device__ __forceinline__ long long cls_wave_add_i64(long long v) {
+#pragma unroll
+    for (int off = 32; off > 0; off >>= 1) v += __shfl_xor(v, off, 64);
+    return v;
+}
+
+__global__ __launch_bounds__(CLS_THREADS) void class_key_kernel(const uint8_t *__restrict__ rec, const int64_t *__restrict__ rec_off,
+                                                                const int32_t *__restrict__ ndist, int ldc, int H, int64_t R,
+                                                                long long *__restrict__ keys) {
+    __shared__ int s_hist[CLS_THREADS / 64][ENC_MAX_CODES];
+    const int lane = threadIdx.x & 63;
+    const int wv = __builtin_amdgcn_readfirstlane((int)(threadIdx.x >> 6));
+    int *hist = s_hist[wv];
+    const int ndw = ldc >> 2;
+    for (int64_t r = (int64_t)blockIdx.x * (CLS_THREADS / 64) + wv; r < R; r += (int64_t)gridDim.x * (CLS_THREADS / 64)) {
+        const int nd = ndist[r];
+        if (nd <= 0 || nd > ENC_MAX_CODES) {
+            if (lane == 0) keys[r] = -1;
+            continue;
+        }
+        const unsigned int *codes = reinterpret_cast<const unsigned int *>(rec + rec_off[r]);
+        wave_lds_fence();
+        for (int i = lane; i < ENC_MAX_CODES; i += 64) hist[i] = 0;
+        wave_lds_fence();
+        const int cand = (int)(codes[0] & 255u);
+        long long ncand = 0;
+        for (int i = lane; i < ndw; i += 64) {
+            const unsigned int wd = codes[i];
+#pragma unroll
+            for (int e = 0; e < 4; ++e) {
+                const int c = (int)((wd >> (8 * e)) & 255u);
+                if (4 * i + e < H) {
+                    if (c == cand) ++ncand;
+                    else atomicAdd(&hist[c], 1);
+                }
+            }
+        }
+        ncand = cls_wave_add_i64(ncand);
+        wave_lds_fence();
+        long long best = (ncand << 16) | (long long)(0xffff - cand);
+        for (int i = lane; i < ENC_MAX_CODES; i += 64) {
+            const long long v = ((long long)hist[i] << 16) | (long long)(0xffff - i);
+            best = v > best ? v : best;
+        }
+#pragma unroll
+        for (int off = 32; off > 0; off >>= 1) {
+            const long long o = __shfl_xor(best, off, 64);
+            best = o > best ? o : best;
+        }
+        const int maj = 0xffff - (int)(best & 0xffff);
+        unsigned long long key = 0ull;
+        for (int i = lane; i < ndw; i += 64) {
+            const unsigned int wd = codes[i];
+#pragma unroll
+            for (int e = 0; e < 4; ++e) {
+                const int c = (int)((wd >> (8 * e)) & 255u);
+                if (4 * i + e < H && c != maj) key += cls_mix((unsigned long long)(4 * i + e));
+            }
+        }
+        key = (unsigned long long)cls_wave_add_i64((long long)key);
+        if (lane == 0) keys[r] = (long long)(key >> 1);
+    }
+}
+
+__device__ __forceinline__ bool cls_row_ok(int64_t r, int64_t R, const int32_t *__restrict__ ndist) {
+    if (r < 0 || r >= R) return false;
+    const int nd = ndist[r];
+    return nd > 0 && nd <= ENC_MAX_CODES;
+}
+
+#define CLS_NJ (CLS_MAX_LDC / 4 / CLS_THREADS)
+__global__ __launch_bounds__(CLS_THREADS) void class_build_kernel(const uint8_t *__restrict__ rec, const int64_t *__restrict__ rec_off,
+                                                                  const int32_t *__restrict__ ndist, int ldc, int H, int64_t R,
+                                                                  const int64_t *__restrict__ rows, const int64_t *__restrict__ chunk_ptr,
+                                                                  int64_t n_chunks, int hash_rows, uint8_t *__restrict__ cdir,
+                                                                  int32_t *__restrict__ ncls) {
+    __shared__ unsigned long long s_tab[CLS_HASH];
+    __shared__ int s_first[CLS_HASH];
+    __shared__ unsigned short s_id[CLS_HASH];
+    __shared__ unsigned short s_cls[CLS_MAX_LDC];
+    __shared__ int s_scan[CLS_THREADS];
+    __shared__ int s_cnt[CLS_MAX + 1];
+    __shared__ int s_n;
+    const int t = threadIdx.x;
+    const int ndw = ldc >> 2;
+    const size_t stride = cls_stride(ldc);
+    for (int64_t k = blockIdx.x; k < n_chunks; k += gridDim.x) {
+        const int64_t lo = chunk_ptr[k];
+        int64_t nr64 = chunk_ptr[k + 1] - lo;
+        const int nrows = nr64 < 0 ? 0 : (nr64 > CLS_MAX_ROWS ? CLS_MAX_ROWS : (int)nr64);
+        for (int i = t; i < CLS_HASH; i += CLS_THREADS) {
+            s_tab[i] = 0ull;
+            s_first[i] = 0x7fffffff;
+        }
+        for (int i = t; i <= CLS_MAX; i += CLS_THREADS) s_cnt[i] = 0;
+        if (t == 0) s_n = 0;
+        unsigned long long acc[CLS_NJ][4];
+#pragma unroll
+        for (int j = 0; j < CLS_NJ; ++j)
+#pragma unroll
+            for (int e = 0; e < 4; ++e) acc[j][e] = 0ull;
+        const int nhash = (hash_rows > 0 && hash_rows < nrows) ? hash_rows : nrows;
+        for (int i = 0; i < nhash; ++i) {
+            const int64_t r = rows[lo + i];
+            if (!cls_row_ok(r, R, ndist)) continue;
+            const unsigned int *codes = reinterpret_cast<const unsigned int *>(rec + rec_off[r]);
+            const unsigned long long mul = cls_mix((unsigned long long)i) | 1ull;
+#pragma unroll
+            for (int j = 0; j < CLS_NJ; ++j) {
+                const int idx = t + CLS_THREADS * j;
+                if (idx < ndw) {
+                    const unsigned int wd = codes[idx];
+#pragma unroll
+                    for (int e = 0; e < 4; ++e) acc[j][e] += mul * (unsigned long long)(((wd >> (8 * e)) & 255u) + 1u);
+                }
+            }
+        }
+        __syncthreads();
+        int slot[CLS_NJ][4];
+#pragma unroll
+        for (int j = 0; j < CLS_NJ; ++j) {
+#pragma unroll
+            for (int e = 0; e < 4; ++e) {
+                const int col = 4 * (t + CLS_THREADS * j) + e;
+                slot[j][e] = -1;
+                if (col < H) {
+                    const unsigned long long h = cls_mix(acc[j][e]);
+                    const unsigned long long tagged = h | (1ull << 63);
+                    unsigned int at = (unsigned int)(cls_mix(h) & (CLS_HASH - 1));
+                    for (int probe = 0; probe < CLS_HASH; ++probe) {
+                        if (__hip_atomic_load(&s_n, __ATOMIC_RELAXED, __HIP_MEMORY_SCOPE_WORKGROUP) > CLS_MAX) break;
+                        unsigned long long old = __hip_atomic_load(&s_tab[at], __ATOMIC_RELAXED, __HIP_MEMORY_SCOPE_WORKGROUP);
+                        if (old == 0ull) {
+                            old = atomicCAS(&s_tab[at], 0ull, tagged);
+                            if (old == 0ull) atomicAdd(&s_n, 1);
+                        }
+                        if (old == 0ull || old == tagged) {
+                            slot[j][e] = (int)at;
+                            atomicMin(&s_first[at], col);
+                            break;
+                        }
+                        at = (at + 1) & (CLS_HASH - 1);
+                    }
+                }
+            }
+        }
+        __syncthreads();
+        const int n = s_n;
+        if (n > CLS_MAX || n < 1 || nrows < 1) {
+            if (t == 0) ncls[k] = 0;
+            __syncthreads();
+            continue;
+        }
+#pragma unroll
+        for (int j = 0; j < CLS_NJ; ++j)
+#pragma unroll
+            for (int e = 0; e < 4; ++e) {
+                const int col = 4 * (t + CLS_THREADS * j) + e;
+                if (col < H) s_cls[col] = (unsigned short)slot[j][e];
+            }
+        __syncthreads();
+        const int per = (H + CLS_THREADS - 1) / CLS_THREADS;
+        const int c_lo = t * per, c_hi = (c_lo + per < H) ? c_lo + per : H;
+        int mine = 0;
+        for (int col = c_lo; col < c_hi; ++col) mine += (s_first[s_cls[col]] == col) ? 1 : 0;
+        s_scan[t] = mine;
+        __syncthreads();
+        if (t == 0) {
+            int run = 0;
+            for (int i = 0; i < CLS_THREADS; ++i) {
+                const int x = s_scan[i];
+                s_scan[i] = run;
+                run += x;
+            }
+        }
+        __syncthreads();
+        int id = s_scan[t];
+        for (int col = c_lo; col < c_hi; ++col) {
+            const int sl = s_cls[col];
+            if (s_first[sl] == col) s_id[sl] = (unsigned short)id++;
+        }
+        __syncthreads();
+        uint8_t *dir = cdir + (size_t)k * stride;
+        unsigned long long *codes_out = reinterpret_cast<unsigned long long *>(dir);
+#pragma unroll
+        for (int j = 0; j < CLS_NJ; ++j) {
+            const int idx = t + CLS_THREADS * j;
+            unsigned long long word = 0ull;
+#pragma unroll
+            for (int e = 0; e < 4; ++e) {
+                const int col = 4 * idx + e;
+                if (col < H) {
+                    const unsigned int c = s_id[slot[j][e]];
+                    word |= (unsigned long long)c << (16 * e);
+                    s_cls[col] = (unsigned short)c;
+                    atomicAdd(&s_cnt[c], 1);
+                }
+            }
+            if (idx < ndw) codes_out[idx] = word;
+        }
+        __syncthreads();
+        if (t == 0) {
+            int run = 0;
+            for (int d = 0; d < n; ++d) {
+                const int x = s_cnt[d];
+                s_cnt[d] = run;
+                run += x;
+            }
+            s_cnt[n] = run;
+        }
+        __syncthreads();
+        unsigned short *perm = reinterpret_cast<unsigned short *>(dir + (size_t)2 * ldc);
+        unsigned short *cptr = reinterpret_cast<unsigned short *>(dir + (size_t)4 * ldc);
+        for (int d = t; d <= n; d += CLS_THREADS) cptr[d] = (unsigned short)s_cnt[d];
+        for (int d = t; d < n; d += CLS_THREADS) {
+            int pos = s_cnt[d];
+            for (int col = 0; col < H; ++col)
+                if (s_cls[col] == d) perm[pos++] = (unsigned short)col;
+        }
+        if (t == 0) ncls[k] = n;
+        __syncthreads();
+    }
+}
+
+__global__ __launch_bounds__(CLS_THREADS) void class_tables_kernel(const uint8_t *__restrict__ rec, const int64_t *__restrict__ rec_off,
+                                                                   const int32_t *__restrict__ ndist, int ldc, int H, int64_t R,
+                                                                   const int64_t *__restrict__ rows, const int64_t *__restrict__ chunk_ptr,
+                                                                   int64_t n_chunks, const uint8_t *__restrict__ cdir,
+                                                                   const int32_t *__restrict__ ncls, const int64_t *__restrict__ tab_off,
+                                                                   double *__restrict__ tab, int64_t tab_len,
+                                                                   int64_t *__restrict__ rows_out, uint8_t *__restrict__ in_class) {
+    __shared__ unsigned short s_cls[CLS_MAX_LDC];
+    __shared__ unsigned short s_cfirst[CLS_MAX];
+    __shared__ double s_pt[ENC_MAX_CODES];
+    __shared__ double s_t[CLS_MAX];
+    __shared__ int s_bad;
+    const int t = threadIdx.x;
+    const int ndw = ldc >> 2;
+    const size_t stride = cls_stride(ldc);
+    for (int64_t k = blockIdx.x; k < n_chunks; k += gridDim.x) {
+        const int64_t lo = chunk_ptr[k];
+        int64_t nr64 = chunk_ptr[k + 1] - lo;
+        const int nrows = nr64 < 0 ? 0 : (nr64 > CLS_MAX_ROWS ? CLS_MAX_ROWS : (int)nr64);
+        const int D = ncls[k];
+        const int64_t off = tab_off[k];
+        const bool fits = D >= 1 && D <= CLS_MAX && off >= 0 && off + (int64_t)nrows * D <= tab_len;
+        if (!fits) {
+            for (int i = t; i < nrows; i += CLS_THREADS) rows_out[lo + i] = -1;
+            continue;
+        }
+        const uint8_t *dir = cdir + (size_t)k * stride;
+        const unsigned short *codes_g = reinterpret_cast<const unsigned short *>(dir);
+        const unsigned short *perm = reinterpret_cast<const unsigned short *>(dir + (size_t)2 * ldc);
+        const unsigned short *cptr = reinterpret_cast<const unsigned short *>(dir + (size_t)4 * ldc);
+        __syncthreads();
+        for (int col = t; col < H; col += CLS_THREADS) s_cls[col] = codes_g[col] < D ? codes_g[col] : 0;
+        for (int d = t; d < D; d += CLS_THREADS) {
+            const int at = cptr[d];
+            const int col = at < H ? perm[at] : 0;
+            s_cfirst[d] = (unsigned short)(col < H ? col : 0);
+        }
+        if (t == 0) s_bad = 0;
+        __syncthreads();
+        for (int i = 0; i < nrows; ++i) {
+            const int64_t r = rows[lo + i];
+            if (!cls_row_ok(r, R, ndist)) {
+                for (int d = t; d < D; d += CLS_THREADS) tab[off + (int64_t)i * D + d] = 0.0;
+                if (t == 0) rows_out[lo + i] = -1;
+                continue;
+            }
+            const int nd = ndist[r];
+            const uint8_t *base = rec + rec_off[r];
+            s_pt[t] = (t < nd) ? reinterpret_cast<const double *>(base + ldc)[t] : 0.0;
+            int cf[CLS_MAX / CLS_THREADS];
+#pragma unroll
+            for (int m = 0; m < CLS_MAX / CLS_THREADS; ++m) {
+                const int d = t + CLS_THREADS * m;
+                cf[m] = d < D ? (int)base[s_cfirst[d]] : 0;
+            }
+            unsigned int wd[CLS_NJ];
+#pragma unroll
+            for (int j = 0; j < CLS_NJ; ++j) {
+                const int idx = t + CLS_THREADS * j;
+                wd[j] = idx < ndw ? reinterpret_cast<const unsigned int *>(base)[idx] : 0u;
+            }
+            __syncthreads();
+#pragma unroll
+            for (int m = 0; m < CLS_MAX / CLS_THREADS; ++m) {
+                const int d = t + CLS_THREADS * m;
+                if (d < D) {
+                    const double v = s_pt[cf[m]];
+                    s_t[d] = v;
+                    tab[off + (int64_t)i * D + d] = v;
+                }
+            }
+            __syncthreads();
+            bool bad = false;
+#pragma unroll
+            for (int j = 0; j < CLS_NJ; ++j) {
+#pragma unroll
+                for (int e = 0; e < 4; ++e) {
+                    const int col = 4 * (t + CLS_THREADS * j) + e;
+                    if (col < H) {
+                        const double a = s_pt[(wd[j] >> (8 * e)) & 255u], b = s_t[s_cls[col]];
+                        bad = bad || __double_as_longlong(a) != __double_as_longlong(b);
+                    }
+                }
+            }
+            if (bad) s_bad = 1;
+            __syncthreads();
+            if (t == 0) {
+                const bool ok = s_bad == 0;
+                rows_out[lo + i] = ok ? r : -1;
+                if (ok) in_class[r] = 1;
+                s_bad = 0;
+            }
+        }
+    }
+}
+
+template <int K, int RB>
+__device__ __forceinline__ void class_rows_pass(const double *__restrict__ tab, int D, int nrows, const int64_t *__restrict__ rows,
+                                                int64_t R, const double *__restrict__ w, const double *s_S, double *s_U, int wv,
+                                                int lane, int &fault) {
+    constexpr int NW = CLS_THREADS / 64;
+    double sreg[K], u[K];
+#pragma unroll
+    for (int k = 0; k < K; ++k) {
+        const int d = lane + 64 * k;
+        sreg[k] = d < D ? s_S[d] : 0.0;
+        u[k] = 0.0;
+    }
+    for (int i0 = wv * RB; i0 < nrows; i0 += NW * RB) {
+        double tv[RB][K], wr[RB];
+#pragma unroll
+        for (int j = 0; j < RB; ++j) {
+            const int i = i0 + j;
+            int64_t r = -1;
+            if (i < nrows) {
+                r = rows[i];
+                if (r >= R || r < -1) {
+                    fault = 1;
+                    r = -1;
+                }
+            }
+            wr[j] = r >= 0 ? (w != nullptr ? w[r] : 1.0) : 0.0;
+#pragma unroll
+            for (int k = 0; k < K; ++k) {
+                const int d = lane + 64 * k;
+                tv[j][k] = (r >= 0 && d < D) ? tab[(int64_t)i * D + d] : 0.0;
+            }
+        }
+#pragma unroll
+        for (int j = 0; j < RB; ++j) {
+            double z = 0.0;
+#pragma unroll
+            for (int k = 0; k < K; ++k) z = fma(tv[j][k], sreg[k], z);
+            z = wave_sum_lane63(z);
+            const double g = readlane_f64(weight_over_norm(wr[j], z), 63);
+#pragma unroll
+            for (int k = 0; k < K; ++k) u[k] = fma(g, tv[j][k], u[k]);
+        }
+    }
+#pragma unroll
+    for (int x = 0; x < NW; ++x) {
+        if (wv == x) {
+#pragma unroll
+            for (int k = 0; k < K; ++k) {
+                const int d = lane + 64 * k;
+                if (d < D) s_U[d] += u[k];
+            }
+        }
+        __syncthreads();
+    }
+}
+
+template <int NCH>
+__global__ __launch_bounds__(CLS_THREADS, 2) void em_iter_class_kernel(
+    const uint8_t *__restrict__ cdir, const int32_t *__restrict__ ncls, const int64_t *__restrict__ chunk_ptr,
+    const int64_t *__restrict__ tab_off, const double *__restrict__ tab, int64_t tab_len, const int64_t *__restrict__ rows,
+    int64_t n_member, int64_t n_chunks, int64_t R, const double *__restrict__ w, const double *__restrict__ props, int H, int ldc,
+    double *__restrict__ partial, int64_t ldpart, int part_row0, const mxm_em_state *__restrict__ state, int run,
+    const int32_t *__restrict__ ndist, const int32_t *__restrict__ nquad, const int64_t *__restrict__ quad_rows, int64_t n_quad,
+    const int64_t *__restrict__ byte_rows, int64_t n_byte) {
+    if (state != nullptr && state[run].done != 0) return;
+    __shared__ __attribute__((aligned(16))) double s_p[NCH * CLS_THREADS * 4];
+    __shared__ __attribute__((aligned(16))) double s_S[CLS_MAX];
+    __shared__ __attribute__((aligned(16))) double s_U[CLS_MAX];
+    __shared__ __attribute__((aligned(16))) unsigned short s_perm[NCH * CLS_THREADS * 4];
+    __shared__ unsigned short s_cptr[CLS_CPTR];
+    constexpr int CLS_NBIG = CLS_MAX_LDC / CLS_BIG + 8;
+    __shared__ unsigned short s_big[CLS_NBIG];
+    __shared__ int s_nbig;
+    const int t = threadIdx.x, lane = t & 63;
+    const int wv = __builtin_amdgcn_readfirstlane(t >> 6);
+    constexpr int NW = CLS_THREADS / 64;
+    props += (int64_t)run * H;
+    const int ndw = ldc >> 2;
+    const size_t stride = cls_stride(ldc);
+    double acc[NCH][4];
+#pragma unroll
+    for (int k = 0; k < NCH; ++k)
+#pragma unroll
+        for (int e = 0; e < 4; ++e) acc[k][e] = 0.0;
+    for (int c = t; c < NCH * CLS_THREADS * 4; c += CLS_THREADS) s_p[c] = c < H ? props[c] : 0.0;
+    int fault = 0;
+    {
+        const int64_t stride = (int64_t)gridDim.x * CLS_THREADS;
+        for (int64_t e = (int64_t)blockIdx.x * CLS_THREADS + t; e < n_quad; e += stride) {
+            const int64_t r = quad_rows[e];
+            if (r < 0 || r >= R || (e > 0 && quad_rows[e - 1] >= r)) fault = 1;
+            else if (nquad[r] < 1 || nquad[r] > QUAD_MAX || ndist[r] < 1 || ndist[r] > ENC_MAX_CODES) fault = 1;
+        }
+        for (int64_t e = (int64_t)blockIdx.x * CLS_THREADS + t; e < n_byte; e += stride) {
+            const int64_t r = byte_rows[e];
+            if (r < 0 || r >= R || (e > 0 && byte_rows[e - 1] >= r)) fault = 1;
+            else if (nquad[r] != 0 || ndist[r] < 1 || ndist[r] > ENC_MAX_CODES) fault = 1;
+        }
+    }
+    for (int64_t k = blockIdx.x; k < n_chunks; k += gridDim.x) {
+        const int D = ncls[k];
+        if (D == 0) continue;
+        const int64_t lo = chunk_ptr[k];
+        const int64_t nr64 = chunk_ptr[k + 1] - lo;
+        const int64_t off = tab_off[k];
+        if (D < 0 || D > CLS_MAX || nr64 < 1 || nr64 > CLS_MAX_ROWS || lo < 0 || lo + nr64 > n_member || off < 0 ||
+            off + nr64 * D > tab_len) {
+            fault = 1;
+            continue;
+        }
+        const int nrows = (int)nr64;
+        const uint8_t *dir = cdir + (size_t)k * stride;
+        const unsigned long long *codes_g = reinterpret_cast<const unsigned long long *>(dir);
+        const unsigned short *perm = reinterpret_cast<const unsigned short *>(dir + (size_t)2 * ldc);
+        const unsigned short *cptr = reinterpret_cast<const unsigned short *>(dir + (size_t)4 * ldc);
+        unsigned long long cw[NCH];
+#pragma unroll
+        for (int j = 0; j < NCH; ++j) {
+            const int idx = t + CLS_THREADS * j;
+            cw[j] = idx < ndw ? codes_g[idx] : 0ull;
+        }
+        __syncthreads();
+        for (int i = t; i < H; i += CLS_THREADS) {
+            const unsigned short c = perm[i];
+            s_perm[i] = c < H ? c : 0;
+        }
+        for (int d = t; d <= D; d += CLS_THREADS) {
+            const unsigned short at = cptr[d];
+            s_cptr[d] = at <= H ? at : (unsigned short)H;
+        }
+        for (int d = t; d < CLS_MAX; d += CLS_THREADS) s_U[d] = 0.0;
+        if (t == 0) s_nbig = 0;
+        __syncthreads();
+        for (int d = t; d < D; d += CLS_THREADS) {
+            const int a = s_cptr[d], b = s_cptr[d + 1];
+            if (b - a > CLS_BIG) {
+                const int at = atomicAdd(&s_nbig, 1);
+                if (at < CLS_NBIG) s_big[at] = (unsigned short)d;
+                else fault = 1;
+            } else {
+                double s = 0.0;
+                for (int i = a; i < b; ++i) s += s_p[s_perm[i]];
+                s_S[d] = s;
+            }
+        }
+        __syncthreads();
+        const int nbig = s_nbig < CLS_NBIG ? s_nbig : CLS_NBIG;
+        for (int x = wv; x < nbig; x += NW) {
+            const int d = s_big[x];
+            const int a = s_cptr[d], b = s_cptr[d + 1];
+            double s = 0.0;
+            for (int i = a + lane; i < b; i += 64) s += s_p[s_perm[i]];
+            s = wave_sum_lane63(s);
+            if (lane == 63) s_S[d] = s;
+        }
+        __syncthreads();
+        const double *tb = tab + off;
+        const int64_t *rw = rows + lo;
+        if (D <= 64) class_rows_pass<1, 8>(tb, D, nrows, rw, R, w, s_S, s_U, wv, lane, fault);
+        else if (D <= 128) class_rows_pass<2, 4>(tb, D, nrows, rw, R, w, s_S, s_U, wv, lane, fault);
+        else if (D <= 256) class_rows_pass<4, 2>(tb, D, nrows, rw, R, w, s_S, s_U, wv, lane, fault);
+        else class_rows_pass<16, 1>(tb, D, nrows, rw, R, w, s_S, s_U, wv, lane, fault);
+#pragma unroll
+        for (int j = 0; j < NCH; ++j) {
+#pragma unroll
+            for (int e = 0; e < 4; ++e) {
+                const unsigned int c = (unsigned int)(cw[j] >> (16 * e)) & (CLS_MAX - 1);
+                acc[j][e] += s_U[c];
+            }
+        }
+    }
+    const int64_t row = (int64_t)part_row0 + blockIdx.x;
+    fault = __syncthreads_or(fault);
+    if (t == 0) {
+        int *out = reinterpret_cast<int *>(partial + (int64_t)MXM_MAX_WG * ldpart) + 2 * row;
+        out[0] = 0;
+        out[1] = fault;
+    }
+    double *dst = partial + row * ldpart;
+#pragma unroll
+    for (int j = 0; j < NCH; ++j) {
+        const int c = 4 * (t + j * CLS_THREADS);
+#pragma unroll
+        for (int e = 0; e < 4; ++e)
+            if (c + e < H) dst[c + e] = acc[j][e];
+    }
+}
+
+#endif
diff --git a/mixemt_amd/csrc/mixemt_hip.hip b/mixemt_amd/csrc/mixemt_hip.hip
--- a/mixemt_amd/csrc/mixemt_hip.hip
+++ b/mixemt_amd/csrc/mixemt_hip.hip
@@ -13,6 +13,7 @@
 
 #include "mixemt_hip.h"
 #include "mixemt_hip_tuning.h"
+#include "mixemt_hip_classes.h"
 
 #include "common.hpp"
 #include "aln_encode.hpp"
@@ -20,6 +21,7 @@
 #include "coded_kernels.hpp"
 #include "quad_kernels.hpp"
 #include "quad_batched_kernels.hpp"
+#include "class_kernels.hpp"
 #include "build_kernels.hpp"
 #include "build_lut_kernels.hpp"
 #include "build_sparse_kernels.hpp"
@@ -57,6 +59,8 @@
     int quad_encoder = 1;
     int sparse_long = 1;
     int coded_bt = 3;
+    int class_form = -1;
+    int class_hash_rows = 0;
     int fused_force_abort = 0;
     double fused_cells = 1.0e8;
     hipEvent_t ev_start = nullptr, ev_stop = nullptr;
@@ -443,6 +447,11 @@
     if (bt != 1 && bt != 3) return fail(-1, "mxm_set_coded_batch_tile: 1 or 3, got %d", bt);
     return tune_set([bt](mxm_tuning &t) { t.coded_bt = bt; });
 }
+extern "C" int mxm_set_class_form(int32_t mode, int32_t hash_rows) {
+    if (mode < -1 || mode > 1 || hash_rows < 0 || hash_rows > CLS_MAX_ROWS)
+        return fail(-1, "mxm_set_class_form: mode -1, 0 or 1 and 0..%d hashed rows, got %d, %d", CLS_MAX_ROWS, mode, hash_rows);
+    return tune_set([=](mxm_tuning &t) { t.class_form = mode; t.class_hash_rows = hash_rows; });
+}
 extern "C" int mxm_set_quad_encoder(int32_t kind) {
     if (kind != 0 && kind != 1) return fail(-1, "mxm_set_quad_encoder: 0 or 1, got %d", kind);
     return tune_set([kind](mxm_tuning &t) { t.quad_encoder = kind; });
@@ -819,6 +828,7 @@
     return 0;
 }
 
+#define QUAD_MAX_NCH 6
 static int coded_check(const mxm_coded *c, int32_t H, const char *who) {
     if (c == nullptr || c->R <= 0 || H <= 0 || !mxm_linear_supported(H))
         return fail(-1, "%s: bad coded matrix (rows %lld, H %d)", who, (long long)(c ? c->R : 0), H);
@@ -835,7 +845,22 @@
         if (c->n_quad_rows + c->n_byte_rows + c->n_wide + c->R_rest != c->R)
             return fail(-1, "%s: quad_rows + byte_rows + wide_rows + the dense rest must be all %lld rows", who, (long long)c->R);
     }
-    return 0;
+    if (c->classes != nullptr) {
+        const mxm_classes *k = c->classes;
+        if (c->qrec == nullptr) return fail(-1, "%s: column classes need a quad dictionary", who);
+        if (k->n_chunks < 1 || k->n_member < 1 || k->tab_len < 0 || k->chunk_ptr == nullptr || k->rows == nullptr || k->cdir == nullptr ||
+            k->ncls == nullptr || k->tab_off == nullptr || (k->tab_len > 0 && k->tab == nullptr) || k->n_left_quad < 0 ||
+            k->n_left_byte < 0 || (k->n_left_quad > 0 && k->left_quad_rows == nullptr) ||
+            (k->n_left_byte > 0 && k->left_byte_rows == nullptr) || (reinterpret_cast<uintptr_t>(k->cdir) & 7))
+            return fail(-1, "%s: column class arrays missing (or cdir not 8-byte aligned)", who);
+        if (k->n_left_quad > c->n_quad_rows || k->n_left_byte > c->n_byte_rows)
+            return fail(-1, "%s: the class form's left-over lists are longer than the quad dictionary's lists", who);
+    }
+    return 0;
+}
+static bool classes_used(const mxm_coded *c, int H) {
+    return c != nullptr && c->classes != nullptr && c->qrec != nullptr && T.class_form != 0 &&
+           (coded_ld(H) / 4 + QUAD_THREADS - 1) / QUAD_THREADS <= QUAD_MAX_NCH;
 }
 
 static int rest_check(const char *who, int32_t H, const double *M_rest, int64_t ldm_rest, const int64_t *rest_rows, int64_t n_rest) {
@@ -902,6 +927,64 @@
                            reinterpret_cast<unsigned long long *>(stats));
     HIP_TRY(hipGetLastError());
     return 0;
+}
+
+static int class_args_check(const char *who, const mxm_coded *c, int32_t H) {
+    if (c == nullptr || c->R <= 0 || c->rec == nullptr || c->rec_off == nullptr || c->ndist == nullptr || !mxm_linear_supported(H))
+        return fail(-1, "%s: bad coded matrix (rows %lld, H %d)", who, (long long)(c ? c->R : 0), H);
+    if (coded_ld(H) > CLS_MAX_LDC) return fail(-1, "%s: H=%d beyond the class form's %d columns", who, H, CLS_MAX_LDC);
+    return 0;
+}
+extern "C" int mxm_class_keys(const mxm_coded *c, int32_t H, int64_t *keys, void *stream) {
+    MXM_ENTER();
+    RC_TRY(class_args_check("mxm_class_keys", c, H));
+    if (keys == nullptr) return fail(-1, "mxm_class_keys: keys required");
+    hipLaunchKernelGGL(class_key_kernel, dim3(clamp_grid((c->R + 3) / 4, num_cu() * 8)), dim3(CLS_THREADS), 0, (hipStream_t)stream,
+                       c->rec, c->rec_off, c->ndist, coded_ld(H), (int)H, c->R, reinterpret_cast<long long *>(keys));
+    HIP_TRY(hipGetLastError());
+    return 0;
+}
+extern "C" size_t mxm_class_bytes(int64_t n_chunks, int32_t H) {
+    return (n_chunks > 0 && H > 0) ? (size_t)n_chunks * cls_stride(coded_ld(H)) : 0;
+}
+extern "C" int mxm_build_classes(const mxm_coded *c, int32_t H, const int64_t *rows, const int64_t *chunk_ptr, int64_t n_chunks,
+                                 uint8_t *cdir, size_t cdir_bytes, int32_t *ncls, void *stream) {
+    MXM_ENTER();
+    RC_TRY(class_args_check("mxm_build_classes", c, H));
+    if (rows == nullptr || chunk_ptr == nullptr || n_chunks < 1 || cdir == nullptr || ncls == nullptr ||
+        (reinterpret_cast<uintptr_t>(cdir) & 7))
+        return fail(-1, "mxm_build_classes: rows, chunk_ptr, ncls and an 8-byte aligned cdir required");
+    if (cdir_bytes < mxm_class_bytes(n_chunks, H)) return fail(-1, "mxm_build_classes: cdir too small");
+    hipLaunchKernelGGL(class_build_kernel, dim3(clamp_grid(n_chunks, num_cu() * 4)), dim3(CLS_THREADS), 0, (hipStream_t)stream, c->rec,
+                       c->rec_off, c->ndist, coded_ld(H), (int)H, c->R, rows, chunk_ptr, n_chunks, T.class_hash_rows, cdir, ncls);
+    HIP_TRY(hipGetLastError());
+    return 0;
+}
+extern "C" int mxm_build_class_tables(const mxm_coded *c, int32_t H, const int64_t *rows, const int64_t *chunk_ptr,
+                                      int64_t n_chunks, const uint8_t *cdir, const int32_t *ncls, const int64_t *tab_off,
+                                      double *tab, int64_t tab_len, int64_t *rows_out, uint8_t *in_class, void *stream) {
+    MXM_ENTER();
+    RC_TRY(class_args_check("mxm_build_class_tables", c, H));
+    if (rows == nullptr || chunk_ptr == nullptr || n_chunks < 1 || cdir == nullptr || ncls == nullptr || tab_off == nullptr ||
+        tab_len < 0 || (tab_len > 0 && tab == nullptr) || rows_out == nullptr || rows_out == rows || in_class == nullptr)
+        return fail(-1, "mxm_build_class_tables: bad arguments");
+    hipLaunchKernelGGL(class_tables_kernel, dim3(clamp_grid(n_chunks, num_cu() * 4)), dim3(CLS_THREADS), 0, (hipStream_t)stream, c->rec,
+                       c->rec_off, c->ndist, coded_ld(H), (int)H, c->R, rows, chunk_ptr, n_chunks, cdir, ncls, tab_off, tab, tab_len,
+                       rows_out, in_class);
+    HIP_TRY(hipGetLastError());
+    return 0;
+}
+static int launch_classes(int nch, int nwg, hipStream_t stream, const mxm_coded *c ,
+                          int ldc, const double *w, const double *props, int H, double *partial, int64_t ldpart, int part_row0,
+                          const mxm_em_state *state, int run) {
+    const mxm_classes *k = c->classes;
+    const int64_t R = c->R;
+    const bool ok = dispatch_width<QUAD_MAX_NCH>(nch, [&](auto n) {
+        hipLaunchKernelGGL((em_iter_class_kernel<decltype(n)::value>), dim3(nwg), dim3(CLS_THREADS), 0, stream, k->cdir, k->ncls,
+                           k->chunk_ptr, k->tab_off, k->tab, k->tab_len, k->rows, k->n_member, k->n_chunks, R, w, props, H, ldc, partial,
+                           ldpart, part_row0, state, run, c->ndist, c->nquad, c->quad_rows, c->n_quad_rows, c->byte_rows, c->n_byte_rows);
+    });
+    return ok ? 0 : fail(-1, "mxm_em_iter_coded: H=%d outside the class kernel's range", H);
 }
 
 extern "C" int mxm_decode_rows(const mxm_coded *c, int32_t H, double *P, int64_t ldp, void *stream) {
@@ -1024,7 +1107,6 @@
     });
     return launched ? 0 : fail(-1, "mxm_em_iter_coded: H=%d outside the kernel's range", H);
 }
-#define QUAD_MAX_NCH 6
 static int quad_left_share(const mxm_coded *c, int slots) {
     if (c->n_byte_rows <= 0 && c->n_wide <= 0) return 0;
     const double left_cost = 1.0 * (double)c->n_byte_rows + 1.5 * (double)c->n_wide;
@@ -1067,12 +1149,29 @@
     if (cap > MXM_MAX_WG - num_cu()) cap = MXM_MAX_WG - num_cu();
     if (cap < 1) cap = 1;
     const bool quads = c->qrec != nullptr && c->n_quad_rows > 0 && nch <= QUAD_MAX_NCH;
-    int nwg_q = 0, nwg = 0;
+    const bool classes = quads && classes_used(c, H);
+    mxm_coded left;
+    const mxm_coded *whole = c;
+    if (classes) {
+        left = *c;
+        left.quad_rows = c->classes->left_quad_rows != nullptr ? c->classes->left_quad_rows : c->quad_rows;
+        left.n_quad_rows = c->classes->n_left_quad;
+        left.byte_rows = c->classes->left_byte_rows;
+        left.n_byte_rows = c->classes->n_left_byte;
+        c = &left;
+    }
+    int nwg_q = 0, nwg = 0, nwg_c = 0;
     if (quads) {
-        const int slots = cap < 2 * num_cu() ? cap : 2 * num_cu();
+        int slots = cap < 2 * num_cu() ? cap : 2 * num_cu();
+        if (classes && c->R_rest > 0 && slots > num_cu()) slots = num_cu();
         const int nwg_b = quad_left_share(c, slots);
         nwg_q = clamp_grid((c->n_quad_rows + sh.nbuf - 1) / sh.nbuf, slots - nwg_b < 1 ? 1 : slots - nwg_b);
         nwg = nwg_q + nwg_b;
+        if (classes) {
+            int room = MXM_MAX_WG - (c->R_rest > 0 ? num_cu() : 0) - nwg;
+            if (room > 2 * num_cu()) room = 2 * num_cu();
+            nwg_c = clamp_grid(c->classes->n_chunks, room < 1 ? 1 : room);
+        }
     } else {
         nwg = clamp_grid((c->R + sh.nbuf - 1) / sh.nbuf, cap);
     }
@@ -1083,6 +1182,11 @@
         if (nwg > nwg_q) lrc = launch_quad_coded(nch, nwg, nwg - nwg_q, stream, c, ldc, w, props, H, partial, ldpart, state, run);
         else lrc = launch_quad(nch, nwg_q, stream, c, w, props, H, partial, ldpart, state, run);
         if (lrc != 0) return lrc;
+        if (classes) {
+            lrc = launch_classes(nch, nwg_c, stream, whole, ldc, w, props, H, partial, ldpart, nwg, state, run);
+            if (lrc != 0) return lrc;
+            nwg += nwg_c;
+        }
     } else {
         lrc = launch_coded<256, 4, 2>(nch, nwg, stream, c, ldc, w, props, H, partial, ldpart, state, run);
         if (lrc != 0) return lrc;
@@ -1111,6 +1215,12 @@
 static int em_iter_coded_batched(const mxm_coded *c, const double *w, const double *props, int H, const mxm_slots &tile,
                                  const mxm_em_state *state, double *colsum, double *partial, hipStream_t stream, bool timed,
                                  const fin_args *fin = nullptr) {
+    if (classes_used(c, H)) {
+        for (int i = 0; i < QB_BT; ++i) {
+            RC_TRY(em_iter_coded_one(c, w, props, H, tile.s[i], state, colsum, partial, stream, timed && i == 0, fin));
+        }
+        return 0;
+    }
     const int64_t ldpart = part_ld(H);
     const int ldc = coded_ld(H);
     const int nch = ((ldc / 4 + QUAD_THREADS - 1) / QUAD_THREADS + 1) / 2;
@@ -1251,6 +1361,7 @@
 extern "C" int64_t mxm_quad_loop_min_rows(int32_t B) { return B >= 3 ? QUAD_BATCH_MIN_ROWS : QUAD_PER_ITER_MIN_ROWS; }
 static bool fused_coded_eligible(const mxm_coded *c, int H, int B, size_t ws_bytes, int running = 1) {
     if (T.loop_fused == 0 || c == nullptr || c->R_rest > 0 || !mxm_linear_supported(H) || (H & 1)) return false;
+    if (T.class_form == 1 && T.loop_fused != 1 && classes_used(c, H)) return false;
     if (c->qrec != nullptr && c->n_quad_rows >= QUAD_PER_ITER_MIN_ROWS && T.loop_fused != 1 &&
         (coded_ld(H) / 4 + QUAD_THREADS - 1) / QUAD_THREADS <= QUAD_MAX_NCH)
         return false;
diff --git a/mixemt_amd/em.py b/mixemt_amd/em.py
--- a/mixemt_amd/em.py
+++ b/mixemt_amd/em.py
@@ -69,6 +69,9 @@
 
 AUTO_CODED_MIN_CELLS = 1.5e7
 QUADS = {"off": False, "0": False, "on": True, "1": True}.get(os.environ.get("MXM_QUADS", "auto").strip().lower(), "auto")
+CLASSES = {"off": False, "0": False, "on": True, "1": True}.get(os.environ.get("MXM_CLASSES", "auto").strip().lower(), "auto")
+CLASS_MIN_RUN = 16
+CLASS_MAX_ROWS = 256
 QUADS_MIN_ROWS = 300000
 QUADS_MIN_ROWS_MULTI = 20000
 QUADS_MAX_FOOTPRINT = 60e9
@@ -201,6 +204,8 @@
             if not floor_ok or int(rec.numel()) + guess > QUADS_MAX_FOOTPRINT:
                 return False
         n_rows = self.n_rows
+        self._class_keep = None
+        self.coded.classes = None
         laps = {} if os.environ.get("MXM_PIPELINE_TIMING") else None
         self.quad_laps = laps
         t_lap = [time.perf_counter()]
@@ -270,6 +275,92 @@
         self._accounting = account
         for name in ("quad_bytes", "coded_record_bytes", "coded_bytes"):
             self.__dict__.pop(name, None)
+        self.attach_classes()
+        return True
+
+    def _class_chunks(self, min_run=CLASS_MIN_RUN, max_rows=CLASS_MAX_ROWS):
+        lib, dev, n_rows, n_haps = self.lib, self.dev, self.n_rows, self.n_haps
+        keys = torch.empty(n_rows, dtype=torch.int64, device=dev)
+        _lib.check(lib.mxm_class_keys(ctypes.byref(self.coded), n_haps, keys.data_ptr(), current_stream()), "mxm_class_keys")
+        elig = torch.nonzero(keys >= 0).squeeze(1)
+        if elig.numel() == 0:
+            return None
+        ks, idx = torch.sort(keys[elig], stable=True)
+        _, counts = torch.unique_consecutive(ks, return_counts=True)
+        cnt = counts.cpu().numpy().astype(numpy.int64)
+        keep = cnt >= max(1, int(min_run))
+        if not keep.any():
+            return None
+        member = elig[idx][torch.repeat_interleave(torch.from_numpy(keep).to(dev), counts)].contiguous()
+        run_rows = cnt[keep]
+        run_chunks = -(-run_rows // int(max_rows))
+        run_id = numpy.repeat(numpy.arange(len(run_rows)), run_chunks)
+        j = numpy.arange(int(run_chunks.sum())) - (numpy.cumsum(run_chunks) - run_chunks)[run_id]
+        size = run_rows[run_id] // run_chunks[run_id] + (j < run_rows[run_id] % run_chunks[run_id])
+        chunk_ptr_h = numpy.zeros(int(size.size) + 1, dtype=numpy.int64)
+        chunk_ptr_h[1:] = numpy.cumsum(size)
+        return member, chunk_ptr_h
+
+    def attach_classes(self, mode=None, min_run=CLASS_MIN_RUN, max_rows=CLASS_MAX_ROWS):
+        mode = CLASSES if mode is None else mode
+        if self.coded is None or mode is False or self._quad_keep is None or getattr(self, "_class_keep", None) is not None:
+            return getattr(self, "_class_keep", None) is not None
+        lib, dev, n_rows, n_haps = self.lib, self.dev, self.n_rows, self.n_haps
+        if (n_haps + 7) // 8 * 8 > 6144:
+            return False
+        ndist = self._coded_keep[2]
+        nquad = self._quad_keep[2]
+        stream = current_stream()
+        cut = self._class_chunks(min_run, max_rows)
+        if cut is None:
+            return False
+        member, chunk_ptr_h = cut
+        n_chunks = int(chunk_ptr_h.size) - 1
+        chunk_ptr = torch.from_numpy(chunk_ptr_h).to(dev)
+        try:
+            cdir = device_empty((int(lib.mxm_class_bytes(n_chunks, n_haps)),), torch.uint8, dev, "the class directory")
+        except ValueError:
+            if mode == "auto":
+                return False
+            raise
+        ncls = torch.empty(n_chunks, dtype=torch.int32, device=dev)
+        _lib.check(lib.mxm_build_classes(ctypes.byref(self.coded), n_haps, member.data_ptr(), chunk_ptr.data_ptr(), n_chunks,
+                                         cdir.data_ptr(), cdir.numel(), ncls.data_ptr(), stream), "mxm_build_classes")
+        sizes = (chunk_ptr[1:] - chunk_ptr[:-1]) * ncls.to(torch.int64)
+        tab_off = (torch.cumsum(sizes, 0) - sizes).contiguous()
+        tab_len = int(sizes.sum().item())
+        try:
+            tab = device_empty((max(1, tab_len),), torch.float64, dev, "the class tables")
+        except ValueError:
+            if mode == "auto":
+                return False
+            raise
+        rows_out = torch.empty_like(member)
+        in_class = torch.zeros(n_rows, dtype=torch.uint8, device=dev)
+        _lib.check(lib.mxm_build_class_tables(ctypes.byref(self.coded), n_haps, member.data_ptr(), chunk_ptr.data_ptr(), n_chunks,
+                                              cdir.data_ptr(), ncls.data_ptr(), tab_off.data_ptr(), tab.data_ptr(), tab_len,
+                                              rows_out.data_ptr(), in_class.data_ptr(), stream), "mxm_build_class_tables")
+        inside = in_class.bool()
+        n_in = int(inside.sum().item())
+        if n_in == 0:
+            return False
+        zero = torch.zeros_like(ndist)
+        nd_left, nq_left = torch.where(inside, zero, ndist), torch.where(inside, zero, nquad)
+        left_quad = torch.empty(n_rows, dtype=torch.int64, device=dev)
+        left_byte = torch.empty(n_rows, dtype=torch.int64, device=dev)
+        left_n = torch.empty(2, dtype=torch.int64, device=dev)
+        scratch = torch.empty(max(1, (lib.mxm_quad_lists_scratch_bytes(n_rows) + 7) // 8), dtype=torch.int64, device=dev)
+        _lib.check(lib.mxm_quad_lists(nd_left.data_ptr(), nq_left.data_ptr(), n_rows, left_quad.data_ptr(), left_byte.data_ptr(),
+                                      left_n.data_ptr(), scratch.data_ptr(), scratch.numel() * 8, stream), "mxm_quad_lists")
+        n_lq, n_lb = (int(v) for v in left_n.cpu())
+        left_quad, left_byte = left_quad[:n_lq].clone(), left_byte[:n_lb].clone()
+        self._classes = _lib.Classes(n_chunks, chunk_ptr.data_ptr(), rows_out.data_ptr(), int(member.numel()), cdir.data_ptr(),
+                                     ncls.data_ptr(), tab_off.data_ptr(), tab.data_ptr(), tab_len,
+                                     left_quad.data_ptr() if n_lq else None, n_lq, left_byte.data_ptr() if n_lb else None, n_lb)
+        self._class_keep = (chunk_ptr, rows_out, cdir, ncls, tab_off, tab, left_quad, left_byte, in_class)
+        self.coded.classes = ctypes.addressof(self._classes)
+        self.class_rows_n, self.class_left_n, self.class_chunks_n = n_in, n_lq + n_lb, n_chunks
+        self.class_bytes = int(cdir.numel()) + 8 * tab_len
         return True
 
     def __getattr__(self, name):
@@ -329,6 +420,7 @@
                                 w_rest.data_ptr() if n_rest else None, n_rest,
                                 wide.data_ptr() if self.coded_wide else None, self.coded_wide)
         self._quad_keep = None
+        self._class_keep = None
         self.attach_quads()
 
     def mat_args(self):
```

Result: no change. 865.1 billion, median of 2 (-0.1%).
